# hazdzz/STGCN

Measured on AMD Instinct MI355X. Metric: training windows/sec, METR-LA ChebConv K=3 bs=32, higher is better.
Workload: dtype f32; 1 GPU; C2: METR-LA 207 nodes, STGCNChebGraphConv Ks=3 Kt=3, n_his=12, bs=32 per GPU, fp32, dropout 0.5, AdamW lr 1e-3 wd 1e-3; full step zero_grad+fwd+MSE+bwd+opt; graph=real metr_la adj -> sym_norm_lap -> cheb GSO, global_batch=32, parallelism=dp1, output_block=fused HIP path (stgcn_outblock_*), launch=hipGraph replay, chains=1, backward_products=fp32, operator_products=fp32

## Files before the change

### include/stgcn_hip.h

```cpp
#ifndef STGCN_HIP_H
#define STGCN_HIP_H
#include <stddef.h>
#include <stdint.h>
#ifdef __cplusplus
extern "C" {
#endif

#define STGCN_ABI_VERSION 9

#define STGCN_OK 0
#define STGCN_ERR_UNSUPPORTED 1
#define STGCN_ERR_INVALID 2
#define STGCN_ERR_LAUNCH 3

#define STGCN_ACT_GLU 0
#define STGCN_ACT_GTU 1
#define STGCN_GC_CHEB 0
#define STGCN_GC_KIPF 1

#define STGCN_DTYPE_F32 0
#define STGCN_DTYPE_BF16 1

typedef struct stgcn_stblock_desc {
    int32_t B, T, N;
    int32_t c_in;
    int32_t c0, c1, c2;
    int32_t Kt, Ks;
    int32_t act;
    int32_t graph_conv;
    int32_t training;
    float droprate;
    float ln_eps;
    int32_t need_dx;
    int32_t reserved;
    int32_t prepacked;
    int32_t defer_reduce;
    int64_t x_bstride;
    const int64_t* x_index_dev;
    int64_t x_index_stride;
    const int64_t* x_window_dev;
    int32_t dy_rowstats_ready;
    int32_t dtype;
} stgcn_stblock_desc;

typedef struct stgcn_stblock_params {
    const float *tc1_w, *tc1_b, *tc1_aw, *tc1_ab;
    const float *al_w, *al_b;
    const float *gc_w, *gc_b;
    const float *tc2_w, *tc2_b, *tc2_aw, *tc2_ab;
    const float *ln_w, *ln_b;
} stgcn_stblock_params;

typedef struct stgcn_stblock_grads {
    float *tc1_w, *tc1_b, *tc1_aw, *tc1_ab;
    float *al_w, *al_b;
    float *gc_w, *gc_b;
    float *tc2_w, *tc2_b, *tc2_aw, *tc2_ab;
    float *ln_w, *ln_b;
} stgcn_stblock_grads;

typedef struct stgcn_stblock_plan {
    int64_t T1, T2, rows1, rows2, NP;
    int64_t y_floats;
    int64_t saved_floats, ws_floats;
    int64_t sv_U1, sv_S1;
    int64_t sv_A;
    int64_t sv_Xk;
    int64_t sv_G;
    int64_t sv_U2, sv_S2;
    int64_t sv_mean, sv_rstd;
    int64_t sv_rowstat;
    int64_t ws_W1p, ws_W1d, ws_b1, ws_Wap, ws_WaT, ws_ba, ws_W2p, ws_W2d, ws_b2;
    int64_t ws_W1dense;
    int64_t recompute_tc1;
    int64_t ws_WaDense;
    int64_t thin_tc1;
    int64_t ws_rowstat_b;
    int64_t ws_dZ2;
    int64_t ws_dYg;
    int64_t ws_dA;
    int64_t ws_dZ1;
    int64_t ws_part;
    int64_t part_floats;
    int64_t tiled_gc;
    int64_t ws_Gk;
    int64_t ws_XT;
    int64_t fused_tc2_bwd;
    int64_t ws_W2dense;
    int64_t fused_tc1_bwd;
    int64_t stored_US2;
    int64_t ws_chain;
    int64_t chain_words;
} stgcn_stblock_plan;

int stgcn_version(void);
const char* stgcn_backend(void);
const char* stgcn_last_error(void);

int stgcn_stblock_plan_query(const stgcn_stblock_desc* desc, stgcn_stblock_plan* plan);

int stgcn_gso_prepare(const float* gso, int32_t N, int32_t terms, float* gso_pad, float* gso_t_pad, float* scratch, void* stream);

int stgcn_gso_layout(int32_t N, int32_t terms, int64_t* NP, int64_t* mats, int64_t* scratch_mats, int32_t* tiled);

int stgcn_set_debug_stages(int32_t on);

int stgcn_set_tc1_bwd_wgs(int32_t n);

int stgcn_stblock_chain_status(const stgcn_stblock_desc* desc, const float* ws, uint32_t* sticky, void* stream);

int stgcn_set_tc2ln_peers(int32_t n);

int stgcn_set_gc_tiled_min_nodes(int32_t n);

int stgcn_set_gc_precision(int32_t mode);

int stgcn_set_slab_gc_precision(int32_t mode);

int stgcn_set_bwd_precision(int32_t mode);

int stgcn_set_gemm_big_nt(int32_t nt);

int stgcn_set_gc_ld_pad(int32_t pad);

int stgcn_stblock_forward(const stgcn_stblock_desc* desc, const stgcn_stblock_params* params, const float* x,
                          const float* gso_pad, float* y, float* saved, float* ws, uint64_t seed, uint64_t offset,
                          const uint64_t* offset_dev, void* stream);

int stgcn_stblock_backward(const stgcn_stblock_desc* desc, const stgcn_stblock_params* params, const float* x,
                           const float* gso_t_pad, const float* dy, const float* y, const float* saved, float* ws,
                           const stgcn_stblock_grads* grads, float* dx, uint64_t seed, uint64_t offset,
                           const uint64_t* offset_dev, void* stream);

typedef struct stgcn_ln_hook {
    float* rowstat;
    const float* y;
    const float *gamma, *beta;
    int32_t N, C, reserved, training;
    float droprate;
    int32_t dtype;
    uint64_t seed, offset;
    const uint64_t* offset_dev;
} stgcn_ln_hook;
int stgcn_stblock_ln_hook(const stgcn_stblock_desc* desc, const stgcn_stblock_params* params, const float* y, float* ws, uint64_t seed,
                          uint64_t offset, const uint64_t* offset_dev, stgcn_ln_hook* hook);
int stgcn_stblock_backward_hook(const stgcn_stblock_desc* desc, const stgcn_stblock_params* params, const float* x,
                                const float* gso_t_pad, const float* dy, const float* y, const float* saved, float* ws,
                                const stgcn_stblock_grads* grads, float* dx, uint64_t seed, uint64_t offset,
                                const uint64_t* offset_dev, const stgcn_ln_hook* dx_hook, void* stream);

int stgcn_dropout_mask(float* out, int64_t n, float droprate, uint64_t seed, uint64_t offset, const uint64_t* offset_dev,
                       void* stream);

typedef struct stgcn_outblock_desc {
    int32_t B, T, N;
    int32_t c_in, c0, c1, c_end;
    int32_t Ko;
    int32_t act;
    int32_t training;
    float droprate;
    float ln_eps;
    int32_t need_dx;
    int32_t dtype;
    int32_t prepacked;
    int32_t defer_reduce;
} stgcn_outblock_desc;

typedef struct stgcn_outblock_params {
    const float *tc_w, *tc_b, *tc_aw, *tc_ab, *ln_w, *ln_b, *fc1_w, *fc1_b, *fc2_w, *fc2_b;
} stgcn_outblock_params;
typedef struct stgcn_outblock_grads {
    float *tc_w, *tc_b, *tc_aw, *tc_ab, *ln_w, *ln_b, *fc1_w, *fc1_b, *fc2_w, *fc2_b;
    float* loss;
} stgcn_outblock_grads;

typedef struct stgcn_head_loss {
    const float* pred;
    const float* target;
    const int64_t* target_index_dev;
    int64_t target_index_stride;
    const int64_t* target_window_dev;
    float grad_scale;
    int32_t reserved;
} stgcn_head_loss;

typedef struct stgcn_outblock_plan {
    int64_t T1, rows, rows_in;
    int64_t out_floats;
    int64_t saved_floats, ws_floats;
    int64_t sv_U, sv_S;
    int64_t sv_mean, sv_rstd;
    int64_t sv_yln;
    int64_t sv_hd;
    int64_t sv_rowstat;
    int64_t ws_Wp, ws_Wd, ws_b, ws_W1p, ws_W1d;
    int64_t ws_rowstat_b, ws_dh1, ws_dyln, ws_dZ, ws_part, part_floats;
    int64_t ws_chain;
    int64_t chain_words;
} stgcn_outblock_plan;

int stgcn_outblock_plan_query(const stgcn_outblock_desc* desc, stgcn_outblock_plan* plan);
int stgcn_outblock_forward(const stgcn_outblock_desc* desc, const stgcn_outblock_params* params, const float* x, float* out,
                           float* saved, float* ws, uint64_t seed, uint64_t offset, const uint64_t* offset_dev, void* stream);
int stgcn_outblock_chain_status(const stgcn_outblock_desc* desc, const float* ws, uint32_t* sticky, void* stream);
int64_t stgcn_set_chain_spin_ticks(int64_t ticks);
int stgcn_outblock_backward(const stgcn_outblock_desc* desc, const stgcn_outblock_params* params, const float* x,
                            const float* dout, const float* saved, float* ws, const stgcn_outblock_grads* grads, float* dx,
                            void* stream);
int stgcn_outblock_backward_hook(const stgcn_outblock_desc* desc, const stgcn_outblock_params* params, const float* x,
                                 const float* dout, const float* saved, float* ws, const stgcn_outblock_grads* grads, float* dx,
                                 const stgcn_ln_hook* dx_hook, void* stream);
int stgcn_outblock_backward_loss(const stgcn_outblock_desc* desc, const stgcn_outblock_params* params, const float* x,
                                 const stgcn_head_loss* loss, const float* saved, float* ws, const stgcn_outblock_grads* grads, float* dx,
                                 const stgcn_ln_hook* dx_hook, void* stream);

typedef struct stgcn_prepack_block {
    const stgcn_stblock_desc* desc;
    const stgcn_stblock_params* params;
    float* ws;
} stgcn_prepack_block;
typedef struct stgcn_step_counter {
    int64_t* ptr;
    int64_t inc, mod;
} stgcn_step_counter;
int stgcn_prepack(int32_t n_blocks, const stgcn_prepack_block* blocks, const stgcn_outblock_desc* head_desc,
                  const stgcn_outblock_params* head_params, float* head_ws, int32_t n_counters, const stgcn_step_counter* counters,
                  void* stream);
int stgcn_prepack_park(int32_t n_blocks, const stgcn_prepack_block* blocks, const stgcn_outblock_desc* head_desc,
                  const stgcn_outblock_params* head_params, float* head_ws, int32_t n_counters, const stgcn_step_counter* counters,
                  void* stream);
int stgcn_prepack_flush(void);

typedef struct stgcn_adamw_tensor {
    float* param;
    const float* grad;
    float* exp_avg;
    float* exp_avg_sq;
    int64_t numel;
} stgcn_adamw_tensor;
int stgcn_adamw_step(const stgcn_adamw_tensor* tensors, int32_t count, float lr, float beta1, float beta2, float eps,
                     float weight_decay, int64_t step, const int64_t* step_dev, const float* lr_dev, void* stream);

typedef struct stgcn_flush_block {
    const stgcn_stblock_desc* desc;
    const stgcn_stblock_grads* grads;
    float* ws;
} stgcn_flush_block;
typedef struct stgcn_adamw_hyper {
    float lr, beta1, beta2, eps, weight_decay;
    int64_t step;
    const int64_t* step_dev;
    const float* lr_dev;
} stgcn_adamw_hyper;
int stgcn_grad_flush(int32_t n_blocks, const stgcn_flush_block* blocks, const stgcn_outblock_desc* head_desc,
                     const stgcn_outblock_grads* head_grads, float* head_ws, const stgcn_adamw_tensor* opt, int32_t opt_count,
                     const stgcn_adamw_hyper* hyper, void* stream);

#define STGCN_OPT_ADAMW 0
#define STGCN_OPT_NADAMW 1
#define STGCN_OPT_LION 2
typedef struct stgcn_optim_hyper {
    int32_t kind;
    double lr, beta1, beta2, eps, weight_decay, momentum_decay;
    int64_t step;
    const int64_t* step_dev;
    const float* lr_dev;
    float mu_product;
    float* mu_product_dev;
} stgcn_optim_hyper;
int stgcn_optim_step(const stgcn_adamw_tensor* tensors, int32_t count, const stgcn_optim_hyper* hyper, void* stream);
int stgcn_grad_flush_optim(int32_t n_blocks, const stgcn_flush_block* blocks, const stgcn_outblock_desc* head_desc,
                           const stgcn_outblock_grads* head_grads, float* head_ws, const stgcn_adamw_tensor* opt, int32_t opt_count,
                           const stgcn_optim_hyper* hyper, void* stream);

int stgcn_mse_loss_grad(const float* pred, const float* target, int64_t n, float grad_scale, float* loss, float* dpred,
                        const int64_t* target_index_dev, int64_t target_index_stride, void* stream);
int stgcn_mse_loss_grad_windows(const float* pred, const float* target, int64_t n, float grad_scale, float* loss, float* dpred,
                                const int64_t* target_index_dev, int64_t target_index_stride, const int64_t* target_window_dev,
                                int64_t window_floats, void* stream);

#define STGCN_EVAL_STATE_WORDS 264
#define STGCN_EVAL_POS_WORDS 4
int stgcn_eval_arm(double* state, int64_t* pos, void* stream);
int stgcn_eval_accumulate(const float* pred, const float* target, int32_t B, int32_t N, const float* scale, const float* mean,
                          int64_t first_valid, int64_t* pos, int64_t target_stride, int64_t num_windows, double* state, void* stream);

// ... 8 lines not shown
```

### stgcn_amd/_lib.py

```python
from __future__ import annotations

import ctypes as C
import os
from typing import Optional

_HERE = os.path.dirname(os.path.abspath(__file__))
DEFAULT_LIB = os.path.join(_HERE, "libstgcn_hip.so")

STGCN_OK = 0
ABI_VERSION = 9
ACT = {"glu": 0, "gtu": 1}
GRAPH_CONV = {"cheb_graph_conv": 0, "graph_conv": 1}
DTYPE_F32, DTYPE_BF16 = 0, 1
EVAL_STATE_WORDS, EVAL_POS_WORDS = 264, 4

_fp = C.POINTER(C.c_float)


class StblockDesc(C.Structure):
    _fields_ = [("B", C.c_int32), ("T", C.c_int32), ("N", C.c_int32), ("c_in", C.c_int32),
                ("c0", C.c_int32), ("c1", C.c_int32), ("c2", C.c_int32), ("Kt", C.c_int32), ("Ks", C.c_int32),
                ("act", C.c_int32), ("graph_conv", C.c_int32), ("training", C.c_int32),
                ("droprate", C.c_float), ("ln_eps", C.c_float), ("need_dx", C.c_int32), ("reserved", C.c_int32),
                ("prepacked", C.c_int32), ("defer_reduce", C.c_int32),
                ("x_bstride", C.c_int64), ("x_index_dev", C.c_void_p), ("x_index_stride", C.c_int64), ("x_window_dev", C.c_void_p),
                ("dy_rowstats_ready", C.c_int32), ("dtype", C.c_int32)]


class LnHook(C.Structure):
    _fields_ = [("rowstat", C.c_void_p), ("y", C.c_void_p), ("gamma", C.c_void_p), ("beta", C.c_void_p),
                ("N", C.c_int32), ("C", C.c_int32), ("reserved", C.c_int32), ("training", C.c_int32), ("droprate", C.c_float), ("dtype", C.c_int32),
                ("seed", C.c_uint64), ("offset", C.c_uint64), ("offset_dev", C.c_void_p)]


PARAM_FIELDS = ["tc1_w", "tc1_b", "tc1_aw", "tc1_ab", "al_w", "al_b", "gc_w", "gc_b",
                "tc2_w", "tc2_b", "tc2_aw", "tc2_ab", "ln_w", "ln_b"]


class StblockParams(C.Structure):
    _fields_ = [(n, C.c_void_p) for n in PARAM_FIELDS]


class StblockGrads(C.Structure):
    _fields_ = [(n, C.c_void_p) for n in PARAM_FIELDS]


PLAN_FIELDS = ["T1", "T2", "rows1", "rows2", "NP", "y_floats", "saved_floats", "ws_floats",
               "sv_U1", "sv_S1", "sv_A", "sv_Xk", "sv_G", "sv_U2", "sv_S2", "sv_mean", "sv_rstd", "sv_rowstat",
               "ws_W1p", "ws_W1d", "ws_b1", "ws_Wap", "ws_WaT", "ws_ba", "ws_W2p", "ws_W2d", "ws_b2", "ws_W1dense", "recompute_tc1", "ws_WaDense", "thin_tc1",
               "ws_rowstat_b", "ws_dZ2", "ws_dYg", "ws_dA", "ws_dZ1", "ws_part", "part_floats",
               "tiled_gc", "ws_Gk", "ws_XT", "fused_tc2_bwd", "ws_W2dense", "fused_tc1_bwd", "stored_US2", "ws_chain", "chain_words"]


class StblockPlan(C.Structure):
    _fields_ = [(n, C.c_int64) for n in PLAN_FIELDS]


class OutblockDesc(C.Structure):
    _fields_ = [("B", C.c_int32), ("T", C.c_int32), ("N", C.c_int32), ("c_in", C.c_int32), ("c0", C.c_int32), ("c1", C.c_int32),
                ("c_end", C.c_int32), ("Ko", C.c_int32), ("act", C.c_int32), ("training", C.c_int32), ("droprate", C.c_float),
                ("ln_eps", C.c_float), ("need_dx", C.c_int32), ("dtype", C.c_int32), ("prepacked", C.c_int32),
                ("defer_reduce", C.c_int32)]


HEAD_PARAM_FIELDS = ["tc_w", "tc_b", "tc_aw", "tc_ab", "ln_w", "ln_b", "fc1_w", "fc1_b", "fc2_w", "fc2_b"]


class OutblockParams(C.Structure):
    _fields_ = [(n, C.c_void_p) for n in HEAD_PARAM_FIELDS]


class PrepackBlock(C.Structure):
    _fields_ = [("desc", C.POINTER(StblockDesc)), ("params", C.POINTER(StblockParams)), ("ws", C.c_void_p)]


class OutblockGrads(C.Structure):
    _fields_ = [(n, C.c_void_p) for n in HEAD_PARAM_FIELDS] + [("loss", C.c_void_p)]


class HeadLoss(C.Structure):
    _fields_ = [("pred", C.c_void_p), ("target", C.c_void_p), ("target_index_dev", C.c_void_p), ("target_index_stride", C.c_int64),
                ("target_window_dev", C.c_void_p), ("grad_scale", C.c_float), ("reserved", C.c_int32)]


HEAD_PLAN_FIELDS = ["T1", "rows", "rows_in", "out_floats", "saved_floats", "ws_floats", "sv_U", "sv_S", "sv_mean", "sv_rstd", "sv_yln",
                    "sv_hd", "sv_rowstat", "ws_Wp", "ws_Wd", "ws_b", "ws_W1p", "ws_W1d", "ws_rowstat_b", "ws_dh1", "ws_dyln", "ws_dZ", "ws_part",
                    "part_floats", "ws_chain", "chain_words"]


class OutblockPlan(C.Structure):
    _fields_ = [(n, C.c_int64) for n in HEAD_PLAN_FIELDS]


class AdamwTensor(C.Structure):
    _fields_ = [("param", C.c_void_p), ("grad", C.c_void_p), ("exp_avg", C.c_void_p), ("exp_avg_sq", C.c_void_p), ("numel", C.c_int64)]


class StepCounter(C.Structure):
    _fields_ = [("ptr", C.c_void_p), ("inc", C.c_int64), ("mod", C.c_int64)]


class FlushBlock(C.Structure):
    _fields_ = [("desc", C.POINTER(StblockDesc)), ("grads", C.POINTER(StblockGrads)), ("ws", C.c_void_p)]


class AdamwHyper(C.Structure):
    _fields_ = [("lr", C.c_float), ("beta1", C.c_float), ("beta2", C.c_float), ("eps", C.c_float), ("weight_decay", C.c_float),
                ("step", C.c_int64), ("step_dev", C.c_void_p), ("lr_dev", C.c_void_p)]


OPT_ADAMW, OPT_NADAMW, OPT_LION = 0, 1, 2


class OptimHyper(C.Structure):
    _fields_ = [("kind", C.c_int32), ("lr", C.c_double), ("beta1", C.c_double), ("beta2", C.c_double), ("eps", C.c_double),
                ("weight_decay", C.c_double), ("momentum_decay", C.c_double), ("step", C.c_int64), ("step_dev", C.c_void_p),
                ("lr_dev", C.c_void_p), ("mu_product", C.c_float), ("mu_product_dev", C.c_void_p)]


class StgcnError(RuntimeError):
    pass


class _Lib:
    def __init__(self, path: str):
        if not os.path.exists(path):
            raise StgcnError(
                f"{path} not found: the HIP extension has not been built. Run `python -c 'import __graft_entry__ as g; "
                f"g.build()'` (or `python -m stgcn_amd.build`). There is no fallback path.")
        self.path = path
        self.dll = C.CDLL(path)
        d = self.dll
        d.stgcn_version.restype = C.c_int
        got = int(d.stgcn_version())
        if got != ABI_VERSION:
            raise StgcnError(f"{path} was built for ABI revision {got}, this binding needs {ABI_VERSION} (include/stgcn_hip.h "
                             f"STGCN_ABI_VERSION): rebuild with `python -m stgcn_amd.build --force`")
        d.stgcn_backend.restype = C.c_char_p
        d.stgcn_last_error.restype = C.c_char_p
        d.stgcn_stblock_plan_query.argtypes = [C.POINTER(StblockDesc), C.POINTER(StblockPlan)]
        d.stgcn_gso_prepare.argtypes = [C.c_void_p, C.c_int32, C.c_int32, C.c_void_p, C.c_void_p, C.c_void_p, C.c_void_p]
        d.stgcn_gso_layout.argtypes = [C.c_int32, C.c_int32, C.POINTER(C.c_int64), C.POINTER(C.c_int64), C.POINTER(C.c_int64),
                                       C.POINTER(C.c_int32)]
        d.stgcn_gso_layout.restype = C.c_int
        d.stgcn_set_gc_tiled_min_nodes.argtypes = [C.c_int32]
        d.stgcn_set_gc_tiled_min_nodes.restype = C.c_int
        d.stgcn_outblock_backward_loss.argtypes = [C.POINTER(OutblockDesc), C.POINTER(OutblockParams), C.c_void_p, C.POINTER(HeadLoss), C.c_void_p,
                                                   C.c_void_p, C.POINTER(OutblockGrads), C.c_void_p, C.POINTER(LnHook), C.c_void_p]
        d.stgcn_outblock_backward_loss.restype = C.c_int
        d.stgcn_set_bwd_precision.argtypes = [C.c_int32]
        d.stgcn_set_bwd_precision.restype = C.c_int
        d.stgcn_set_slab_gc_precision.argtypes = [C.c_int32]
        d.stgcn_set_slab_gc_precision.restype = C.c_int
        d.stgcn_set_tc1_bwd_wgs.argtypes = [C.c_int32]
        d.stgcn_set_tc1_bwd_wgs.restype = C.c_int
        d.stgcn_set_tc2ln_peers.argtypes = [C.c_int32]
        d.stgcn_set_tc2ln_peers.restype = C.c_int
        d.stgcn_stblock_chain_status.argtypes = [C.POINTER(StblockDesc), C.c_void_p, C.POINTER(C.c_uint32), C.c_void_p]
        d.stgcn_stblock_chain_status.restype = C.c_int
        d.stgcn_set_debug_stages.argtypes = [C.c_int32]
        d.stgcn_set_debug_stages.restype = C.c_int
        d.stgcn_set_gc_precision.argtypes = [C.c_int32]
        d.stgcn_set_gc_precision.restype = C.c_int
        d.stgcn_set_gc_ld_pad.argtypes = [C.c_int32]
        d.stgcn_set_gc_ld_pad.restype = C.c_int
        d.stgcn_set_gemm_big_nt.argtypes = [C.c_int32]
        d.stgcn_set_gemm_big_nt.restype = C.c_int
        d.stgcn_set_chain_spin_ticks.argtypes = [C.c_int64]
        d.stgcn_set_chain_spin_ticks.restype = C.c_int64
        d.stgcn_outblock_chain_status.argtypes = [C.POINTER(OutblockDesc), C.c_void_p, C.POINTER(C.c_uint32), C.c_void_p]
        d.stgcn_outblock_chain_status.restype = C.c_int
        d.stgcn_stblock_forward.argtypes = [C.POINTER(StblockDesc), C.POINTER(StblockParams), C.c_void_p, C.c_void_p,
                                            C.c_void_p, C.c_void_p, C.c_void_p, C.c_uint64, C.c_uint64, C.c_void_p, C.c_void_p]
        d.stgcn_stblock_backward.argtypes = [C.POINTER(StblockDesc), C.POINTER(StblockParams), C.c_void_p, C.c_void_p,
                                             C.c_void_p, C.c_void_p, C.c_void_p, C.c_void_p, C.POINTER(StblockGrads), C.c_void_p,
                                             C.c_uint64, C.c_uint64, C.c_void_p, C.c_void_p]
        d.stgcn_stblock_backward_hook.argtypes = [C.POINTER(StblockDesc), C.POINTER(StblockParams), C.c_void_p, C.c_void_p,
                                                  C.c_void_p, C.c_void_p, C.c_void_p, C.c_void_p, C.POINTER(StblockGrads), C.c_void_p,
                                                  C.c_uint64, C.c_uint64, C.c_void_p, C.POINTER(LnHook), C.c_void_p]
        d.stgcn_stblock_ln_hook.argtypes = [C.POINTER(StblockDesc), C.POINTER(StblockParams), C.c_void_p, C.c_void_p, C.c_uint64, C.c_uint64,
                                            C.c_void_p, C.POINTER(LnHook)]
        d.stgcn_outblock_backward_hook.argtypes = [C.POINTER(OutblockDesc), C.POINTER(OutblockParams), C.c_void_p, C.c_void_p, C.c_void_p,
                                                   C.c_void_p, C.POINTER(OutblockGrads), C.c_void_p, C.POINTER(LnHook), C.c_void_p]
        for f in ("stgcn_stblock_backward_hook", "stgcn_stblock_ln_hook", "stgcn_outblock_backward_hook"):
            getattr(d, f).restype = C.c_int
        d.stgcn_dropout_mask.argtypes = [C.c_void_p, C.c_int64, C.c_float, C.c_uint64, C.c_uint64, C.c_void_p, C.c_void_p]
        d.stgcn_outblock_plan_query.argtypes = [C.POINTER(OutblockDesc), C.POINTER(OutblockPlan)]
        d.stgcn_outblock_forward.argtypes = [C.POINTER(OutblockDesc), C.POINTER(OutblockParams), C.c_void_p, C.c_void_p, C.c_void_p,
                                             C.c_void_p, C.c_uint64, C.c_uint64, C.c_void_p, C.c_void_p]
        d.stgcn_outblock_backward.argtypes = [C.POINTER(OutblockDesc), C.POINTER(OutblockParams), C.c_void_p, C.c_void_p, C.c_void_p,
                                              C.c_void_p, C.POINTER(OutblockGrads), C.c_void_p, C.c_void_p]
        for f in ("stgcn_outblock_plan_query", "stgcn_outblock_forward", "stgcn_outblock_backward"):
            getattr(d, f).restype = C.c_int
        d.stgcn_adamw_step.argtypes = [C.POINTER(AdamwTensor), C.c_int32, C.c_float, C.c_float, C.c_float, C.c_float, C.c_float, C.c_int64,
                                       C.c_void_p, C.c_void_p, C.c_void_p]
        d.stgcn_adamw_step.restype = C.c_int
        d.stgcn_prepack.argtypes = [C.c_int32, C.POINTER(PrepackBlock), C.POINTER(OutblockDesc), C.POINTER(OutblockParams), C.c_void_p,
                                    C.c_int32, C.POINTER(StepCounter), C.c_void_p]
        d.stgcn_prepack.restype = C.c_int
        d.stgcn_prepack_park.argtypes = [C.c_int32, C.POINTER(PrepackBlock), C.POINTER(OutblockDesc), C.POINTER(OutblockParams), C.c_void_p,
                                    C.c_int32, C.POINTER(StepCounter), C.c_void_p]
        d.stgcn_prepack_park.restype = C.c_int
        d.stgcn_prepack_flush.argtypes = []
        d.stgcn_prepack_flush.restype = C.c_int
        d.stgcn_grad_flush.argtypes = [C.c_int32, C.POINTER(FlushBlock), C.POINTER(OutblockDesc), C.POINTER(OutblockGrads), C.c_void_p,
                                       C.POINTER(AdamwTensor), C.c_int32, C.POINTER(AdamwHyper), C.c_void_p]
        d.stgcn_grad_flush.restype = C.c_int
        d.stgcn_optim_step.argtypes = [C.POINTER(AdamwTensor), C.c_int32, C.POINTER(OptimHyper), C.c_void_p]
        d.stgcn_optim_step.restype = C.c_int
        d.stgcn_grad_flush_optim.argtypes = [C.c_int32, C.POINTER(FlushBlock), C.POINTER(OutblockDesc), C.POINTER(OutblockGrads), C.c_void_p,
                                             C.POINTER(AdamwTensor), C.c_int32, C.POINTER(OptimHyper), C.c_void_p]
        d.stgcn_grad_flush_optim.restype = C.c_int
        d.stgcn_mse_loss_grad.argtypes = [C.c_void_p, C.c_void_p, C.c_int64, C.c_float, C.c_void_p, C.c_void_p, C.c_void_p, C.c_int64,
                                          C.c_void_p]
        d.stgcn_mse_loss_grad.restype = C.c_int
        d.stgcn_mse_loss_grad_windows.argtypes = [C.c_void_p, C.c_void_p, C.c_int64, C.c_float, C.c_void_p, C.c_void_p, C.c_void_p, C.c_int64,
                                                  C.c_void_p, C.c_int64, C.c_void_p]
        d.stgcn_mse_loss_grad_windows.restype = C.c_int
        d.stgcn_eval_arm.argtypes = [C.c_void_p, C.c_void_p, C.c_void_p]
        d.stgcn_eval_arm.restype = C.c_int
        d.stgcn_eval_accumulate.argtypes = [C.c_void_p, C.c_void_p, C.c_int32, C.c_int32, C.c_void_p, C.c_void_p, C.c_int64, C.c_void_p,
                                            C.c_int64, C.c_int64, C.c_void_p, C.c_void_p]
        d.stgcn_eval_accumulate.restype = C.c_int
        d.stgcn_profile_enable.argtypes = [C.c_int]
        d.stgcn_profile_enable.restype = C.c_int
        d.stgcn_profile_collect.argtypes = [C.c_char_p, C.c_size_t]
        d.stgcn_profile_collect.restype = C.c_int
        for f in ("stgcn_stblock_plan_query", "stgcn_gso_prepare", "stgcn_stblock_forward", "stgcn_stblock_backward",
                  "stgcn_dropout_mask"):
            getattr(d, f).restype = C.c_int
        self.backend = d.stgcn_backend().decode()
        self.is_emulator = self.backend.startswith("emu")

    def check(self, rc: int, what: str):
        if rc != STGCN_OK:
            msg = self.dll.stgcn_last_error().decode()
            if rc == 1:
                raise NotImplementedError(f"{what}: {msg}")
            if rc == 2:
                raise ValueError(f"{what}: {msg}")
            raise StgcnError(f"{what}: {msg} (code {rc})")


_lib: Optional[_Lib] = None


def use_library(path: str) -> _Lib:
    global _lib
    _lib = _Lib(path)
    return _lib


def lib() -> _Lib:
    global _lib
    if _lib is None:
        _lib = _Lib(os.environ.get("STGCN_AMD_LIB", DEFAULT_LIB))
    return _lib


EXPORTED_SYMBOLS = ["stgcn_version", "stgcn_backend", "stgcn_last_error", "stgcn_stblock_plan_query", "stgcn_gso_prepare",
                    "stgcn_stblock_forward", "stgcn_stblock_backward", "stgcn_dropout_mask", "stgcn_profile_enable",
                    "stgcn_profile_collect", "stgcn_outblock_plan_query", "stgcn_outblock_forward", "stgcn_outblock_backward", "stgcn_adamw_step", "stgcn_prepack",
                    "stgcn_mse_loss_grad", "stgcn_mse_loss_grad_windows", "stgcn_grad_flush", "stgcn_gso_layout", "stgcn_set_gc_tiled_min_nodes",
                    "stgcn_set_gc_precision", "stgcn_set_gc_ld_pad", "stgcn_set_debug_stages",
                    "stgcn_stblock_ln_hook", "stgcn_stblock_backward_hook", "stgcn_outblock_backward_hook", "stgcn_set_tc1_bwd_wgs",
                    "stgcn_set_slab_gc_precision", "stgcn_outblock_backward_loss", "stgcn_set_bwd_precision", "stgcn_set_gemm_big_nt",
                    "stgcn_set_chain_spin_ticks", "stgcn_outblock_chain_status", "stgcn_set_tc2ln_peers", "stgcn_stblock_chain_status", "stgcn_prepack_park", "stgcn_prepack_flush",
                    "stgcn_optim_step", "stgcn_grad_flush_optim", "stgcn_eval_arm", "stgcn_eval_accumulate"]
```

### stgcn_amd/csrc/stgcn_capi_head.inc

```

struct HeadGeom {
    int T1, NC, KP, KCH, CPin, ln_spg, ln_sg, fc_wgs;
    int dense_bwd;
    int fused_ln_bwd;
    int64_t rows, rows_in, slabs;
    WgradGeom wc, wf;
    long off_ln_g, off_ln_b, off_fc, total;
};

static int head_check(const stgcn_outblock_desc* d) {
    if (!d) return fail(STGCN_ERR_INVALID, "desc is NULL");
    if (d->B < 1 || d->T < 1 || d->N < 1 || d->c_in < 1 || d->Ko < 1) return fail(STGCN_ERR_INVALID, "B/T/N/c_in/Ko must be positive");
    if (d->T < d->Ko) return fail(STGCN_ERR_INVALID, "T=%d shorter than Ko=%d", d->T, d->Ko);
    if (d->act != STGCN_ACT_GLU && d->act != STGCN_ACT_GTU) return fail(STGCN_ERR_INVALID, "act must be glu or gtu");
    if (d->droprate < 0.f || d->droprate >= 1.f) return fail(STGCN_ERR_INVALID, "droprate must be in [0, 1)");
    if (!(d->c0 == 64 || d->c0 == 128)) return fail(STGCN_ERR_UNSUPPORTED, "output-head conv channels must be 64 or 128 (got %d)", d->c0);
    if (d->c1 != 128) return fail(STGCN_ERR_UNSUPPORTED, "output-head fc1 width must be 128 (got %d)", d->c1);
    if (d->c_end != 1) return fail(STGCN_ERR_UNSUPPORTED, "end_channel must be 1 (got %d)", d->c_end);
    if ((d->c_in & 3) != 0 && d->Ko * d->c_in > 16) return fail(STGCN_ERR_UNSUPPORTED, "c_in=%d must be a multiple of 4", d->c_in);
    if (d->dtype != STGCN_DTYPE_F32 && d->dtype != STGCN_DTYPE_BF16) return fail(STGCN_ERR_INVALID, "dtype must be STGCN_DTYPE_F32 or STGCN_DTYPE_BF16");
    return STGCN_OK;
}

static HeadGeom head_geom(const stgcn_outblock_desc* d) {
    HeadGeom g;
    g.T1 = d->T - d->Ko + 1;
    g.NC = 2 * d->c0;
    g.KP = (int)rup((int64_t)d->Ko * d->c_in, 16);
    g.KCH = g.KP / 16;
    g.CPin = (int)rup(d->c_in, 16);
    {
        static const int off = getenv("STGCN_TCONV4") ? atoi(getenv("STGCN_TCONV4")) == 0 : 0;
        g.dense_bwd = !off && g.T1 == 1 && g.NC == 256 && d->Ko * d->c_in == 256 && (d->c_in & 3) == 0;
    }
    g.rows = (int64_t)d->B * g.T1 * d->N;
    g.rows_in = (int64_t)d->B * d->T * d->N;
    g.slabs = (int64_t)d->B * g.T1;
    const long n = (long)d->N * d->c0, n4 = n / 4;
    const int colgroups = (int)((n4 + kThreads - 1) / kThreads);
    int sg = (512 + colgroups - 1) / colgroups;
    if (colgroups >= kLnBigColgroups) sg = (4096 + colgroups - 1) / colgroups;
    if (sg > g.slabs) sg = (int)g.slabs;
    if (sg < 1) sg = 1;
    g.ln_spg = (int)((g.slabs + sg - 1) / sg);
    g.ln_sg = (int)((g.slabs + g.ln_spg - 1) / g.ln_spg);
    const bool fusable = (fuse_mask() & FUSE_HEAD_LN_BWD) && (fuse_mask() & FUSE_ROWSTATS) && g.dense_bwd && d->c0 == 128 && d->c1 == 128 &&
                         d->N <= 1024 && colgroups < kLnBigColgroups;
    const long sg_plain = g.ln_sg, sg_max = fusable && g.slabs > sg_plain ? g.slabs : sg_plain;
    g.fused_ln_bwd = fusable && d->need_dx;
    if (g.fused_ln_bwd) { g.ln_spg = 1; g.ln_sg = (int)g.slabs; }
    const long tiles = (g.rows + head_fc_tile_rows() - 1) / head_fc_tile_rows();
    g.fc_wgs = (int)(tiles < 512 * 32 / head_fc_tile_rows() / 2 ? tiles : 512 * 32 / head_fc_tile_rows() / 2);
    long o = 0;
    auto take = [&](long f) { long at = o; o += (f + 63) / 64 * 64; return at; };
    g.off_ln_g = take(sg_max * n);
    g.off_ln_b = take((d->dtype == STGCN_DTYPE_BF16 ? sg_max : sg_plain) * n);
    g.off_fc = take((long)g.fc_wgs * (d->c1 + 2));
    constexpr int t_conv = 160, t_fc = 96;
    const bool one_round = g.rows <= 32768;
    g.wc = wgrad_geom(g.rows, d->Ko * d->c_in, g.NC, 0, one_round ? t_conv : 256);
    g.wc.off = take(g.wc.floats);
    g.wf = wgrad_geom(g.rows, d->c0, d->c1, 0, one_round ? t_fc : 256);
    g.wf.off = take(g.wf.floats);
    g.total = o;
    return g;
}

static void reduce_jobs_head(ReduceList& L, const stgcn_outblock_desc* d, const HeadGeom& g, const float* part, const float* dyln,
                             const stgcn_outblock_grads* G) {
    {
        const WgradGeom& w = g.wc;
        const float* wp = part + w.off;
        const float* bp = wp + (long)w.chunks * w.Mpad * w.NC;
        const long ps = (long)w.Mpad * w.NC;
        L.add(G->tc_w, wp, w.chunks, ps, w.NC, d->Ko, d->c_in, w.Mpad, d->c_in, 1, (long)d->c_in * d->Ko, 1, d->Ko);
        L.add_flat(G->tc_b, bp, w.chunks, w.NC, w.NC);
        if (d->c_in > d->c0) {
            L.add(G->tc_aw, wp + (long)(d->Ko - 1) * d->c_in, w.chunks, ps, 1, d->c0, d->c_in, 0, w.Mpad, 1, 0, d->c_in, 1);
            L.add_flat(G->tc_ab, bp, w.chunks, w.NC, d->c0);
        }
    }
    {
        const WgradGeom& w = g.wf;
        const float* wp = part + w.off;
        const float* bp = wp + (long)w.chunks * w.Mpad * w.NC;
        L.add(G->fc1_w, wp, w.chunks, (long)w.Mpad * w.NC, 1, d->c1, d->c0, 0, w.Mpad, 1, 0, d->c0, 1);
        L.add_flat(G->fc1_b, bp, w.chunks, w.NC, d->c1);
    }
    L.add_flat(G->fc2_w, part + g.off_fc, g.fc_wgs, d->c1 + 2, d->c1);
    L.add_flat(G->fc2_b, part + g.off_fc + d->c1, g.fc_wgs, d->c1 + 2, 1);
    if (G->loss) L.add_flat(G->loss, part + g.off_fc + d->c1 + 1, g.fc_wgs, d->c1 + 2, 1);
    const int n = d->N * d->c0;
    L.add_flat(G->ln_w, part + g.off_ln_g, g.ln_sg, n, n);
    if (g.fused_ln_bwd && d->dtype == STGCN_DTYPE_F32) L.add_flat(G->ln_b, dyln, g.ln_sg, n, n);
    else L.add_flat(G->ln_b, part + g.off_ln_b, g.ln_sg, n, n);
}

int stgcn_outblock_plan_query(const stgcn_outblock_desc* d, stgcn_outblock_plan* p) {
    int rc = head_check(d);
    if (rc) return rc;
    if (!p) return fail(STGCN_ERR_INVALID, "plan is NULL");
    const HeadGeom g = head_geom(d);
    memset(p, 0, sizeof(*p));
    p->T1 = g.T1; p->rows = g.rows; p->rows_in = g.rows_in; p->out_floats = g.rows * d->c_end;
    int64_t o = 0;
    auto take = [&](int64_t n) { int64_t at = o; o += rup(n, 64); return at; };
    const bool bf = d->dtype == STGCN_DTYPE_BF16;
    auto act = [&](int64_t n) { return bf ? (n + 1) / 2 : n; };
    p->sv_U = take(act(g.rows * d->c0));
    p->sv_S = take(act(g.rows * d->c0));
    p->sv_mean = take(g.slabs);
    p->sv_rstd = take(g.slabs);
    p->sv_yln = take(act(g.rows * d->c0));
    p->sv_hd = take(act(g.rows * d->c1));
    p->sv_rowstat = take(2 * g.rows);
    p->saved_floats = o;
    o = 0;
    p->chain_words = kChainHdr + g.slabs;
    p->ws_chain = take(p->chain_words);
    p->ws_Wp = take((int64_t)g.NC * g.KP);
    p->ws_Wd = take((int64_t)d->Ko * g.NC * g.CPin);
    p->ws_b = take(g.NC);
    p->ws_W1p = take((int64_t)d->c0 * d->c1);
    p->ws_W1d = take((int64_t)d->c1 * d->c0);
    p->ws_rowstat_b = take(2 * g.rows + 2 * g.slabs);
    p->ws_dh1 = take(act(g.rows * d->c1));
    p->ws_dyln = take(act(g.rows * d->c0));
    p->ws_dZ = take(act(g.rows * g.NC));
    p->part_floats = g.total;
    p->ws_part = take(g.total);
    p->ws_floats = o;
    return STGCN_OK;
}

}
namespace {
bool pack_fill_head(PackList& L, const stgcn_outblock_desc* d, const stgcn_outblock_params* P, const stgcn_outblock_plan& pl, float* ws,
                    bool all) {
    const HeadGeom g = head_geom(d);
    bool ok = true;
    ok &= L.add(PK_TCONV_FWD, g.NC * g.KP, ws + pl.ws_Wp, P->tc_w, P->tc_b, P->tc_aw, P->tc_ab, d->c_in, d->c0, d->Ko, g.KCH);
    if (d->need_dx || all) {
        if (g.dense_bwd)
            ok &= L.add(PK_TCONV_BWDT, g.NC * d->Ko * d->c_in, ws + pl.ws_Wd, P->tc_w, P->tc_b, P->tc_aw, P->tc_ab, d->c_in, d->c0, d->Ko, g.NC / 16);
        else
            ok &= L.add(PK_TCONV_BWD, d->Ko * g.NC * g.CPin, ws + pl.ws_Wd, P->tc_w, P->tc_b, P->tc_aw, P->tc_ab, d->c_in, d->c0, d->Ko,
                        d->Ko * g.NC / 16);
    }
    ok &= L.add(PK_TCONV_BIAS, g.NC, ws + pl.ws_b, P->tc_w, P->tc_b, P->tc_aw, P->tc_ab, d->c_in, d->c0, d->Ko, 0);
    ok &= L.add(PK_LIN_FWD, d->c0 * d->c1, ws + pl.ws_W1p, P->fc1_w, nullptr, nullptr, nullptr, d->c0, d->c1, 1, d->c0 / 16);
    ok &= L.add(PK_LIN_BWD, d->c1 * d->c0, ws + pl.ws_W1d, P->fc1_w, nullptr, nullptr, nullptr, d->c0, d->c1, 1, d->c1 / 16);
    ok &= L.add(PK_ZERO, (int)pl.chain_words, ws + pl.ws_chain, nullptr, nullptr, nullptr, nullptr, 0, 0, 0, 0);
    return ok;
}
}
extern "C" {

}
namespace {
int prepack_impl(int32_t n_blocks, const stgcn_prepack_block* blocks, const stgcn_outblock_desc* hd, const stgcn_outblock_params* hp,
                 float* hws, int32_t n_counters, const stgcn_step_counter* counters, void* stream, bool park);
}
extern "C" {
int stgcn_prepack(int32_t n_blocks, const stgcn_prepack_block* blocks, const stgcn_outblock_desc* hd, const stgcn_outblock_params* hp,
                  float* hws, int32_t n_counters, const stgcn_step_counter* counters, void* stream) {
    return prepack_impl(n_blocks, blocks, hd, hp, hws, n_counters, counters, stream, false);
}
int stgcn_prepack_flush(void) {
    return flush_pending_pack();
}
int stgcn_prepack_park(int32_t n_blocks, const stgcn_prepack_block* blocks, const stgcn_outblock_desc* hd, const stgcn_outblock_params* hp,
                       float* hws, int32_t n_counters, const stgcn_step_counter* counters, void* stream) {
    return prepack_impl(n_blocks, blocks, hd, hp, hws, n_counters, counters, stream, true);
}
}
namespace {
int prepack_impl(int32_t n_blocks, const stgcn_prepack_block* blocks, const stgcn_outblock_desc* hd, const stgcn_outblock_params* hp,
                 float* hws, int32_t n_counters, const stgcn_step_counter* counters, void* stream, bool park) {
    if (n_blocks < 0 || (n_blocks > 0 && !blocks)) return fail(STGCN_ERR_INVALID, "stgcn_prepack: bad block list");
    if (n_counters < 0 || n_counters > kMaxStepCounters || (n_counters > 0 && !counters))
        return fail(STGCN_ERR_INVALID, "stgcn_prepack: at most %d step counters", kMaxStepCounters);
    STGCN_FLUSH_PENDING_PACK();
    g_prof_tag = 0;
    PackList L;
    L.pa.ncounters = n_counters;
    for (int k = 0; k < n_counters; ++k) {
        if (!counters[k].ptr) return fail(STGCN_ERR_INVALID, "stgcn_prepack: NULL step counter %d", k);
        L.pa.cptr[k] = reinterpret_cast<long*>(counters[k].ptr); L.pa.cinc[k] = (long)counters[k].inc; L.pa.cmod[k] = (long)counters[k].mod;
    }
    auto flush_list = [&]() -> int {
        const int rc = launch_pack_list("prepack", L, (hipStream_t)stream);
        L = PackList();
        return rc;
    };
    for (int i = 0; i < n_blocks; ++i) {
        const stgcn_prepack_block& b = blocks[i];
        if (!b.desc || !b.params || !b.ws) return fail(STGCN_ERR_INVALID, "stgcn_prepack: NULL entry in block %d", i);
        stgcn_stblock_plan pl;
        int rc = stgcn_stblock_plan_query(b.desc, &pl);
        if (rc) return rc;
        PackList trial = L;
        if (!pack_fill_block(trial, b.desc, b.params, pl, b.ws, true)) {
            if (L.nj == 0) return fail(STGCN_ERR_UNSUPPORTED, "stgcn_prepack: one block needs more than %d pack jobs", kMaxPackJobs);
            rc = flush_list();
            if (rc) return rc;
            trial = L;
            if (!pack_fill_block(trial, b.desc, b.params, pl, b.ws, true)) return fail(STGCN_ERR_UNSUPPORTED, "stgcn_prepack: pack job table overflow");
        }
        L = trial;
    }
    if (hd) {
        if (!hp || !hws) return fail(STGCN_ERR_INVALID, "stgcn_prepack: head params / ws are NULL");
        stgcn_outblock_plan pl;
        int rc = stgcn_outblock_plan_query(hd, &pl);
        if (rc) return rc;
        PackList trial = L;
        if (!pack_fill_head(trial, hd, hp, pl, hws, true)) {
            rc = flush_list();
            if (rc) return rc;
            trial = L;
            if (!pack_fill_head(trial, hd, hp, pl, hws, true)) return fail(STGCN_ERR_UNSUPPORTED, "stgcn_prepack: pack job table overflow");
        }
        L = trial;
    }
    if (L.nj == 0 && L.pa.ncounters == 0) return STGCN_OK;
    if (park && L.nj > 0) {
        g_pending_pack.valid = true;
        g_pending_pack.L = L;
        g_pending_pack.st = (hipStream_t)stream;
        return STGCN_OK;
    }
    return launch_pack_list("prepack", L, (hipStream_t)stream);
}
}
extern "C" {

int stgcn_outblock_forward(const stgcn_outblock_desc* d, const stgcn_outblock_params* P, const float* x, float* out, float* saved,
                           float* ws, uint64_t seed, uint64_t offset, const uint64_t* offset_dev, void* stream) {
    STGCN_FLUSH_PENDING_PACK();
    stgcn_outblock_plan pl;
    int rc = stgcn_outblock_plan_query(d, &pl);
    if (rc) return rc;
    if (!P || !x || !out || !saved || !ws) return fail(STGCN_ERR_INVALID, "stgcn_outblock_forward: NULL buffer");
    if (!P->tc_w || !P->tc_b || !P->ln_w || !P->ln_b || !P->fc1_w || !P->fc2_w)
        return fail(STGCN_ERR_INVALID, "stgcn_outblock_forward: missing parameter pointer");
    if (d->c_in > d->c0 && !P->tc_aw) return fail(STGCN_ERR_INVALID, "tc_aw required when c_in > c0");
    const HeadGeom g = head_geom(d);
    hipStream_t st = (hipStream_t)stream;
    g_prof_tag = 0;
    g_bf16 = d->dtype == STGCN_DTYPE_BF16;

    if (!d->prepacked) {
        PackList L;
        if (!pack_fill_head(L, d, P, pl, ws, false)) return fail(STGCN_ERR_INVALID, "pack job table overflow");
        rc = launch_pack_list("head.pack", L, st);
        if (rc) return rc;
    }

    TconvFwdArgs t;
    memset(&t, 0, sizeof(t));
    t.ts.src = x; t.ts.C = d->c_in; t.ts.taps = d->Ko; t.ts.N = d->N; t.ts.Tsrc = d->T; t.ts.Tdst = g.T1; t.ts.dir = 1; t.ts.rows = g.rows;
    t.Wp = ws + pl.ws_Wp; t.bias = ws + pl.ws_b; t.KCH = g.KCH; t.Cout = d->c0; t.act = d->act;
    t.U = saved + pl.sv_U; t.S = saved + pl.sv_S; t.rowstat = reinterpret_cast<float2*>(saved + pl.sv_rowstat);

    if (head_fuse_mode() && g.T1 == 1 && d->c0 == 128 && d->c1 == 128 && tconv4_ok(t)) {
        constexpr int KC = 4;
        int tm = 0, ticket = 0;
        {
            const int forced = head_fuse_mode() > 1 ? head_fuse_mode() : 0;
            const size_t l2 = (size_t)(tconv2_lds_floats(g.KP, 256, 32) + 48) * sizeof(float), l4 = (size_t)(tconv2_lds_floats(g.KP, 256, 64) + 48) * sizeof(float);
            const int cap2 = STGCN_ET_VALUE(wg_capacity(head_fwd_kernel<2, KC, ET>, 512, l2));
            const int cap4 = STGCN_ET_VALUE(wg_capacity(head_fwd_kernel<4, KC, ET>, 512, l4));
            const int t2 = cdiv(g.rows, 32), t4 = cdiv(g.rows, 64);
            const bool tk2 = d->N >= 32 && d->N <= 1024 && cap2 >= 4 * cdiv(d->N, 32) + 16, tk4 = d->N >= 64 && d->N <= 2048 && cap4 >= 4 * cdiv(d->N, 64) + 16;
            if (forced == 2) { if (d->N >= 32 && t2 <= cap2) tm = 2; }
            else if (forced == 4) { if (d->N >= 64 && t4 <= cap4) tm = 4; }
            else if (forced == 3) { if (tk2) { tm = 2; ticket = 1; } }
            else if (forced == 5) { if (tk4) { tm = 4; ticket = 1; } }
            else if (tk2 && t2 <= cap2) { tm = 2; ticket = 1; }
            else if (tk4 && t4 <= cap4) { tm = 4; ticket = 1; }
            else if (tk2) { tm = 2; ticket = 1; }
            else if (tk4) { tm = 4; ticket = 1; }
        }
        if (tm) {
            Tconv4Args aa;
            memset(&aa, 0, sizeof(aa));
            aa.f = t;
            HeadFcTail f;
            memset(&f, 0, sizeof(f));
            const int TR = 16 * tm, tiles = cdiv(g.rows, TR);
            f.chain.words = reinterpret_cast<unsigned*>(ws + pl.ws_chain); f.chain.ncount = (int)g.slabs; f.chain.total = (unsigned)tiles;
            f.chain.spin = g_chain_spin_ticks;
            f.gamma = P->ln_w; f.beta = P->ln_b; f.yln = saved + pl.sv_yln; f.mean = saved + pl.sv_mean; f.rstd = saved + pl.sv_rstd;
            f.eps = d->ln_eps;
            f.W1p = ws + pl.ws_W1p; f.b1 = P->fc1_b; f.w2 = P->fc2_w; f.b2 = P->fc2_b; f.hd = saved + pl.sv_hd; f.out = out;
            f.training = d->training && d->droprate > 0.f;
            f.keep_scale = 1.0f / (1.0f - d->droprate); f.thresh = drop_thresh(d->droprate); f.seed = seed; f.offset = offset;
            f.offset_dev = offset_dev;
            f.use_ticket = ticket;
            const size_t lds = (size_t)(tconv2_lds_floats(g.KP, 256, TR) + 48) * sizeof(float);
            if (tm == 2) STGCN_LAUNCH_ET("head.fwd", st, (head_fwd_kernel<2, KC, ET>), dim3(tiles), dim3(512), lds, aa, f);
            else STGCN_LAUNCH_ET("head.fwd", st, (head_fwd_kernel<4, KC, ET>), dim3(tiles), dim3(512), lds, aa, f);
            return STGCN_OK;
        }
    }
    rc = launch_tconv_fwd("head.tconv_fwd", t, st);
    if (rc) return rc;

    LnFwdArgs ln;
    memset(&ln, 0, sizeof(ln));
    ln.U = saved + pl.sv_U; ln.S = saved + pl.sv_S; ln.gamma = P->ln_w; ln.beta = P->ln_b; ln.y = saved + pl.sv_yln;
    ln.mean = saved + pl.sv_mean; ln.rstd = saved + pl.sv_rstd; ln.rowstat = reinterpret_cast<const float2*>(saved + pl.sv_rowstat);
    ln.n = d->N * d->c0; ln.N = d->N; ln.C = d->c0; ln.act = d->act; ln.training = 0;
    ln.eps = d->ln_eps; ln.keep_scale = 1.f; ln.thresh = 0;
    const bool fuse_ln = (fuse_mask() & FUSE_HEAD_LN_FWD) && g.T1 == 1 && d->c0 % 16 == 0 && d->c0 <= 128 && d->N <= 1024;
    if (!fuse_ln) {
        rc = launch_ln_fwd("head.ln_fwd", ln, g.slabs, st);
        if (rc) return rc;
    }

    FcFwdArgs f;
    memset(&f, 0, sizeof(f));
    if (fuse_ln) f.ln = ln;
    f.ts.src = saved + pl.sv_yln; f.ts.C = d->c0; f.ts.taps = 1; f.ts.N = d->N; f.ts.Tsrc = g.T1; f.ts.Tdst = g.T1; f.ts.dir = 1;
    f.ts.rows = g.rows;
    f.W1p = ws + pl.ws_W1p; f.b1 = P->fc1_b; f.w2 = P->fc2_w; f.b2 = P->fc2_b; f.hd = saved + pl.sv_hd; f.out = out;
    f.KCH = d->c0 / 16; f.c1 = d->c1; f.training = d->training && d->droprate > 0.f;
    f.keep_scale = 1.0f / (1.0f - d->droprate); f.thresh = drop_thresh(d->droprate); f.seed = seed; f.offset = offset;
    f.offset_dev = offset_dev;
    const int fct = (getenv("STGCN_HEAD_FC_TILE") || g.rows <= 32768) ? head_fc_tile_rows() : 32;
    const size_t lds = (size_t)(kTileHdr + fct * (128 + 4)) * sizeof(float);
    if (fct == 16) STGCN_LAUNCH_ET("head.fc_fwd", st, (fc_fwd_kernel<1, ET>), dim3(cdiv(g.rows, 16)), dim3(kThreads), lds, f);
    else STGCN_LAUNCH_ET("head.fc_fwd", st, (fc_fwd_kernel<2, ET>), dim3(cdiv(g.rows, 32)), dim3(kThreads), lds, f);
    return STGCN_OK;
}


int stgcn_outblock_chain_status(const stgcn_outblock_desc* d, const float* ws, uint32_t* sticky, void* stream) {
    STGCN_FLUSH_PENDING_PACK();
    stgcn_outblock_plan pl;
    int rc = stgcn_outblock_plan_query(d, &pl);
    if (rc) return rc;
    if (!ws || !sticky) return fail(STGCN_ERR_INVALID, "stgcn_outblock_chain_status: NULL argument");
    if (hipStreamSynchronize((hipStream_t)stream) != hipSuccess) return fail(STGCN_ERR_LAUNCH, "stgcn_outblock_chain_status: stream synchronisation failed");
    unsigned w = 0;
    if (hipMemcpy(&w, reinterpret_cast<const unsigned*>(ws + pl.ws_chain) + 2, sizeof(w), hipMemcpyDeviceToHost) != hipSuccess)
        return fail(STGCN_ERR_LAUNCH, "stgcn_outblock_chain_status: copy failed");
    *sticky = w;
    return STGCN_OK;
}

}
namespace {
int outblock_backward_impl(const stgcn_outblock_desc* d, const stgcn_outblock_params* P, const float* x, const float* dout,
                           const stgcn_head_loss* hl, const float* saved, float* ws, const stgcn_outblock_grads* G, float* dx,
                           const stgcn_ln_hook* dx_hook, void* stream);
}
extern "C" {
int stgcn_outblock_backward(const stgcn_outblock_desc* d, const stgcn_outblock_params* P, const float* x, const float* dout,
                            const float* saved, float* ws, const stgcn_outblock_grads* G, float* dx, void* stream) {
    return outblock_backward_impl(d, P, x, dout, nullptr, saved, ws, G, dx, nullptr, stream);
}

int stgcn_outblock_backward_hook(const stgcn_outblock_desc* d, const stgcn_outblock_params* P, const float* x, const float* dout,
                                 const float* saved, float* ws, const stgcn_outblock_grads* G, float* dx, const stgcn_ln_hook* dx_hook,
                                 void* stream) {
    return outblock_backward_impl(d, P, x, dout, nullptr, saved, ws, G, dx, dx_hook, stream);
}

int stgcn_outblock_backward_loss(const stgcn_outblock_desc* d, const stgcn_outblock_params* P, const float* x, const stgcn_head_loss* hl,
                                 const float* saved, float* ws, const stgcn_outblock_grads* G, float* dx, const stgcn_ln_hook* dx_hook,
                                 void* stream) {
    if (!hl || !hl->pred || !hl->target) return fail(STGCN_ERR_INVALID, "stgcn_outblock_backward_loss: NULL pred / target");
    if (!G || !G->loss) return fail(STGCN_ERR_INVALID, "stgcn_outblock_backward_loss: grads->loss is NULL");
    if (hl->target_window_dev && !hl->target_index_dev)
        return fail(STGCN_ERR_INVALID, "stgcn_outblock_backward_loss: target_window_dev (window table) needs target_index_dev != NULL");
    return outblock_backward_impl(d, P, x, nullptr, hl, saved, ws, G, dx, dx_hook, stream);
}
}
namespace {
int outblock_backward_impl(const stgcn_outblock_desc* d, const stgcn_outblock_params* P, const float* x, const float* dout,
                           const stgcn_head_loss* hl, const float* saved, float* ws, const stgcn_outblock_grads* G, float* dx,
                           const stgcn_ln_hook* dx_hook, void* stream) {
    STGCN_FLUSH_PENDING_PACK();
    stgcn_outblock_plan pl;
    int rc = stgcn_outblock_plan_query(d, &pl);
    if (rc) return rc;
    if (!P || !x || (!dout && !hl) || !saved || !ws || !G) return fail(STGCN_ERR_INVALID, "stgcn_outblock_backward: NULL buffer");
    if (d->need_dx && !dx) return fail(STGCN_ERR_INVALID, "stgcn_outblock_backward: need_dx set but dx is NULL");
    if (dx_hook && dx_hook->rowstat && (dx_hook->N != d->N || dx_hook->C != d->c_in || !d->need_dx))
        return fail(STGCN_ERR_INVALID, "stgcn_outblock_backward: dx_hook describes a LayerNorm over [%d, %d], the input gradient is [%d, %d] per slab",
                    dx_hook->N, dx_hook->C, d->N, d->c_in);
    const HeadGeom g = head_geom(d);
    hipStream_t st = (hipStream_t)stream;
    g_prof_tag = 0;
    g_bf16 = d->dtype == STGCN_DTYPE_BF16;
    if (dx_hook && dx_hook->rowstat && dx_hook->dtype != d->dtype)
        return fail(STGCN_ERR_INVALID, "stgcn_outblock_backward: dx_hook describes tensors of another dtype than this call");
    float* part = ws + pl.ws_part;
    const int training = d->training && d->droprate > 0.f;
    const bool own_rowstats = (fuse_mask() & FUSE_ROWSTATS) && d->c0 == d->c1 && d->c0 == 128;

    {
        FcBwdArgs a;
        memset(&a, 0, sizeof(a));
        a.dout = dout; a.hd = saved + pl.sv_hd; a.w2 = P->fc2_w; a.W1d = ws + pl.ws_W1d; a.dh1 = ws + pl.ws_dh1; a.dyln = ws + pl.ws_dyln;
        a.part = part + g.off_fc; a.rows = g.rows; a.c0 = d->c0; a.c1 = d->c1; a.KCH = d->c1 / 16;
        a.grad_scale = training ? 1.0f / (1.0f - d->droprate) : 1.0f;
        if (hl) {
            a.pred = hl->pred; a.target = hl->target; a.target_index = reinterpret_cast<const long*>(hl->target_index_dev);
            a.target_index_stride = (long)hl->target_index_stride; a.loss_scale = hl->grad_scale;
            a.target_window = reinterpret_cast<const long*>(hl->target_window_dev); a.target_window_elems = (unsigned)(g.rows / d->B);
        }
        if (own_rowstats) {
            a.rs.rowstat = reinterpret_cast<float2*>(ws + pl.ws_rowstat_b); a.rs.U = saved + pl.sv_U; a.rs.S = saved + pl.sv_S; a.rs.gamma = P->ln_w;
            a.rs.mean = saved + pl.sv_mean; a.rs.rstd = saved + pl.sv_rstd; a.rs.N = d->N; a.rs.C = d->c0; a.rs.act = d->act; a.rs.training = 0;
            a.rs.keep_scale = 1.f;
        }
        const size_t lds = (size_t)(head_fc_tile_rows() * (d->c1 + 4) + 8 * d->c1 + 16) * sizeof(float);
        if (head_fc_tile_rows() == 16) {
            if (d->c0 == 128) STGCN_LAUNCH_ETB("head.fc_bwd", st, (fc_bwd_kernel<1, 2, ET>), dim3(g.fc_wgs), dim3(kThreads), lds, a);
            else STGCN_LAUNCH_ETB("head.fc_bwd", st, (fc_bwd_kernel<1, 1, ET>), dim3(g.fc_wgs), dim3(kThreads), lds, a);
        } else if (d->c0 == 128) STGCN_LAUNCH_ETB("head.fc_bwd", st, (fc_bwd_kernel<2, 2, ET>), dim3(g.fc_wgs), dim3(kThreads), lds, a);
        else STGCN_LAUNCH_ETB("head.fc_bwd", st, (fc_bwd_kernel<2, 1, ET>), dim3(g.fc_wgs), dim3(kThreads), lds, a);
    }
    TconvBwdWeightArgs wa;
    memset(&wa, 0, sizeof(wa));
    wa.ts.src = saved + pl.sv_yln; wa.ts.C = d->c0; wa.ts.taps = 1; wa.ts.N = d->N; wa.ts.Tsrc = g.T1; wa.ts.Tdst = g.T1; wa.ts.dir = 1;
    wa.ts.rows = g.rows;
    wa.dZ = ws + pl.ws_dh1; wa.part = part + g.wf.off; wa.NC = d->c1; wa.Mpad = g.wf.Mpad; wa.rows_per_chunk = g.wf.rows_per_chunk;
    wa.chunks = g.wf.chunks;
    const TconvBwdWeightArgs wfc = wa;
    TconvBwdWeightArgs wcv = wa;
    wcv.ts.src = x; wcv.ts.C = d->c_in; wcv.ts.taps = d->Ko; wcv.ts.Tsrc = d->T; wcv.ts.Tdst = g.T1;
    wcv.dZ = ws + pl.ws_dZ; wcv.part = part + g.wc.off; wcv.NC = g.NC; wcv.Mpad = g.wc.Mpad; wcv.rows_per_chunk = g.wc.rows_per_chunk;
    wcv.chunks = g.wc.chunks;
    const bool pair = wgrad_pair_ok(wcv, g.wc, wfc, g.wf);
    if (!pair) {
        rc = launch_bwd_weight("head.fc1_bwd_weight", wfc, g.wf, st);
        if (rc) return rc;
    }
    LnBwdArgs ln;
    memset(&ln, 0, sizeof(ln));
    ln.dy = ws + pl.ws_dyln; ln.U = saved + pl.sv_U; ln.S = saved + pl.sv_S; ln.gamma = P->ln_w;
    ln.mean = saved + pl.sv_mean; ln.rstd = saved + pl.sv_rstd; ln.rowstat = reinterpret_cast<float2*>(ws + pl.ws_rowstat_b);
    ln.dZ = ws + pl.ws_dZ; ln.dgam_part = part + g.off_ln_g; ln.dbet_part = part + g.off_ln_b;
    ln.n = d->N * d->c0; ln.N = d->N; ln.C = d->c0; ln.act = d->act; ln.training = 0; ln.spg = g.ln_spg; ln.slabs = g.slabs;
    ln.keep_scale = 1.f; ln.thresh = 0;
    if (!own_rowstats)
        STGCN_LAUNCH_ET("head.ln_bwd_rowstats", st, (ln_bwd_rowstats_kernel<ET>), dim3(cdiv(g.slabs * (ln.n / 4), kThreads)), dim3(kThreads), 0, ln);
    if (cdiv(ln.n / 4, kThreads) >= kLnBigColgroups) {
        ln.slabconst = reinterpret_cast<float2*>(ws + pl.ws_rowstat_b + 2 * g.rows);
        STGCN_LAUNCH("head.ln_slab_consts", st, ln_slab_consts_kernel, dim3((unsigned)g.slabs), dim3(kThreads), 64, ln);
    }
    const bool fused_ln = g.fused_ln_bwd && own_rowstats;
    if (!fused_ln)
        STGCN_LAUNCH_ET("head.ln_gate_bwd", st, (ln_gate_bwd_kernel<ET>), dim3(cdiv(ln.n / 4, kThreads), g.ln_sg), dim3(kThreads),
                        (8 + 2 * g.ln_spg) * sizeof(float), ln);
    bool hook_pending = false;
    if (d->need_dx && g.dense_bwd) {
        Tconv4Args aa;
        memset(&aa, 0, sizeof(aa));
        aa.f.ts.src = ws + pl.ws_dZ; aa.f.ts.C = g.NC; aa.f.ts.taps = 1; aa.f.ts.N = d->N; aa.f.ts.Tsrc = 1; aa.f.ts.Tdst = 1; aa.f.ts.dir = 1;
        aa.f.ts.rows = g.rows;
        aa.f.Wp = ws + pl.ws_Wd; aa.f.KCH = g.NC / 16; aa.f.Cout = 128;
        aa.out = dx; aa.outT = d->T; aa.outC = d->c_in;
        const bool epi = dx_hook && dx_hook->rowstat && dx_hook->C == d->c_in && (d->c_in == 64 || d->c_in == 128) && dx_hook->N == d->N;
        if (epi) aa.rs = rowstat_out(dx_hook);
        if (fused_ln) {
            aa.lnb.dy = ln.dy; aa.lnb.U = ln.U; aa.lnb.S = ln.S; aa.lnb.gamma = ln.gamma; aa.lnb.mean = ln.mean; aa.lnb.rstd = ln.rstd;
            aa.lnb.rowstat = ln.rowstat; aa.lnb.dZ = ln.dZ; aa.lnb.dgam = ln.dgam_part; aa.lnb.N = d->N; aa.lnb.C = d->c0; aa.lnb.act = d->act;
            aa.lnb.dbet = g_bf16 ? ln.dbet_part : nullptr;
        }
        rc = launch_tconv_fwd4<true>("head.tconv_bwd_data", aa, st);
        if (rc) return rc;
        if (dx_hook && dx_hook->rowstat && !epi) hook_pending = true;
    } else if (d->need_dx) {
        TconvBwdDataArgs a;
        memset(&a, 0, sizeof(a));
        a.ts.src = ws + pl.ws_dZ; a.ts.C = g.NC; a.ts.taps = d->Ko; a.ts.N = d->N; a.ts.Tsrc = g.T1; a.ts.Tdst = d->T; a.ts.dir = -1;
        a.ts.rows = g.rows_in;
        a.Wp = ws + pl.ws_Wd; a.KCH = d->Ko * g.NC / 16; a.Cin = d->c_in; a.Gmask = nullptr; a.dX = dx;
        rc = launch_bwd_data("head.tconv_bwd_data", a, g.CPin / 16, st);
        if (rc) return rc;
        if (dx_hook && dx_hook->rowstat) hook_pending = true;
    }
    rc = pair ? launch_wgrad_pair("head.wgrad_pair", wcv, g.wc, wfc, g.wf, st) : launch_bwd_weight("head.tconv_bwd_weight", wcv, g.wc, st);
    if (rc) return rc;
    if (hook_pending) {
        LnBwdArgs hl;
        memset(&hl, 0, sizeof(hl));
        const LnRowstatOut o = rowstat_out(dx_hook);
        hl.dy = dx; hl.y = o.y; hl.beta = o.beta; hl.gamma = o.gamma; hl.rowstat = o.rowstat;
        hl.n = o.N * o.C; hl.N = o.N; hl.C = o.C; hl.act = o.act; hl.training = o.training; hl.slabs = (long)d->B * d->T;
        hl.keep_scale = o.keep_scale; hl.thresh = o.thresh; hl.seed = o.seed; hl.offset = o.offset; hl.offset_dev = o.offset_dev;
        STGCN_LAUNCH_ET("ln_bwd_rowstats", st, (ln_bwd_rowstats_kernel<ET>), dim3(cdiv(hl.slabs * (hl.n / 4), kThreads)), dim3(kThreads), 0, hl);
    }
    if (d->defer_reduce) return STGCN_OK;
    ReduceList RL;
    reduce_jobs_head(RL, d, g, part, ws + pl.ws_dyln, G);
    return launch_reduce_list("head.reduce", RL, st);
}
// ... 257 lines not shown
```

### stgcn_amd/csrc/stgcn_kernels_fwd.hip.h

```cpp
#pragma once
#include "stgcn_device.hip.h"

namespace stgcn {

enum PackKind { PK_TCONV_FWD = 0, PK_TCONV_BWD = 1, PK_TCONV_BIAS = 2, PK_ALIGN_FWD = 3, PK_ALIGN_BWD = 4, PK_ALIGN_BIAS = 5,
                PK_LIN_FWD = 6, PK_LIN_BWD = 7,
                PK_TCONV_DENSE = 8, PK_ALIGN_DENSE = 9,
                PK_TCONV_BWDT = 10,
                PK_ZERO = 11 };

struct PackJob {
    int kind;
    int n;
    float* dst;
    const float* w;
    const float* b;
    const float* aw;
    const float* ab;
    int Cin, Cout, Kt, KCH, gated;
};
constexpr int kMaxPackJobs = 40;
constexpr int kMaxStepCounters = 4;
struct PackArgs {
    PackJob job[kMaxPackJobs];
// ... 517 lines not shown
    const ET* const src = tap_origin<ET>(ts);
    const TapWin tw = tap_win(ts);
    if ((ts.C & 3) == 0) {
        const int c4n = ts.C >> 2, c4sh = pow2_shift(c4n), per_tap = TR * c4n, total = ts.taps * per_tap;
        for (int base = 0; base < total; base += THREADS * SB) {
            f32x4 v[SB];
            int dst[SB];
#pragma unroll
            for (int i = 0; i < SB; ++i) {
                const int idx = base + i * THREADS + tid;
                v[i] = zero4();
                dst[i] = -1;
                if (idx < total) {
                    int tap = 0, rem = idx;
                    while (rem >= per_tap) { rem -= per_tap; ++tap; }
                    const int r = fast_div(rem, c4n, c4sh), c4 = rem - r * c4n;
                    dst[i] = r * lda + tap * ts.C + 4 * c4;
                    if (row0 + r < ts.rows) {
                        const RowCoord c = row_advance(ts, c0, r);
                        v[i] = ldx4(src + (tap_src_row(tw, (unsigned)c.b, (unsigned)(c.t * ts.N + c.n)) + (size_t)tap * ts.N) * ts.C + 4 * c4);
                    }
                }
            }
#pragma unroll
            for (int i = 0; i < SB; ++i)
                if (dst[i] >= 0) st4(At + dst[i], v[i]);
        }
        if (K < KP) {
            const int padw = KP - K;
            for (int idx = tid; idx < TR * padw; idx += THREADS) {
                const int r = idx / padw, q = idx - r * padw;
                At[r * lda + K + q] = 0.f;
            }
        }
    } else {
        const int total = TR * KP;
        for (int base = 0; base < total; base += THREADS * SB) {
            float v[SB];
            int dst[SB];
#pragma unroll
            for (int i = 0; i < SB; ++i) {
                const int idx = base + i * THREADS + tid;
                v[i] = 0.f;
                dst[i] = -1;
                if (idx < total) {
                    const int r = idx / KP, q = idx - r * KP;
                    dst[i] = r * lda + q;
                    if (q < K && row0 + r < ts.rows) {
                        const int tap = q / ts.C, ch = q - tap * ts.C;
                        const RowCoord c = row_advance(ts, c0, r);
                        v[i] = ldx1(src + (tap_src_row(tw, (unsigned)c.b, (unsigned)(c.t * ts.N + c.n)) + (size_t)tap * ts.N) * ts.C + ch);
                    }
                }
            }
#pragma unroll
            for (int i = 0; i < SB; ++i)
                if (dst[i] >= 0) At[dst[i]] = v[i];
        }
    }
}

inline int tconv2_lds_floats(int kp, int nc, int rows) { return rows * ((kp > nc ? kp : nc) + 4); }


struct LnRowstatOut {
    float2* rowstat;
    const float* y;
    const float* beta;
    const float* U;
    const float* S;
    const float* gamma;
    const float* mean;
    const float* rstd;
    int N, C, act, training;
    int mask_from_y;
    float keep_scale;
    uint32_t thresh;
    uint64_t seed, offset;
    const uint64_t* offset_dev;
};
__device__ __forceinline__ uint64_t ln_rowstat_offset(const LnRowstatOut& o) {
    return (o.rowstat && o.training) ? o.offset + (o.offset_dev ? *o.offset_dev : 0) : 0;
}
template <typename ET = float>
__device__ __forceinline__ float2 ln_rowstat4(const LnRowstatOut& o, uint64_t off, f32x4 dy, long slab, int node, int c) {
    const size_t e = ((size_t)slab * o.N + node) * o.C + c;
    const f32x4 ga = ld4(o.gamma + (size_t)node * o.C + c);
    f32x4 k = {1.f, 1.f, 1.f, 1.f};
    if (o.training && !(o.y && o.mask_from_y)) {
        k = dropout_scale4((uint64_t)slab * (((uint64_t)o.N * o.C) >> 2) + (((uint64_t)node * o.C + c) >> 2), o.seed, off, o.thresh, o.keep_scale);
    }
    float s1 = 0.f, s2 = 0.f;
    if (o.y) {
        const f32x4 y = ldx4(et_ptr<ET>(o.y) + e), be = ld4(o.beta + (size_t)node * o.C + c);
        const float ks = o.training ? o.keep_scale : 1.f;
        if (o.training && o.mask_from_y) {
#pragma unroll
            for (int i = 0; i < 4; ++i) {
                const float yi = y[i];
                k[i] = drop_kept(yi) ? o.keep_scale : 0.f;
            }
        }
#pragma unroll
        for (int i = 0; i < 4; ++i) {
            s1 += dy[i] * k[i] * ga[i];
            if (k[i] > 0.f) s2 += dy[i] * (y[i] - ks * be[i]);
        }
        return make_float2(s1, s2);
    }
    const f32x4 u = ldx4(et_ptr<ET>(o.U) + e), s = ldx4(et_ptr<ET>(o.S) + e);
    const float mean = o.mean[slab], rstd = o.rstd[slab];
#pragma unroll
    for (int i = 0; i < 4; ++i) dy[i] *= k[i];
#pragma unroll
    for (int i = 0; i < 4; ++i) {
        const float xh = (gate_fwd(u[i], s[i], o.act) - mean) * rstd;
        const float gg = dy[i] * ga[i];
        s1 += gg;
        s2 += gg * xh;
    }
    return make_float2(s1, s2);
}

struct LnGateBwdIn {
    const float* dy;
    const float* U;
    const float* S;
    const float* gamma;
    const float* mean;
    const float* rstd;
    const float2* rowstat;
    float* dZ;
    float* dgam;
    float* dbet;
    int N, C, act;
};
struct Tconv4Args {
    TconvFwdArgs f;
    float* out;
    int outT, outC;
    LnRowstatOut rs;
    LnGateBwdIn lnb;
};

struct HeadFcTail {
    ChainCtl chain;
    const float* gamma;
    const float* beta;
    float* yln;
    float* mean;
    float* rstd;
    float eps;
    const float* W1p;
    const float* b1;
    const float* w2;
    const float* b2;
    float* hd;
    float* out;
    int training;
    float keep_scale;
    uint32_t thresh;
    uint64_t seed, offset;
    const uint64_t* offset_dev;
    int use_ticket;
};

template <int TM, int KC, bool PLAIN, typename ET, bool HEADF = false>
__device__ __forceinline__ void tconv_fwd4_body(const Tconv4Args& aa, const HeadFcTail* ht) {
    static_assert(!(PLAIN && HEADF), "the fused head tail follows the gated epilogue");
    constexpr int WAVES = 8, NT = 2, THREADS = 512, TR = TM * 16, NC = 256, COUT = 128, LDZ = NC + 4;
    const TconvFwdArgs& a = aa.f;
    ET* const U_ = et_ptr<ET>(a.U);
    ET* const S_ = et_ptr<ET>(a.S);
    ET* const H_ = et_ptr<ET>(a.H);
    ET* const out_ = et_ptr<ET>(aa.out);
    extern __shared__ float stgcn_smem[];
    float* At = stgcn_smem;
    const int tid = threadIdx.x, wave = tid >> 6, lane = tid & 63, g = lane >> 4, l15 = lane & 15;
    long row0 = (long)xcd_item(blockIdx.x, gridDim.x) * TR;
    const int KCH = a.KCH, KP = KCH * 16, lda = KP + 4;

    f32x4 wA[KC][NT], wB[KC][NT];
    auto load_round = [&](f32x4 (&w)[KC][NT], int kc0) {
#pragma unroll
        for (int kc = 0; kc < KC; ++kc)
#pragma unroll
            for (int j = 0; j < NT; ++j)
                w[kc][j] = (kc0 + kc < KCH) ? ld4(a.Wp + ((size_t)((wave + WAVES * j) * KCH + kc0 + kc) * 64 + lane) * 4) : zero4();
    };
    load_round(wA, 0);
    if constexpr (HEADF) {
        if (ht->use_ticket) row0 = (long)chain_enter_peer(ht->chain, reinterpret_cast<unsigned*>(stgcn_smem + TR * LDZ + 4 * WAVES)) * TR;
    }
    bool staged = false;
    if constexpr (PLAIN) {
        if (aa.lnb.dy) {
            staged = true;
            const LnGateBwdIn& b = aa.lnb;
            const int N = b.N, C = b.C, c4n = C >> 2;
            const float inv_n = 1.0f / ((float)N * (float)C);
            const long rows = a.ts.rows, rend = row0 + TR < rows ? row0 + TR : rows;
            float* red = At + TR * lda;
            for (long slab = row0 / N; slab * N < rend; ++slab) {
                float x = 0.f, y = 0.f;
                for (int r = tid; r < N; r += THREADS) {
                    const float2 v = b.rowstat[slab * N + r];
                    x += v.x;
                    y += v.y;
                }
#pragma unroll
                for (int m = 32; m >= 1; m >>= 1) {
                    x += __shfl_xor(x, m);
                    y += __shfl_xor(y, m);
                }
                __syncthreads();
                if (lane == 0) {
                    red[wave] = x;
                    red[WAVES + wave] = y;
                }
                __syncthreads();
                float c1 = 0.f, c2 = 0.f;
#pragma unroll
                for (int w = 0; w < WAVES; ++w) {
                    c1 += red[w];
                    c2 += red[WAVES + w];
                }
                c1 *= inv_n;
                c2 *= inv_n;
                const float mean = b.mean[slab], rstd = b.rstd[slab];
                for (int idx = tid; idx < TR * c4n; idx += THREADS) {
                    const int row = idx / c4n, c4 = idx - row * c4n;
                    const long R = row0 + row;
                    if (R >= rows || R / N != slab) continue;
                    const int n = (int)(R - slab * N);
                    const size_t e = (size_t)R * C + 4 * c4;
                    const f32x4 dy = ldx4(et_ptr<ET>(b.dy) + e), u = ldx4(et_ptr<ET>(b.U) + e), sg = ldx4(et_ptr<ET>(b.S) + e),
                                ga = ld4(b.gamma + (size_t)n * C + 4 * c4);
                    f32x4 du, dq, dg;
#pragma unroll
                    for (int i = 0; i < 4; ++i) {
                        const float xh = (gate_fwd(u[i], sg[i], b.act) - mean) * rstd;
                        const float dh = rstd * (dy[i] * ga[i] - c1 - xh * c2);
                        dg[i] = dy[i] * xh;
                        float du_, dq_;
                        gate_bwd(dh, u[i], sg[i], b.act, du_, dq_);
                        du[i] = du_;
                        dq[i] = dq_;
                    }
                    st4(At + row * lda + 4 * c4, du);
                    st4(At + row * lda + C + 4 * c4, dq);
                    stx4_wt(et_ptr<ET>(b.dZ) + (size_t)R * 2 * C + 4 * c4, du);
                    stx4_wt(et_ptr<ET>(b.dZ) + (size_t)R * 2 * C + C + 4 * c4, dq);
// ... 60 lines not shown
            if (rin) stx4_wt(out_ + (((size_t)c.b * aa.outT + tap) * a.ts.N + c.n) * aa.outC + ci, v);
            if (aa.rs.rowstat) {
                const long slab = (long)c.b * aa.outT + tap;
                float2 p = rin ? ln_rowstat4<ET>(aa.rs, hoff, v, slab, c.n, ci) : make_float2(0.f, 0.f);
                for (int m = aa.outC >> 3; m >= 1; m >>= 1) {
                    p.x += __shfl_xor(p.x, m);
                    p.y += __shfl_xor(p.y, m);
                }
                if (rin && ci == 0) aa.rs.rowstat[slab * a.ts.N + c.n] = p;
            }
        }
    } else {
        constexpr int C4N = COUT / 4, NIT = TR * C4N / THREADS;
        const int c4 = tid & (C4N - 1);
        const f32x4 bp = ld4(a.bias + 4 * c4), bq = ld4(a.bias + COUT + 4 * c4);
        f32x4 uk[HEADF ? NIT : 1], sk[HEADF ? NIT : 1];
#pragma unroll
        for (int it = 0; it < NIT; ++it) {
            const int row = (tid + it * THREADS) / C4N;
            const long R = row0 + row;
            const f32x4 p = ld4(Zt + row * LDZ + 4 * c4), q = ld4(Zt + row * LDZ + COUT + 4 * c4);
            f32x4 u, sg, h;
#pragma unroll
            for (int i = 0; i < 4; ++i) {
                u[i] = p[i] + bp[i];
                sg[i] = sigmoid_f(q[i] + bq[i]);
                h[i] = gate_fwd(u[i], sg[i], a.act);
            }
            if constexpr (HEADF) {
                uk[it] = u;
                sk[it] = sg;
            } else if (R < a.ts.rows) {
                const size_t o = (size_t)R * COUT + 4 * c4;
                if (a.U) stx4_wt(U_ + o, u);
                if (a.S) stx4_wt(S_ + o, sg);
                if (a.H) stx4_wt(H_ + o, h);
            }
            if constexpr (HEADF) {
                f32x4 hs = h;
                if constexpr (sizeof(ET) == 2) {
                    const f32x4 ur = et_round4<ET>(u), sr_ = et_round4<ET>(sg);
#pragma unroll
                    for (int i = 0; i < 4; ++i) hs[i] = gate_fwd(ur[i], sr_[i], a.act);
                }
                st4(Zt + row * LDZ + 4 * c4, hs);
            }
            if (a.rowstat) {
                float sr = (h[0] + h[1]) + (h[2] + h[3]);
#pragma unroll
                for (int m = C4N >> 1; m >= 1; m >>= 1) sr += __shfl_xor(sr, m);
                const float mr = sr / (float)COUT;
                float d2 = 0.f;
#pragma unroll
                for (int i = 0; i < 4; ++i) d2 += (h[i] - mr) * (h[i] - mr);
#pragma unroll
                for (int m = C4N >> 1; m >= 1; m >>= 1) d2 += __shfl_xor(d2, m);
                if (c4 == 0 && R < a.ts.rows) {
                    if constexpr (HEADF) st2_wt(a.rowstat + R, make_float2(mr, d2));
                    else a.rowstat[R] = make_float2(mr, d2);
                }
            }
        }
        if constexpr (HEADF) {
            const HeadFcTail& f = *ht;
            const long rows = a.ts.rows;
            const int N = a.ts.N;
            const long rend = row0 + TR < rows ? row0 + TR : rows;
            const int s_lo = (int)(row0 / N), s_hi = (int)((rend - 1) / N);
            chain_drain_stores();
            __syncthreads();
            if (tid == 0 && !chain_withhold(f.chain, row0))
                for (int sw = s_lo; sw <= s_hi; ++sw) chain_publish_peer(f.chain, sw);
#pragma unroll
            for (int it = 0; it < NIT; ++it) {
                const long R = row0 + (tid + it * THREADS) / C4N;
                if (R < rows) {
                    const size_t o = (size_t)R * COUT + 4 * c4;
                    if (a.U) stx4_wt(U_ + o, uk[it]);
                    if (a.S) stx4_wt(S_ + o, sk[it]);
                }
            }
            PreW<1, 8> w1;
            pre_load_weights<1, 8>(w1, f.W1p, 8, wave, 8);
            f32x4 ga[NIT], be[NIT];
#pragma unroll
            for (int it = 0; it < NIT; ++it) {
                const int row = (tid + it * THREADS) / C4N;
                const long R = row0 + row < rows ? row0 + row : rows - 1;
                const int n = (int)(R % N);
                ga[it] = ld4(f.gamma + (size_t)n * COUT + 4 * c4);
                be[it] = ld4(f.beta + (size_t)n * COUT + 4 * c4);
            }
            const f32x4 w2 = ld4(f.w2 + 4 * c4);
            f32x4 b1 = zero4();
            if (f.b1) b1 = ld4(f.b1 + 4 * c4);
            const float b2 = f.b2 ? f.b2[0] : 0.f;
            const uint64_t off = f.offset + (f.offset_dev ? *f.offset_dev : 0);
            float* const gaveup = Zt + TR * LDZ + 4 * WAVES + 1;
            if (tid == 0) {
                bool ok = true;
                for (int sw = s_lo; sw <= s_hi; ++sw) {
                    const long w0 = (long)sw * N, w1r = w0 + N < rows ? w0 + N : rows;
                    ok &= chain_poll_peer(f.chain, sw, (unsigned)((w1r - 1) / TR - w0 / TR + 1));
                }
                *gaveup = ok ? 0.f : __builtin_nanf("");
            }
            __syncthreads();
            const float poison = *gaveup;
            float* red = Zt + TR * LDZ;
            float mean2[2] = {0.f, 0.f}, rstd2[2] = {1.f, 1.f};
            {
                const bool two = s_hi > s_lo;
                const float2* rs0 = a.rowstat + (size_t)s_lo * N;
                const float2* rs1 = a.rowstat + (size_t)s_hi * N;
                const float xa = ld2_sc1(rs0, N, 0).x, xb = two ? ld2_sc1(rs1, N, 0).x : 0.f;
                float sa1 = 0.f, sa2 = 0.f, sb1 = 0.f, sb2 = 0.f;
                for (int r = tid; r < N; r += THREADS) {
                    const float2 va = ld2_sc1(rs0, N, r);
                    float2 vb = make_float2(0.f, 0.f);
                    if (two) vb = ld2_sc1(rs1, N, r);
                    const float da = va.x - xa, db = vb.x - xb;
                    sa1 += da;
                    sa2 += va.y + (float)COUT * da * da;
                    sb1 += db;
                    sb2 += vb.y + (float)COUT * db * db;
                }
#pragma unroll
                for (int m = 32; m >= 1; m >>= 1) {
                    sa1 += __shfl_xor(sa1, m);
                    sa2 += __shfl_xor(sa2, m);
                    sb1 += __shfl_xor(sb1, m);
                    sb2 += __shfl_xor(sb2, m);
                }
                if (lane == 0) {
                    red[wave] = sa1;
                    red[WAVES + wave] = sa2;
                    red[2 * WAVES + wave] = sb1;
                    red[3 * WAVES + wave] = sb2;
                }
                __syncthreads();
                sa1 = sa2 = sb1 = sb2 = 0.f;
#pragma unroll
                for (int wv = 0; wv < WAVES; ++wv) {
                    sa1 += red[wv];
                    sa2 += red[WAVES + wv];
                    sb1 += red[2 * WAVES + wv];
                    sb2 += red[3 * WAVES + wv];
                }
                const float nf = (float)N, nc = (float)N * (float)COUT;
                const float dma = sa1 / nf, dmb = sb1 / nf;
                mean2[0] = xa + dma;
                mean2[1] = xb + dmb;
                rstd2[0] = 1.0f / sqrtf(fmaxf(sa2 - nc * dma * dma, 0.f) / nc + f.eps);
                rstd2[1] = 1.0f / sqrtf(fmaxf(sb2 - nc * dmb * dmb, 0.f) / nc + f.eps);
                if (tid == 0) {
                    if ((long)s_lo * N >= row0) {
                        f.mean[s_lo] = mean2[0];
                        f.rstd[s_lo] = rstd2[0];
                    }
                    if (two) {
                        f.mean[s_hi] = mean2[1];
                        f.rstd[s_hi] = rstd2[1];
                    }
                }
            }
            ET* const yln_ = et_ptr<ET>(f.yln);
#pragma unroll
            for (int it = 0; it < NIT; ++it) {
                const int row = (tid + it * THREADS) / C4N;
                const long R = row0 + row;
                f32x4 o = zero4();
                if (R < rows) {
                    const int wi = (int)(R / N) - s_lo;
                    const float mean = wi ? mean2[1] : mean2[0], rstd = wi ? rstd2[1] : rstd2[0];
                    const f32x4 h = ld4(Zt + row * LDZ + 4 * c4);
#pragma unroll
                    for (int i = 0; i < 4; ++i) o[i] = (h[i] - mean) * rstd * ga[it][i] + be[it][i];
                    stx4_wt(yln_ + (size_t)R * COUT + 4 * c4, o);
                }
                st4(Zt + row * LDZ + 4 * c4, o);
            }
            __syncthreads();
            f32x4 acc1[TM][1];
#pragma unroll
            for (int i = 0; i < TM; ++i) acc1[i][0] = zero4();
            pre_mma<TM, 1, 8, ET>(acc1, Zt, LDZ, 0, 8, w1);
#pragma unroll
            for (int i = 0; i < TM; ++i)
#pragma unroll
                for (int r = 0; r < 4; ++r) Zt[(i * 16 + 4 * g + r) * LDZ + COUT + wave * 16 + l15] = acc1[i][0][r];
            __syncthreads();
            ET* const hd_ = et_ptr<ET>(f.hd);
#pragma unroll
            for (int it = 0; it < NIT; ++it) {
                const int row = (tid + it * THREADS) / C4N;
                const long R = row0 + row;
                f32x4 h = ld4(Zt + row * LDZ + COUT + 4 * c4);
#pragma unroll
                for (int i = 0; i < 4; ++i) h[i] = fmaxf(h[i] + b1[i], 0.f);
                if (f.training) {
                    const f32x4 k = dropout_scale4((uint64_t)R * C4N + c4, f.seed, off, f.thresh, f.keep_scale);
#pragma unroll
                    for (int i = 0; i < 4; ++i) h[i] *= k[i];
                }
                float pd = h[0] * w2[0] + h[1] * w2[1] + h[2] * w2[2] + h[3] * w2[3];
#pragma unroll
                for (int m = 16; m >= 1; m >>= 1) pd += __shfl_xor(pd, m);
                if (R < rows) {
                    stx4_wt(hd_ + (size_t)R * COUT + 4 * c4, h);
                    if (c4 == 0) f.out[R] = pd + b2 + poison;
                }
            }
            chain_exit(f.chain);
        }
    }
}
template <int TM, int KC, bool PLAIN, typename ET>
__global__ __launch_bounds__(512) void tconv_fwd4_kernel(Tconv4Args aa) {
    tconv_fwd4_body<TM, KC, PLAIN, ET, false>(aa, nullptr);
}
template <int TM, int KC, typename ET>
__global__ __launch_bounds__(512) void head_fwd_kernel(Tconv4Args aa, HeadFcTail ht) {
    tconv_fwd4_body<TM, KC, false, ET, true>(aa, &ht);
}

struct GconvFwdArgs {
    const float* A;
    const float* Lp;
    const float* W;
    const float* bias;
    float* Xk;
    float* G;
    int N, NP, Ks, kipf;
    int parts;
    long slabs;
    float* XT;
};

__host__ __device__ inline int gc_np32(int N) { return (N + 31) / 32 * 32; }
inline size_t gconv_fwd_b16p_lds_bytes(int NP, int N) { return (size_t)16 * (NP + 4) * 4 + (size_t)16 * (gc_np32(N) + 8) * 2; }
__host__ __device__ inline size_t gc_plane_floats(int NP, int N) { return (size_t)(NP / 16) * (gc_np32(N) / 32) * 64 * 4; }
template <int MAXQ, int MAXW, typename ET, int SP, bool B16P = false>
__device__ __forceinline__ void gconv_fwd_body(const GconvFwdArgs& a, const int bid, const int THREADS) {
    static_assert(!B16P || (sizeof(ET) == 2 && SP == 1), "the bf16-plane products are the bf16-activation form, one slab per workgroup");
    typedef Mma<ET> MM;
    extern __shared__ float stgcn_smem[];
    const int tid = threadIdx.x, lane = tid & 63, g = lane >> 4, l15 = lane & 15;
    const int P = a.parts, part = (int)((unsigned)bid % (unsigned)P);
    const long slab0 = (long)((unsigned)bid / (unsigned)P) * SP;
    const int wave = part + P * __builtin_amdgcn_readfirstlane(tid >> 6), WAVES = P * (THREADS >> 6);
    const int N = a.N, NP = a.NP, LDX = NP + 4, HT = NP >> 4, KCH = NP >> 4;
    const size_t MSZ = (size_t)NP * NP;
    float* const XT0 = stgcn_smem;
    const int NP32 = gc_np32(N), KC32 = NP32 >> 5, LDB = NP32 + 8;
    unsigned short* const XH = reinterpret_cast<unsigned short*>(XT0 + SP * 16 * LDX);

    STGCN_PHASE(4, 0);
    ET* const Xk_ = et_ptr<ET>(a.Xk);
    ET* const G_ = et_ptr<ET>(a.G);
    bool live[SP];
#pragma unroll
    for (int j = 0; j < SP; ++j) {
        live[j] = slab0 + j < a.slabs;
        const ET* Asl = et_ptr<ET>(a.A) + (size_t)(live[j] ? slab0 + j : slab0) * N * 16;
        for (int idx0 = tid; idx0 < NP * 4; idx0 += 4 * THREADS) {
            Raw4<ET> rw[4];
#pragma unroll
            for (int u = 0; u < 4; ++u) {
                const int idx = idx0 + u * THREADS, n = idx >> 2, c4 = idx & 3;
                const int eo = (n < N ? n : N - 1) * 16 + c4 * 4;
                rw[u] = ldraw4(Asl + eo);
            }
#pragma unroll
            for (int u = 0; u < 4; ++u) {
                const int idx = idx0 + u * THREADS, n = idx >> 2, c4 = idx & 3;
                if (idx < NP * 4) {
                    const f32x4 v = n < N ? cvt4(rw[u]) : zero4();
#pragma unroll
                    for (int i = 0; i < 4; ++i) XT0[(j * 16 + c4 * 4 + i) * LDX + n] = v[i];
                    if constexpr (B16P) {
#pragma unroll
                        for (int i = 0; i < 4; ++i) {
                            const float vi = v[i];
                            XH[(c4 * 4 + i) * LDB + n] = (unsigned short)(__builtin_bit_cast(unsigned, vi) >> 16);
                        }
                    }
                }
            }
        }
    }
    if constexpr (B16P) {
        for (int idx = tid; idx < 16 * (LDB - NP); idx += THREADS) XH[(idx / (LDB - NP)) * LDB + NP + idx % (LDB - NP)] = 0;
    }
    __syncthreads();
    STGCN_PHASE(4, 1);

    f32x4 yacc[MAXQ][SP], res[MAXQ][SP];
#pragma unroll
    for (int q = 0; q < MAXQ; ++q) {
        const int ht = wave + WAVES * q;
#pragma unroll
        for (int j = 0; j < SP; ++j) {
            yacc[q][j] = zero4();
            res[q][j] = ht < HT ? ld4(XT0 + (j * 16 + l15) * LDX + ht * 16 + 4 * g) : zero4();
        }
    }
// ... 267 lines not shown
```

### stgcn_amd/csrc/stgcn_kernels_head.hip.h

```cpp
#pragma once
#include "stgcn_kernels_fwd.hip.h"

namespace stgcn {

struct FcFwdArgs {
    TapSrc ts;
    LnFwdArgs ln;
    const float* W1p;
    const float* b1;
    const float* w2;
    const float* b2;
    float* hd;
    float* out;
    int KCH, c1, training;
    float keep_scale;
    uint32_t thresh;
    uint64_t seed, offset;
    const uint64_t* offset_dev;
};

template <int WM, typename ET>
__global__ __launch_bounds__(256) void fc_fwd_kernel(FcFwdArgs a) {
    constexpr int TR = WM * 16, NT = 2;
    extern __shared__ float stgcn_smem[];
// ... 22 lines not shown
                const f32x4 ga = ld4(a.ln.gamma + (size_t)n * C + 4 * c4), be = ld4(a.ln.beta + (size_t)n * C + 4 * c4);
                f32x4 o;
#pragma unroll
                for (int i = 0; i < 4; ++i) o[i] = (gate_fwd(u[i], sg[i], a.ln.act) - mean) * rstd * ga[i] + be[i];
                st4(At + row * lda0 + 4 * c4, o);
                stx4_wt(et_ptr<ET>(a.ln.y) + (size_t)R * C + 4 * c4, o);
            }
        }
        for (int idx = threadIdx.x; idx < TR * c4n0; idx += kThreads) {
            const int row = idx / c4n0, c4 = idx - row * c4n0;
            if (row0 + row >= rows) st4(At + row * lda0 + 4 * c4, zero4());
        }
    } else {
        stage_tile_fwd<TR, 4, kThreads, ET>(a.ts, row0, KP, At, KP + 4);
    }
    __syncthreads();
    f32x4 acc[WM][NT];
#pragma unroll
    for (int i = 0; i < WM; ++i)
#pragma unroll
        for (int j = 0; j < NT; ++j) acc[i][j] = zero4();
    pre_mma<WM, NT, 8, ET>(acc, At, KP + 4, 0, a.KCH, w);
    __syncthreads();
    const int c1 = a.c1, ldz = c1 + 4;
    float* Zt = At;
#pragma unroll
    for (int j = 0; j < NT; ++j) {
        const int col = (wave + 4 * j) * 16 + l15;
#pragma unroll
        for (int i = 0; i < WM; ++i)
#pragma unroll
            for (int r = 0; r < 4; ++r) Zt[(i * 16 + 4 * g + r) * ldz + col] = acc[i][j][r];
    }
    __syncthreads();
    const uint64_t off = a.offset + (a.offset_dev ? *a.offset_dev : 0);
    const int c4n = c1 >> 2, c4sh = pow2_shift(c4n);
    const float b2 = a.b2 ? a.b2[0] : 0.f;
    for (int idx = threadIdx.x; idx < TR * c4n; idx += kThreads) {
        const int row = fast_div(idx, c4n, c4sh), c4 = idx - row * c4n;
        const long R = row0 + row;
        f32x4 h = ld4(Zt + row * ldz + 4 * c4);
        const f32x4 w2 = ld4(a.w2 + 4 * c4);
        if (a.b1) {
            const f32x4 b1 = ld4(a.b1 + 4 * c4);
#pragma unroll
            for (int i = 0; i < 4; ++i) h[i] += b1[i];
        }
#pragma unroll
        for (int i = 0; i < 4; ++i) h[i] = fmaxf(h[i], 0.f);
        if (a.training) {
            const f32x4 k = dropout_scale4((uint64_t)R * c4n + c4, a.seed, off, a.thresh, a.keep_scale);
#pragma unroll
            for (int i = 0; i < 4; ++i) h[i] *= k[i];
        }
        float p = h[0] * w2[0] + h[1] * w2[1] + h[2] * w2[2] + h[3] * w2[3];
#pragma unroll
        for (int m = 16; m >= 1; m >>= 1) p += __shfl_xor(p, m);
        if (R < a.ts.rows) {
            stx4_wt(et_ptr<ET>(a.hd) + (size_t)R * c1 + 4 * c4, h);
            if (c4 == 0) a.out[R] = p + b2;
        }
    }
}

struct FcBwdArgs {
    const float* dout;
    const float* hd;
    const float* w2;
    const float* W1d;
    float* dh1;
    float* dyln;
    float* part;
    long rows;
    int c0, c1, KCH;
    float grad_scale;
    const float* pred;
    const float* target;
    const long* target_index;
    long target_index_stride;
    const long* target_window;
    unsigned target_window_elems;
    float loss_scale;
    LnRowstatOut rs;
};

__device__ __forceinline__ const float* label_ptr(const float* y, const long* tab, long stride, unsigned per_w, long e) {
    if (!tab) return y + e;
    const unsigned eu = (unsigned)e, b = eu / per_w;
    return y + tab[b] * stride + (eu - b * per_w);
}

template <int WM, int NT, typename ET>
__global__ __launch_bounds__(256) void fc_bwd_kernel(FcBwdArgs a) {
    constexpr int TR = WM * 16;
    extern __shared__ float stgcn_smem[];
    const int tid = threadIdx.x, wave = tid >> 6, lane = tid & 63, g = lane >> 4, l15 = lane & 15;
    const int c1 = a.c1, c0 = a.c0, lda = c1 + 4, c4n = c1 >> 2;
    float* At = stgcn_smem;
    float* red = stgcn_smem + TR * lda;
    const long tiles = (a.rows + TR - 1) / TR;
    const int c4 = tid % c4n, rsub = tid / c4n;
    f32x4 dw2 = zero4();
    float db2 = 0.f, lsum = 0.f;
    const f32x4 w2 = ld4(a.w2 + 4 * c4);
    const float* tgt = a.target;
    const long* ttab = nullptr;
    if (a.pred && a.target_window) ttab = a.target_window + *a.target_index;
    else if (a.pred && a.target_index) tgt += *a.target_index * a.target_index_stride;
    const float inv_n = 1.0f / (float)a.rows;
    PreW<NT, 8> w;
    pre_load_weights<NT, 8>(w, a.W1d, a.KCH, wave, 4);
    for (long t = blockIdx.x; t < tiles; t += gridDim.x) {
        const long row0 = t * TR;
        __syncthreads();
        for (int row = rsub; row < TR; row += kThreads / c4n) {
            const long R = row0 + row;
            f32x4 d = zero4();
            if (R < a.rows) {
                float go;
                if (a.pred) {
                    const float df = a.pred[R] - *label_ptr(tgt, ttab, a.target_index_stride, a.target_window_elems, R);
                    go = 2.0f * df * inv_n * a.loss_scale;
                    if (c4 == 0) lsum += df * df;
                } else {
                    go = a.dout[R];
                }
                const f32x4 h = ldx4(et_ptr<ET>(a.hd) + (size_t)R * c1 + 4 * c4);
#pragma unroll
                for (int i = 0; i < 4; ++i) {
                    d[i] = h[i] != 0.f ? go * w2[i] * a.grad_scale : 0.f;
                    dw2[i] += go * h[i];
                }
                if (c4 == 0) db2 += go;
                stx4_wt(et_ptr<ET>(a.dh1) + (size_t)R * c1 + 4 * c4, d);
            }
            st4(At + row * lda + 4 * c4, d);
        }
        __syncthreads();
        f32x4 acc[WM][NT];
#pragma unroll
        for (int i = 0; i < WM; ++i)
#pragma unroll
            for (int j = 0; j < NT; ++j) acc[i][j] = zero4();
        pre_mma<WM, NT, 8, ET>(acc, At, lda, 0, a.KCH, w);
        if (a.rs.rowstat && c0 == c1) {
            __syncthreads();
#pragma unroll
            for (int j = 0; j < NT; ++j) {
                const int col = (wave + 4 * j) * 16 + l15;
#pragma unroll
                for (int i = 0; i < WM; ++i)
#pragma unroll
                    for (int r = 0; r < 4; ++r) At[(i * 16 + 4 * g + r) * lda + col] = acc[i][j][r];
            }
            __syncthreads();
            const uint64_t hoff = ln_rowstat_offset(a.rs);
            for (int row = rsub; row < TR; row += kThreads / c4n) {
                const long R = row0 + row;
                const bool rin = R < a.rows;
                const f32x4 v = et_round4<ET>(ld4(At + row * lda + 4 * c4));
                if (rin) stx4_wt(et_ptr<ET>(a.dyln) + (size_t)R * c0 + 4 * c4, v);
                const long slab = rin ? R / a.rs.N : 0;
                const int node = rin ? (int)(R - slab * a.rs.N) : 0;
                float2 p = rin ? ln_rowstat4<ET>(a.rs, hoff, v, slab, node, 4 * c4) : make_float2(0.f, 0.f);
                for (int m = c4n >> 1; m >= 1; m >>= 1) {
                    p.x += __shfl_xor(p.x, m);
                    p.y += __shfl_xor(p.y, m);
                }
                if (rin && c4 == 0) a.rs.rowstat[R] = p;
            }
        } else {
#pragma unroll
            for (int j = 0; j < NT; ++j) {
                const int col = (wave + 4 * j) * 16 + l15;
#pragma unroll
                for (int i = 0; i < WM; ++i)
#pragma unroll
                    for (int r = 0; r < 4; ++r) {
                        const long R = row0 + i * 16 + 4 * g + r;
                        if (R < a.rows && col < c0) stx1(et_ptr<ET>(a.dyln) + (size_t)R * c0 + col, acc[i][j][r]);
                    }
            }
        }
    }
    __syncthreads();
    st4(red + rsub * c1 + 4 * c4, dw2);
    if (c4 == 0) {
        red[8 * c1 + rsub] = db2;
        red[8 * c1 + 8 + rsub] = lsum;
    }
    __syncthreads();
    float* part = a.part + (size_t)blockIdx.x * (c1 + 2);
    if (tid < c1) {
        float s = 0.f;
        for (int k = 0; k < kThreads / c4n; ++k) s += red[k * c1 + tid];
        part[tid] = s;
    }
    if (tid == 0) {
        float s = 0.f;
        for (int k = 0; k < kThreads / c4n; ++k) s += red[8 * c1 + k];
        part[c1] = s;
        float l = 0.f;
        for (int k = 0; k < kThreads / c4n; ++k) l += red[8 * c1 + 8 + k];
        part[c1 + 1] = l * inv_n;
    }
}

struct AdamwTensor {
    float* p;
    const float* g;
    float* m;
    float* v;
    long n;
};
constexpr int kAdamwMaxTensors = 48;
constexpr int kAdamwChunk = 512;
struct AdamwArgs {
    AdamwTensor t[kAdamwMaxTensors];
    int start[kAdamwMaxTensors + 1];
    int count;
    float lr, b1, b2, eps, wd;
    float lb1, lb2;
    long step;
    const long* step_dev;
    const float* lr_dev;
};

__global__ __launch_bounds__(256) void adamw_kernel(AdamwArgs a) {
    int jb = 0;
    while (jb + 1 < a.count && (int)blockIdx.x >= a.start[jb + 1]) ++jb;
    const AdamwTensor& T = a.t[jb];
    const long base = ((long)blockIdx.x - a.start[jb]) * kAdamwChunk;
    const float t = (float)(a.step_dev ? *a.step_dev : a.step);
    const float lr = a.lr_dev ? *a.lr_dev : a.lr;
    const float bc1 = -expm1f(t * a.lb1);
    const float rs2 = rsqrtf(-expm1f(t * a.lb2));
    const float decay = 1.0f - lr * a.wd, step_size = lr / bc1;
#pragma unroll
    for (int k = 0; k < kAdamwChunk / kThreads; ++k) {
        const long e = base + k * kThreads + threadIdx.x;
        if (e < T.n) {
            const float g = T.g[e];
            const float m = a.b1 * T.m[e] + (1.0f - a.b1) * g;
            const float v = a.b2 * T.v[e] + (1.0f - a.b2) * g * g;
            T.m[e] = m;
            T.v[e] = v;
            T.p[e] = T.p[e] * decay - step_size * (m / (sqrtf(v) * rs2 + a.eps));
        }
    }
}

template <int KIND>
__global__ __launch_bounds__(256) void optim_kernel(AdamwArgs a, OptimExtra x) {
    int jb = 0;
    while (jb + 1 < a.count && (int)blockIdx.x >= a.start[jb + 1]) ++jb;
    const AdamwTensor& T = a.t[jb];
    const long base = ((long)blockIdx.x - a.start[jb]) * kAdamwChunk;
    const float t = (float)(a.step_dev ? *a.step_dev : a.step);
    const OptimScalars s = optim_scalars<KIND>(t, a.lr_dev ? *a.lr_dev : a.lr, a.b1, a.lb2, a.wd, x);
#pragma unroll
    for (int k = 0; k < kAdamwChunk / kThreads; ++k) {
        const long e = base + k * kThreads + threadIdx.x;
        if (e < T.n) {
            float p = T.p[e], m = T.m[e];
            if (KIND == kOptNadamw) {
                float v = T.v[e];
                nadamw_element(T.g[e], p, m, v, a.b2, a.eps, s, x);
// ... 147 lines not shown
```

### stgcn_amd/ops.py

```python
from __future__ import annotations

import ctypes as C
import os
from dataclasses import dataclass
from typing import Dict, Optional, Tuple

import torch

from . import _lib
from ._lib import (HEAD_PARAM_FIELDS, PARAM_FIELDS, AdamwHyper, AdamwTensor, FlushBlock, OutblockDesc, OutblockGrads, OutblockParams, OutblockPlan, StblockDesc,
                   StblockGrads, StblockParams, StblockPlan)


@dataclass(frozen=True)
class BlockConfig:
    Kt: int
    Ks: int
    n_vertex: int
    c_in: int
    channels: Tuple[int, int, int]
    act_func: str
    graph_conv_type: str
    droprate: float
    ln_eps: float = 1e-12
    tag: int = 0


def _stream_of(t: torch.Tensor) -> Optional[int]:
    if t.is_cuda:
        return torch.cuda.current_stream(t.device).cuda_stream
    return None


ACT_DTYPES = {torch.float32: _lib.DTYPE_F32, torch.bfloat16: _lib.DTYPE_BF16}


def _check_device(t: torch.Tensor, what: str, activation: bool = False):
    L = _lib.lib()
    if activation:
        if t.dtype not in ACT_DTYPES:
            raise TypeError(f"{what}: expected float32 or bfloat16 activations, got {t.dtype}")
    elif t.dtype != torch.float32:
        raise TypeError(f"{what}: expected float32, got {t.dtype}")
    if L.is_emulator:
        if t.is_cuda:
            raise RuntimeError(f"{what}: the bound library is the CPU emulator but the tensor is on {t.device}")
    elif not t.is_cuda:
        raise RuntimeError(f"{what}: stgcn_amd runs on MI355X only (tensor is on {t.device}); there is no CPU fallback")


_input_index: Dict[int, Tuple[torch.Tensor, int, Optional[torch.Tensor]]] = {}


def bind_input_index(base: torch.Tensor, index: torch.Tensor, stride_floats: int, table: Optional[torch.Tensor] = None) -> None:
    assert index.dtype == torch.int64 and index.numel() == 1 and index.device == base.device
    if table is not None:
        if table.dtype != torch.int64 or table.dim() != 1 or not table.is_contiguous() or table.device != base.device:
            raise ValueError("bind_input_index: table must be a contiguous 1-D int64 tensor on the device of base")
    _input_index[base.data_ptr()] = (index, int(stride_floats), table)


def unbind_input_index(base: torch.Tensor) -> None:
    _input_index.pop(base.data_ptr(), None)


def _index_of(t: torch.Tensor):
    e = _input_index.get(t.data_ptr())
    return (None, 0, None) if e is None else (e[0].data_ptr(), e[1], None if e[2] is None else e[2].data_ptr())


def window_strided_rows(x_p: torch.Tensor) -> Optional[int]:
    B, T, N, Cc = x_p.shape
    sb, st, sn, sc = x_p.stride()
    inner = (Cc == 1 or sc == 1) and sn == Cc and st == N * Cc
    if B > 1 and inner and sb >= 0 and sb % Cc == 0 and sb != T * N * Cc:
        return sb // Cc
    return None


def make_desc(cfg: BlockConfig, B: int, T: int, training: bool, need_dx: bool, prepacked: bool = False, defer: bool = False,
              x_bstride: int = 0, x_index: Optional[int] = None, x_index_stride: int = 0, dtype: torch.dtype = torch.float32,
              x_window: Optional[int] = None) -> StblockDesc:
    if cfg.act_func not in _lib.ACT:
        raise NotImplementedError(f"ERROR: The activation function {cfg.act_func} is not implemented.")
# ... 125 lines not shown

def graph_terms(cfg: "BlockConfig") -> int:
    return int(cfg.Ks) if cfg.graph_conv_type == "cheb_graph_conv" else 2


def _optr(t: Optional[torch.Tensor]):
    return None if t is None else t.data_ptr()


def dropout_mask(n: int, droprate: float, seed: int, offset: int, device, offset_dev: Optional[torch.Tensor] = None) -> torch.Tensor:
    L = _lib.lib()
    out = torch.empty(n, dtype=torch.float32, device=device)
    L.check(L.dll.stgcn_dropout_mask(out.data_ptr(), n, float(droprate), seed, offset, _optr(offset_dev), _stream_of(out)),
            "stgcn_dropout_mask")
    return out


def mse_loss_and_grad(pred: torch.Tensor, target: torch.Tensor, grad_scale: float = 1.0) -> Tuple[torch.Tensor, torch.Tensor]:
    L = _lib.lib()
    p = pred.detach()
    _check_device(p, "pred")
    if p.shape != target.shape or not p.is_contiguous() or not target.is_contiguous() or target.dtype != torch.float32:
        raise ValueError(f"mse_loss_and_grad: contiguous float32 tensors of one shape expected, got {tuple(p.shape)} / {tuple(target.shape)}")
    loss = torch.empty(1, dtype=torch.float32, device=p.device)
    dpred = torch.empty_like(p)
    ti, tis, tw = _index_of(target)
    if tw is not None:
        L.check(L.dll.stgcn_mse_loss_grad_windows(p.data_ptr(), target.data_ptr(), p.numel(), float(grad_scale), loss.data_ptr(),
                                                  dpred.data_ptr(), ti, tis, tw, p.numel() // p.shape[0], _stream_of(p)),
                "stgcn_mse_loss_grad_windows")
        return loss, dpred
    L.check(L.dll.stgcn_mse_loss_grad(p.data_ptr(), target.data_ptr(), p.numel(), float(grad_scale), loss.data_ptr(), dpred.data_ptr(),
                                      ti, tis, _stream_of(p)), "stgcn_mse_loss_grad")
    return loss, dpred


EVAL_STATE_WORDS, EVAL_POS_WORDS = _lib.EVAL_STATE_WORDS, _lib.EVAL_POS_WORDS


def eval_state(device) -> Tuple[torch.Tensor, torch.Tensor]:
    return (torch.zeros(EVAL_STATE_WORDS, dtype=torch.float64, device=device), torch.zeros(EVAL_POS_WORDS, dtype=torch.int64, device=device))


def eval_arm(state: torch.Tensor, pos: Optional[torch.Tensor] = None) -> None:
    L = _lib.lib()
    _check_eval_state(L, state, pos)
    L.check(L.dll.stgcn_eval_arm(state.data_ptr(), _optr(pos), _stream_of(state)), "stgcn_eval_arm")


def _check_eval_state(L, state: torch.Tensor, pos: Optional[torch.Tensor]) -> None:
    if state.dtype != torch.float64 or state.numel() < EVAL_STATE_WORDS or not state.is_contiguous():
        raise ValueError(f"evaluation state: {EVAL_STATE_WORDS} contiguous float64 words expected, got {state.numel()} x {state.dtype}")
    if pos is not None and (pos.dtype != torch.int64 or pos.numel() < EVAL_POS_WORDS or not pos.is_contiguous() or pos.device != state.device):
        raise ValueError(f"evaluation position: {EVAL_POS_WORDS} contiguous int64 words on the state's device expected")
    if L.is_emulator == state.is_cuda:
        raise RuntimeError(f"evaluation state is on {state.device}, the bound library is {L.backend}")


def eval_accumulate(pred: torch.Tensor, target: torch.Tensor, state: torch.Tensor, scale: Optional[torch.Tensor] = None,
                    mean: Optional[torch.Tensor] = None, first_valid: int = 0, pos: Optional[torch.Tensor] = None, num_windows: int = 0,
                    target_stride: Optional[int] = None) -> None:
    L = _lib.lib()
    p = pred.detach()
    _check_device(p, "pred")
    _check_eval_state(L, state, pos)
    if p.dim() != 2 or not p.is_contiguous() or target.dtype != torch.float32 or not target.is_contiguous() or target.shape != p.shape:
        raise ValueError(f"eval_accumulate: contiguous float32 (B, N) tensors expected, got {tuple(p.shape)} / {tuple(target.shape)}")
    B, N = p.shape
    for t, what in ((scale, "scale"), (mean, "mean")):
        if t is not None and (t.dtype != torch.float32 or t.numel() != N or not t.is_contiguous() or t.device != p.device):
            raise ValueError(f"eval_accumulate: {what} must be {N} contiguous float32 values on {p.device}")
    L.check(L.dll.stgcn_eval_accumulate(p.data_ptr(), target.data_ptr(), B, N, _optr(scale), _optr(mean), int(first_valid), _optr(pos),
                                        N if target_stride is None else int(target_stride), int(num_windows), state.data_ptr(),
                                        _stream_of(p)), "stgcn_eval_accumulate")


def eval_metrics(words) -> dict:
    import math
    sse, sad, ssd, sy, n = (float(w) for w in words[:5])
    return {"mse": sse / n, "mae": sad / n, "rmse": math.sqrt(ssd / n), "wmape": sad / sy, "elements": int(n)}


class _PendingLoss:
    __slots__ = ("placeholder", "pred", "target", "index", "index_stride", "window", "grad_scale", "loss")


_pending_loss: Optional[_PendingLoss] = None
_VIEW_NODES = ("ViewBackward", "UnsafeViewBackward", "ReshapeAliasBackward", "UnsqueezeBackward", "SqueezeBackward", "AliasBackward")


def _head_node_of(pred: torch.Tensor):
    fn = pred.grad_fn
    while fn is not None and type(fn).__name__.startswith(_VIEW_NODES):
        nxt = [f for f, _ in fn.next_functions if f is not None]
        if len(nxt) != 1:
            return None
        fn = nxt[0]
    return fn if fn is not None and type(fn).__name__ == "_OutBlockFnBackward" else None


def mse_backward(pred: torch.Tensor, target: torch.Tensor, grad_scale: float = 1.0) -> torch.Tensor:
    global _pending_loss
    p = pred.detach()
    if (_head_node_of(pred) is None or not p.is_contiguous() or p.shape != target.shape or not target.is_contiguous()
            or target.dtype != torch.float32 or os.environ.get("STGCN_FUSED_LOSS", "1") == "0"):
        loss, dpred = mse_loss_and_grad(pred, target, grad_scale)
        pred.backward(dpred)
        return loss
    _check_device(p, "pred")
    pl = _PendingLoss()
    pl.placeholder = torch.empty_like(p)
    pl.pred, pl.target, pl.grad_scale = p, target, float(grad_scale)
    pl.index, pl.index_stride, pl.window = _index_of(target)
    pl.loss = torch.empty(1, dtype=torch.float32, device=p.device)
    _pending_loss = pl
    try:
        pred.backward(pl.placeholder)
        if _pending_loss is not None:
            raise RuntimeError("mse_backward: the output head did not take the fused loss (was its backward run through another path?)")
    finally:
        _pending_loss = None
    return pl.loss


class GradSink:

    def __init__(self, grads: Dict[torch.nn.Parameter, torch.Tensor]):
        self.by_ptr = {p.data_ptr(): g for p, g in grads.items()}
        self.blocks = []
        self.head = None
        self.owners = []

    def holds(self, wsc) -> bool:
        return any(o is wsc for o in self.owners)

    def grad_for(self, p: Optional[torch.Tensor]) -> Optional[torch.Tensor]:
        return None if p is None else self.by_ptr.get(p.data_ptr())

    def flush(self, opt_table=None, hyper: Optional[AdamwHyper | _lib.OptimHyper] = None, stream: Optional[int] = None) -> None:
        L = _lib.lib()
        arr = (FlushBlock * max(len(self.blocks), 1))()
        for i, (desc, gst, ws, _) in enumerate(self.blocks):
            arr[i].desc, arr[i].grads, arr[i].ws = C.pointer(desc), C.pointer(gst), ws.data_ptr()
        hd = hg = hws = None
        if self.head is not None:
            hd, hg, hws = C.byref(self.head[0]), C.byref(self.head[1]), self.head[2].data_ptr()
        n_opt = 0 if opt_table is None else len(opt_table)
        if isinstance(hyper, _lib.OptimHyper):
            L.check(L.dll.stgcn_grad_flush_optim(len(self.blocks), arr, hd, hg, hws, opt_table, n_opt, C.byref(hyper), stream),
                    "stgcn_grad_flush_optim")
        else:
            L.check(L.dll.stgcn_grad_flush(len(self.blocks), arr, hd, hg, hws, opt_table, n_opt, None if hyper is None else C.byref(hyper), stream),
                    "stgcn_grad_flush")
        self.blocks, self.head = [], None
        for o in self.owners:
            o.pending_sink = None
        self.owners = []


_sink: Optional[GradSink] = None


class grad_sink_scope:
    def __init__(self, sink: Optional[GradSink]):
        self.sink = sink

    def __enter__(self):
        global _sink
        self.prev, _sink = _sink, self.sink
        return self.sink

    def __exit__(self, *exc):
        global _sink
        _sink = self.prev
        return False


_chain = 0


def current_chain() -> int:
    return _chain


class chain_scope:

    def __init__(self, c: int):
        self.c = int(c)

    def __enter__(self):
        global _chain
        self.prev, _chain = _chain, self.c
        return self

    def __exit__(self, *exc):
        global _chain
        _chain = self.prev
        return False


class WorkspaceCache:

    def __init__(self):
        self.bufs: Dict[int, torch.Tensor] = {}
        self.prepacked = False
        self.pending_sink = None

    @property
    def buf(self) -> Optional[torch.Tensor]:
        return self.bufs.get(0)

    def take_prepacked(self) -> bool:
        p, self.prepacked = self.prepacked, False
        return p

    def get(self, n_floats: int, device) -> torch.Tensor:
        if self.pending_sink is not None and self.pending_sink.holds(self):
            raise RuntimeError("this module's gradient partials are still waiting in an active GradSink: call sink.flush() before the module "
                               "runs again (one forward/backward per module per flush)")
        b = self.bufs.get(_chain)
        if b is None or b.numel() < n_floats or b.device != device:
            nb = torch.empty(max(n_floats, 1), dtype=torch.float32, device=device)
            if b is not None and b.device == device:
                nb[:b.numel()].copy_(b)
            b = self.bufs[_chain] = nb
        return b


class LnHookState:
    __slots__ = ("hook", "keep", "ready", "dx_ptr", "dx_version", "y_ptr")

    def __init__(self, hook, keep):
        self.hook, self.keep, self.ready, self.dx_ptr, self.dx_version, self.y_ptr = hook, keep, False, None, -1, None

    def mark_ready(self, dx: torch.Tensor) -> None:
        self.ready, self.dx_ptr, self.dx_version = True, dx.data_ptr(), dx._version

    def matches(self, dy: torch.Tensor) -> bool:
        return self.ready and self.dx_ptr == dy.data_ptr() and self.dx_version == dy._version


_ln_hooks: "Dict[int, tuple]" = {}
_offer_hook_next = False


def _offer_ln_hook(y: torch.Tensor, state: LnHookState) -> None:
    while len(_ln_hooks) >= 8:
        _ln_hooks.pop(next(iter(_ln_hooks)))
    state.y_ptr = y.data_ptr()
    _ln_hooks[state.y_ptr] = (state, y)


def _retire_ln_hook(state: Optional[LnHookState]) -> None:
    if state is not None and state.y_ptr is not None:
        e = _ln_hooks.get(state.y_ptr)
        if e is not None and e[0] is state:
            del _ln_hooks[state.y_ptr]


def clear_ln_hooks() -> None:
    _ln_hooks.clear()


def _take_ln_hook(x_cl: torch.Tensor) -> Optional[LnHookState]:
    e = _ln_hooks.pop(x_cl.data_ptr(), None)
    if e is None:
        return None
    state, y = e
    if tuple(y.shape) != tuple(x_cl.shape) or y.stride() != x_cl.stride():
        return None
    return state


def _param_struct(cls, tensors):
    s = cls()
    for name, t in zip(PARAM_FIELDS, tensors):
        setattr(s, name, None if t is None else t.data_ptr())
    return s


class _STBlockFn(torch.autograd.Function):

    @staticmethod
    def forward(ctx, x_cl, gso_pad, gso_t_pad, cfg: BlockConfig, training: bool, seed: int, offset: int, offset_dev,
                wsc: WorkspaceCache, *params):
        L = _lib.lib()
        B, T, N, c_in = x_cl.shape
        need_dx = bool(x_cl.requires_grad)
        bstride = 0 if x_cl.is_contiguous() else window_strided_rows(x_cl)
# ... 97 lines not shown
    _offer_hook_next = torch.is_grad_enabled() and (x.requires_grad or any(p is not None and p.requires_grad for p in params))
    y_cl = _STBlockFn.apply(x_cl, gso_pad, gso_t_pad, cfg, training, seed, offset, offset_dev, wsc, *params)
    return y_cl.permute(0, 3, 1, 2)


def prepack_modules(blocks, head, B: int, device, counters=None, dtype: torch.dtype = torch.float32, park: bool = False) -> None:
    L = _lib.lib()
    arr = (_lib.PrepackBlock * max(len(blocks), 1))()
    keep = []
    for i, (cfg, T, params, wsc) in enumerate(blocks):
        desc = make_desc(cfg, B, T, True, True, dtype=dtype)
        plan = query_plan(desc)
        ps = [None if p is None else p.detach() for p in params]
        pst = _param_struct(StblockParams, ps)
        ws = wsc.get(plan.ws_floats, device)
        keep += [desc, pst, ps, ws]
        arr[i].desc = C.pointer(desc)
        arr[i].params = C.pointer(pst)
        arr[i].ws = ws.data_ptr()
    hd = hp = hws = None
    if head is not None:
        cfg, T, params, wsc = head
        hdesc = make_head_desc(cfg, B, T, True, True, dtype=dtype)
        hplan = query_head_plan(hdesc)
        hps = [None if p is None else p.detach() for p in params]
        hpst = _head_struct(OutblockParams, hps)
        hws_t = wsc.get(hplan.ws_floats, device)
        keep += [hdesc, hpst, hps, hws_t]
        hd, hp, hws = C.byref(hdesc), C.byref(hpst), hws_t.data_ptr()
    stream = torch.cuda.current_stream(device).cuda_stream if torch.device(device).type == "cuda" else None
    carr = None
    if counters:
        carr = (_lib.StepCounter * len(counters))()
        for i, (t, inc, mod) in enumerate(counters):
            assert t.dtype == torch.int64 and t.numel() == 1
            carr[i].ptr, carr[i].inc, carr[i].mod = t.data_ptr(), int(inc), int(mod)
    fn = L.dll.stgcn_prepack_park if park else L.dll.stgcn_prepack
    L.check(fn(len(blocks), arr, hd, hp, hws, 0 if carr is None else len(counters), carr, stream), "stgcn_prepack")
    for _, _, _, wsc in blocks:
        wsc.prepacked = True
    if head is not None:
        head[3].prepacked = True


@dataclass(frozen=True)
class HeadConfig:
    Ko: int
    n_vertex: int
    c_in: int
    channels: Tuple[int, int]
    end_channel: int
    act_func: str
    droprate: float
    ln_eps: float = 1e-12


def head_supported(cfg: HeadConfig) -> bool:
    return (cfg.channels[0] in (64, 128) and cfg.channels[1] == 128 and cfg.end_channel == 1 and cfg.act_func in _lib.ACT
            and (cfg.c_in % 4 == 0 or cfg.Ko * cfg.c_in <= 16))


def make_head_desc(cfg: HeadConfig, B: int, T: int, training: bool, need_dx: bool, prepacked: bool = False, defer: bool = False,
                   dtype: torch.dtype = torch.float32) -> OutblockDesc:
    if cfg.act_func not in _lib.ACT:
        raise NotImplementedError(f"ERROR: The activation function {cfg.act_func} is not implemented.")
    d = OutblockDesc()
    d.B, d.T, d.N, d.c_in = B, T, cfg.n_vertex, cfg.c_in
    d.c0, d.c1 = cfg.channels
    d.c_end, d.Ko = cfg.end_channel, cfg.Ko
    d.act = _lib.ACT[cfg.act_func]
    d.training = 1 if training else 0
    d.droprate, d.ln_eps = float(cfg.droprate), float(cfg.ln_eps)
    d.need_dx = 1 if need_dx else 0
    d.prepacked = 1 if prepacked else 0
    d.defer_reduce = 1 if defer else 0
    d.dtype = ACT_DTYPES[dtype]
    return d


_head_plan_cache: Dict[tuple, OutblockPlan] = {}


def query_head_plan(desc: OutblockDesc) -> OutblockPlan:
    key = tuple(getattr(desc, f) for f, _ in OutblockDesc._fields_) + (os.environ.get("STGCN_HEAD_FC_TILE"),)
    p = _head_plan_cache.get(key)
    if p is None:
        L = _lib.lib()
        p = OutblockPlan()
        L.check(L.dll.stgcn_outblock_plan_query(C.byref(desc), C.byref(p)), "stgcn_outblock_plan_query")
        _head_plan_cache[key] = p
    return p


def _head_struct(cls, tensors):
    s = cls()
    for name, t in zip(HEAD_PARAM_FIELDS, tensors):
        setattr(s, name, None if t is None else t.data_ptr())
    return s


class _OutBlockFn(torch.autograd.Function):

    @staticmethod
    def forward(ctx, x_cl, cfg: HeadConfig, training: bool, seed: int, offset: int, offset_dev, wsc: WorkspaceCache, *params):
        L = _lib.lib()
        B, T, N, c_in = x_cl.shape
        need_dx = bool(x_cl.requires_grad)
        desc = make_head_desc(cfg, B, T, training, need_dx, prepacked=wsc.take_prepacked(), dtype=x_cl.dtype)
        plan = query_head_plan(desc)
        dev = x_cl.device
        ps = [None if p is None else p.detach() for p in params]
        out = torch.empty(B, plan.T1, N, dtype=torch.float32, device=dev)
        saved = torch.empty(plan.saved_floats, dtype=torch.float32, device=dev)
        ws = wsc.get(plan.ws_floats, dev)
        pst = _head_struct(OutblockParams, ps)
        L.check(L.dll.stgcn_outblock_forward(C.byref(desc), C.byref(pst), x_cl.data_ptr(), out.data_ptr(), saved.data_ptr(), ws.data_ptr(),
                                             seed, offset, _optr(offset_dev), _stream_of(x_cl)), "stgcn_outblock_forward")
        ctx.in_hook = _take_ln_hook(x_cl) if need_dx else None
        ctx.save_for_backward(x_cl, saved, *[p for p in params if p is not None])
        ctx.param_present = [p is not None for p in params]
        ctx.param_needs_grad = [p is not None and p.requires_grad for p in params]
        ctx.cfg, ctx.training, ctx.ws, ctx.need_dx, ctx.wsc = cfg, training, ws, need_dx, wsc
        return out

    @staticmethod
    def backward(ctx, dout):
        L = _lib.lib()
        x_cl, saved, *present = ctx.saved_tensors
        it = iter(present)
        params = [next(it) if pr else None for pr in ctx.param_present]
        cfg = ctx.cfg
        B, T, N, c_in = x_cl.shape
        sink = _sink
        desc = make_head_desc(cfg, B, T, ctx.training, ctx.need_dx, defer=sink is not None, dtype=x_cl.dtype)
        dout = dout.contiguous()
        if dout.dtype != torch.float32:
            dout = dout.float()
        global _pending_loss
        fused_loss = _pending_loss if (_pending_loss is not None and _pending_loss.placeholder.data_ptr() == dout.data_ptr()) else None
        if fused_loss is not None:
            _pending_loss = None
        used = {"tc_aw": c_in > cfg.channels[0], "tc_ab": c_in > cfg.channels[0]}
        grads = []
        for name, p, need in zip(HEAD_PARAM_FIELDS, params, ctx.param_needs_grad):
            if not (p is not None and need and used.get(name, True)):
                grads.append(None)
            elif sink is not None:
                grads.append(sink.grad_for(p))
                if grads[-1] is None:
                    raise RuntimeError(f"gradient sink has no buffer for head parameter {name}")
            else:
                grads.append(torch.empty_like(p))
        dx = torch.empty_like(x_cl) if ctx.need_dx else None
        pst = _head_struct(OutblockParams, [None if p is None else p.detach() for p in params])
        gst = _head_struct(OutblockGrads, grads)
        ih = ctx.in_hook if dx is not None else None
        if fused_loss is not None:
            gst.loss = fused_loss.loss.data_ptr()
            hl = _lib.HeadLoss()
            hl.pred, hl.target = fused_loss.pred.data_ptr(), fused_loss.target.data_ptr()
            hl.target_index_dev, hl.target_index_stride, hl.grad_scale = fused_loss.index, fused_loss.index_stride, fused_loss.grad_scale
            hl.target_window_dev = fused_loss.window
            ctx.keep_loss = fused_loss
            L.check(L.dll.stgcn_outblock_backward_loss(C.byref(desc), C.byref(pst), x_cl.data_ptr(), C.byref(hl), saved.data_ptr(),
                                                       ctx.ws.data_ptr(), C.byref(gst), None if dx is None else dx.data_ptr(),
                                                       None if ih is None else C.byref(ih.hook), _stream_of(x_cl)),
                    "stgcn_outblock_backward_loss")
        else:
            L.check(L.dll.stgcn_outblock_backward_hook(C.byref(desc), C.byref(pst), x_cl.data_ptr(), dout.data_ptr(), saved.data_ptr(),
                                                       ctx.ws.data_ptr(), C.byref(gst), None if dx is None else dx.data_ptr(),
                                                       None if ih is None else C.byref(ih.hook), _stream_of(x_cl)),
                    "stgcn_outblock_backward")
        if ih is not None:
            ih.mark_ready(dx)
        if sink is not None:
            sink.head = (desc, gst, ctx.ws, (grads, params))
            sink.owners.append(ctx.wsc)
            ctx.wsc.pending_sink = sink
            grads = [None] * len(grads)
        return (dx, None, None, None, None, None, None, *grads)


def block_chain_status(cfg: BlockConfig, B: int, T: int, wsc: WorkspaceCache, dtype=torch.float32) -> int:
    L = _lib.lib()
    ws = wsc.buf
    if ws is None:
        return 0
    desc = make_desc(cfg, B, T, False, False, dtype=dtype)
    w = C.c_uint32(0)
    L.check(L.dll.stgcn_stblock_chain_status(C.byref(desc), ws.data_ptr(), C.byref(w), _stream_of(ws)), "stgcn_stblock_chain_status")
    return int(w.value)


def head_chain_status(cfg: HeadConfig, B: int, T: int, wsc: WorkspaceCache, dtype=torch.float32) -> int:
    L = _lib.lib()
    ws = wsc.buf
    if ws is None:
        return 0
    desc = make_head_desc(cfg, B, T, False, False, dtype=dtype)
    w = C.c_uint32(0)
    L.check(L.dll.stgcn_outblock_chain_status(C.byref(desc), ws.data_ptr(), C.byref(w), _stream_of(ws)), "stgcn_outblock_chain_status")
    return int(w.value)


def output_block(x: torch.Tensor, cfg: HeadConfig, params, training: bool, seed: int, offset: int, wsc: WorkspaceCache,
                 offset_dev: Optional[torch.Tensor] = None) -> torch.Tensor:
    _check_device(x, "x", activation=True)
    if x.dim() != 4 or x.shape[1] != cfg.c_in or x.shape[3] != cfg.n_vertex:
        raise ValueError(f"expected input (B, {cfg.c_in}, T, {cfg.n_vertex}), got {tuple(x.shape)}")
    x_cl = x.permute(0, 2, 3, 1).contiguous()
    out = _OutBlockFn.apply(x_cl, cfg, training, seed, offset, offset_dev, wsc, *params)
    return out.unsqueeze(1)
```

### stgcn_amd/train.py

```python
from __future__ import annotations

import os
from typing import List, Optional, Tuple

import torch
import torch.distributed as dist


def dist_env():
    rank = int(os.environ.get("RANK", "0"))
    local_rank = int(os.environ.get("LOCAL_RANK", "0"))
    world = int(os.environ.get("WORLD_SIZE", "1"))
    return rank, local_rank, world


def init_distributed(backend: Optional[str] = None):
    rank, local_rank, world = dist_env()
    if backend is None:
        backend = "nccl" if torch.cuda.is_available() else "gloo"
    if backend == "nccl":
        torch.cuda.set_device(local_rank)
    if world > 1 and not dist.is_initialized():
        os.environ.setdefault("MASTER_ADDR", "127.0.0.1")
        os.environ.setdefault("MASTER_PORT", "29500")
# ... 54 lines not shown
        "for _ in range(3):\n"
        "    t.fill_(float(r + 1)); g.replay()\n"
        "torch.cuda.synchronize()\n"
        "want = sum(range(1, w + 1)) / w\n"
        "assert abs(float(t[0]) - want) < 1e-6 and abs(float(t[-1]) - want) < 1e-6, (float(t[0]), want)\n"
        "dist.destroy_process_group()\n"
        "print('CAPTURE_OK')\n")
    env = capture_child_env(env)
    ok, why = False, ""
    try:
        p = subprocess.run([sys.executable, "-c", code], env=env, capture_output=True, text=True, timeout=timeout_s)
        ok = p.returncode == 0 and "CAPTURE_OK" in p.stdout
        why = "" if ok else ("probe failed: " + (p.stderr.strip().splitlines() or ["rc %d" % p.returncode])[-1][:200])
    except subprocess.TimeoutExpired:
        why = f"probe hung for {timeout_s:.0f} s (killed)"
    except Exception as e:
        why = "probe could not run: " + repr(e)[:200]
    return ok, why


def sync_operators(model, src: int = 0) -> None:
    if not (dist.is_available() and dist.is_initialized()) or dist.get_world_size() <= 1:
        return
    from .layers import STConvBlock
    seen = {}
    for m in model.modules():
        if isinstance(m, STConvBlock) and torch.is_tensor(m.gso):
            g = seen.get(id(m.gso))
            if g is None:
                home = m.gso.device
                comm_dev = torch.device("cuda", torch.cuda.current_device()) if dist.get_backend() == "nccl" else torch.device("cpu")
                t = m.gso.detach().to(comm_dev, copy=True).contiguous()
                dist.broadcast(t, src=src)
                g = t.to(home)
                seen[id(m.gso)] = g
            m.gso = g
            m.graph_conv.gso = g
            gc = getattr(m.graph_conv, "cheb_graph_conv", None) or getattr(m.graph_conv, "graph_conv", None)
            if gc is not None:
                gc.gso = g
            m._gso_cache = None


class FlatGradAllReduce:

    def __init__(self, params: List[torch.nn.Parameter], world: int):
        self.params = list(params)
        self.world = world
        self.flat: Optional[torch.Tensor] = None
        self.live: Optional[List[torch.nn.Parameter]] = None

    def __call__(self):
        if self.world <= 1:
            return
        live = [p for p in self.params if p.grad is not None]
        if self.live is None or len(live) != len(self.live):
            self.live = live
            n = sum(p.numel() for p in live)
            self.flat = torch.empty(n, dtype=torch.float32, device=live[0].device)
        grads = [p.grad.reshape(-1) for p in live]
        torch.cat(grads, out=self.flat)
        dist.all_reduce(self.flat, op=dist.ReduceOp.SUM)
        self.flat.mul_(1.0 / self.world)
        torch._foreach_copy_([p.grad.reshape(-1) for p in live], list(self.flat.split([p.numel() for p in live])))


def make_optimizer(model: torch.nn.Module, lr: float = 1e-3, weight_decay: float = 1e-3, name: str = "adamw",
                   capturable: bool = False):
    params = list(model.parameters())
    if name == "adamw":
        from .optim import AdamW
        return AdamW(params, lr=lr, weight_decay=weight_decay, capturable=capturable)
    if name == "nadamw":
        from .optim import NAdamW
        return NAdamW(params, lr=lr, weight_decay=weight_decay, capturable=capturable)
    if name == "lion":
        from .optim import Lion
        return Lion(params, lr=lr, weight_decay=weight_decay, capturable=capturable)
    raise ValueError(f"ERROR: The {name} optimizer is undefined.")


def fwd_loss_bwd(model, x, y):
    from . import ops
    y_pred = model(x).reshape(len(x), -1)
    return ops.mse_backward(y_pred, y)[0]


def check_in_launch_waits(model) -> None:
    from .layers import OutputBlock, STConvBlock
    for name, m in model.named_modules():
        if isinstance(m, (STConvBlock, OutputBlock)):
            w = m.chain_status()
            if w:
                what = "(b, t) slab" if isinstance(m, STConvBlock) else "window"
                raise RuntimeError(f"{name or type(m).__name__}: an in-launch wait of the last forward gave up on {what} {w - 1} -- its outputs are NaN "
                                   f"(the device was not this launch's alone for stgcn_set_chain_spin_ticks; the next weight pack re-arms the words)")


def fused_tail_supported(model, live_params) -> bool:
    from . import ops
    from .layers import OutputBlock, STConvBlock
    owned = set()
    for m in model.modules():
        if isinstance(m, STConvBlock) or (isinstance(m, OutputBlock) and ops.head_supported(m.cfg)):
            owned.update(id(p) for p in m.parameters())
    return all(id(p) in owned for p in live_params)


class GradArena:

    def __init__(self, live_params: List[torch.nn.Parameter]):
        from . import ops
        self.params = list(live_params)
        dev = self.params[0].device
        self.flat = torch.zeros(sum(p.numel() for p in self.params), dtype=torch.float32, device=dev)
        self.grads = {}
        off = 0
        for p in self.params:
            self.grads[p] = self.flat[off:off + p.numel()].view_as(p)
            off += p.numel()
        self.sink = ops.GradSink(self.grads)

    def install(self):
        for p, g in self.grads.items():
            p.grad = g


def fused_train_step(model, optimizer, x, y, arena: GradArena, world: int = 1, all_reduce=None):
    from . import ops
    if not fused_tail_supported(model, arena.params):
        raise RuntimeError("fused_train_step: the model has live parameters outside the fused operators (see fused_tail_supported); "
                           "use train_step")
    arena.install()
    with ops.grad_sink_scope(arena.sink):
        y_pred = model(x).reshape(len(x), -1)
        loss = ops.mse_backward(y_pred, y, grad_scale=1.0 / world)
    if world <= 1 and hasattr(optimizer, "flush_with"):
        optimizer.flush_with(arena.sink, arena.grads)
    else:
        arena.sink.flush(stream=torch.cuda.current_stream(x.device).cuda_stream if x.is_cuda else None)
        if world > 1 and all_reduce is not None:
            all_reduce(arena.flat)
        optimizer.step()
    return loss[0]


def train_step(model, optimizer, x, y, allreduce: Optional[FlatGradAllReduce] = None):
    from .layers import DropoutStream
    optimizer.zero_grad(set_to_none=True)
    loss = fwd_loss_bwd(model, x, y)
    if allreduce is not None:
        allreduce()
    optimizer.step()
    DropoutStream.advance()
    return loss.detach()


def tail_step(model, optimizer, x, y, world: int = 1, rank: int = 0):
    from . import ops
    from .layers import DropoutStream
    n = len(x)
    per = (n + world - 1) // world
    lo, hi = min(rank * per, n), min(rank * per + per, n)
    optimizer.zero_grad(set_to_none=True)
    dev = x.device
    loss_sum = torch.zeros(1, dtype=torch.float32, device=dev)
    folded = getattr(model, "_step_counters", None)
    if folded is not None:
        model._step_counters = None
    try:
        if hi > lo:
            pred = model(x[lo:hi]).reshape(hi - lo, -1)
            loss = ops.mse_backward(pred, y[lo:hi].contiguous(), grad_scale=(hi - lo) / n)
            loss_sum = loss * ((hi - lo) / n)
    finally:
        if folded is not None:
            model._step_counters = folded
    if world > 1:
        params = [p for p in model.parameters() if p.requires_grad]
        live = torch.tensor([1.0 if p.grad is not None else 0.0 for p in params], device=dev)
        dist.all_reduce(live, op=dist.ReduceOp.MAX)
        keep = [p for p, l in zip(params, live.tolist()) if l > 0]
        flat = torch.cat([(p.grad if p.grad is not None else torch.zeros_like(p)).reshape(-1) for p in keep])
        dist.all_reduce(flat, op=dist.ReduceOp.SUM)
        for p, g in zip(keep, flat.split([p.numel() for p in keep])):
            p.grad = g.view_as(p).clone()
        dist.all_reduce(loss_sum, op=dist.ReduceOp.SUM)
    if getattr(optimizer, "trainer_owns_step", False) and hasattr(optimizer, "device_step_counter"):
        optimizer.device_step_counter(dev).add_(1)
    optimizer.step()
    DropoutStream.advance()
    return loss_sum[0].detach()


def chained_fwd_bwd(model, x, y, chains: int, streams=None):
    from contextlib import nullcontext
    from . import ops
    params = [p for p in model.parameters() if p.requires_grad]
    B = len(x)
    assert chains >= 1 and B % chains == 0, f"batch {B} does not split into {chains} chains"
    Bc = B // chains
    use_streams = streams is not None and x.is_cuda and chains > 1
    main = torch.cuda.current_stream(x.device) if use_streams else None
    losses, grads = [], []
    for c in range(chains):
        s = streams[c] if (use_streams and c > 0) else None
        if s is not None:
            s.wait_stream(main)
        with (torch.cuda.stream(s) if s is not None else nullcontext()), ops.chain_scope(c):
            xc, yc = x[c * Bc:(c + 1) * Bc], y[c * Bc:(c + 1) * Bc]
            pred = model(xc).reshape(Bc, -1)
            loss = torch.nn.functional.mse_loss(pred, yc) * (1.0 / chains)
            grads.append(torch.autograd.grad(loss, params, allow_unused=True))
            losses.append(loss.detach())
    if use_streams:
        for c in range(1, chains):
            main.wait_stream(streams[c])
    live = [i for i, g in enumerate(grads[0]) if g is not None]
    acc = [grads[0][i] for i in live]
    for c in range(1, chains):
        torch._foreach_add_(acc, [grads[c][i] for i in live])
    for i, g in zip(live, acc):
        params[i].grad = g
    total = losses[0]
    for l in losses[1:]:
        total = total + l
    return total


class WindowOrder:

    def __init__(self, num: int, usable: int, device, seed: int = 0):
        self.num, self.usable = int(num), int(usable)
        assert 0 < self.usable <= self.num
        self.order = torch.arange(self.usable, dtype=torch.int64, device=device)
        self.generator = torch.Generator(device="cpu")
        self.generator.manual_seed(int(seed))

    def set_order(self, starts) -> None:
        import numpy as np
        if isinstance(starts, torch.Tensor):
            if starts.dtype != torch.int64:
                raise ValueError(f"set_order: int64 window starts expected, got {starts.dtype}")
            host = starts.detach().to("cpu").reshape(-1) if starts.dim() == 1 else None
        else:
            arr = np.asarray(starts)
            if arr.dtype != np.int64:
                raise ValueError(f"set_order: int64 window starts expected, got {arr.dtype}")
            host = torch.from_numpy(np.ascontiguousarray(arr)) if arr.ndim == 1 else None
        if host is None or host.numel() != self.usable:
            raise ValueError(f"set_order: {self.usable} window starts expected (one per window of the whole global minibatches), got "
                             f"{'a non 1-D value' if host is None else host.numel()}")
        lo, hi = int(host.min()), int(host.max())
        if lo < 0 or hi > self.num - 1:
            raise ValueError(f"set_order: window starts must lie in [0, {self.num - 1}], got [{lo}, {hi}]")
        self.order.copy_(host, non_blocking=False)
# ... 86 lines not shown
                            DropoutStream.advance()
                            self._advance_series()
                else:
                    self.opt.flush_with(self.arena.sink, self.arena.grads, bump_step=not self.fold)
                    if not self.fold:
                        DropoutStream.advance()
                        self._advance_series()
            else:
                self.loss = self._fwd_bwd()
                if world > 1:
                    self.live = [p for p in model.parameters() if p.grad is not None]
                    self.flat = torch.cat([p.grad.reshape(-1) for p in self.live])
                    if self.capture_collective:
                        dist.all_reduce(self.flat, op=dist.ReduceOp.SUM)
                        self.flat.mul_(1.0 / world)
                        torch._foreach_copy_([p.grad.reshape(-1) for p in self.live], list(self.flat.split([p.numel() for p in self.live])))
                        self.opt.step()
                        DropoutStream.advance()
                        self._advance_series()
                else:
                    self.opt.step()
                    DropoutStream.advance()
                    self._advance_series()
        self.g2 = None
        if world > 1 and not self.capture_collective:
            self.g2 = torch.cuda.CUDAGraph()
            with torch.cuda.graph(self.g2, pool=self.g1.pool(), **cap):
                if not self.fused:
                    self.flat.mul_(1.0 / world)
                    torch._foreach_copy_([p.grad.reshape(-1) for p in self.live], list(self.flat.split([p.numel() for p in self.live])))
                self.opt.step()
                if not self.fold:
                    DropoutStream.advance()
                    self._advance_series()
        self(x_example, y_example)
        torch.cuda.synchronize(dev)

    @property
    def order(self) -> Optional[torch.Tensor]:
        return None if self._order is None else self._order.order

    def set_order(self, starts) -> None:
        if self._order is None:
            raise RuntimeError("set_order: this step was built without shuffle=True (no window table is bound)")
        self._order.set_order(starts)

    def reshuffle(self) -> None:
        if self._order is None:
            raise RuntimeError("reshuffle: this step was built without shuffle=True (no window table is bound)")
        self._order.reshuffle()

    def check(self) -> None:
        check_in_launch_waits(self.model)

    def close(self):
        from . import ops
        from .layers import DropoutStream
        if getattr(self.model, "_step_counters", None) is not None:
            self.model._step_counters = None
        if self.series is not None:
            ops.unbind_input_index(self.x)
            ops.unbind_input_index(self.y)
        if DropoutStream.counter is self.counter:
            DropoutStream.disable_device_counter()
        if hasattr(self.opt, "trainer_owns_step"):
            self.opt.trainer_owns_step = False

    def __enter__(self):
        return self

    def __exit__(self, *exc):
        self.close()
        return False

    def _fwd_bwd(self):
        if self.chains > 1:
            return chained_fwd_bwd(self.model, self.x, self.y, self.chains, self.streams)
        return fwd_loss_bwd(self.model, self.x, self.y)

    def _fused_fwd_bwd(self):
        from . import ops
        self.arena.install()
        with ops.grad_sink_scope(self.arena.sink):
            y_pred = self.model(self.x).reshape(len(self.x), -1)
            loss = ops.mse_backward(y_pred, self.y, grad_scale=1.0 / self.world)
        if self.world > 1:
            self.arena.sink.flush(stream=torch.cuda.current_stream(self.x.device).cuda_stream)
        return loss[0]

    def _try_fold_counters(self, dev):
        from .layers import DropoutStream
        step_t = self.opt.device_step_counter(dev)
        self.model._step_counters = [(DropoutStream.counter, DropoutStream.SITE_STRIDE, 0), (step_t, 1, 0)]
        i0 = None
        if self._index_bump is not None:
            idx, inc, mod = self._index_bump
            i0 = int(idx.item())
            idx.sub_(inc).remainder_(mod)
            self.model._step_counters.append(self._index_bump)
        c0, s0 = int(DropoutStream.counter.item()), int(step_t.item())
        self.fold = True
        self.opt.trainer_owns_step = True
        self._eager_fused_once()
        if int(DropoutStream.counter.item()) != c0 + DropoutStream.SITE_STRIDE or int(step_t.item()) != s0 + 1:
            self.model._step_counters = None
            DropoutStream.counter.fill_(c0 + DropoutStream.SITE_STRIDE)
            step_t.fill_(s0 + 1)
            if i0 is not None:
                self._index_bump[0].fill_((i0 + self._index_bump[1]) % self._index_bump[2])
            self.fold = False
            self.opt.trainer_owns_step = False

    def _eager_fused_once(self):
        from .layers import DropoutStream
        self._fused_fwd_bwd()
        if self.world > 1:
            dist.all_reduce(self.arena.flat)
            self.opt.step()
            if not self.fold:
                DropoutStream.advance()
                self._advance_series()
        else:
            self.opt.flush_with(self.arena.sink, self.arena.grads, bump_step=not self.fold)
            if not self.fold:
                DropoutStream.advance()
                self._advance_series()

    def _eager_once(self):
        from .layers import DropoutStream
        self.opt.zero_grad(set_to_none=True)
        self._fwd_bwd()
        if self.world > 1:
            live = [p for p in self.model.parameters() if p.grad is not None]
            flat = torch.cat([p.grad.reshape(-1) for p in live])
            dist.all_reduce(flat)
            flat.mul_(1.0 / self.world)
            torch._foreach_copy_([p.grad.reshape(-1) for p in live], list(flat.split([p.numel() for p in live])))
        self.opt.step()
        DropoutStream.advance()
        self._advance_series()

    def _advance_series(self):
        if self._index_bump is not None and not self.fold:
            idx, inc, mod = self._index_bump
            idx.add_(inc).remainder_(mod)

    def __call__(self, x: Optional[torch.Tensor] = None, y: Optional[torch.Tensor] = None) -> torch.Tensor:
        if self.series is None:
            self.x.copy_(x, non_blocking=True)
            self.y.copy_(y, non_blocking=True)
        self.g1.replay()
        if self.g2 is not None:
            dist.all_reduce(self.flat, op=dist.ReduceOp.SUM)
            self.g2.replay()
        return self.loss


def _workspace_owners(model):
    from .layers import OutputBlock, STConvBlock
    return [(name or type(m).__name__, m) for name, m in model.named_modules() if isinstance(m, (STConvBlock, OutputBlock))]


class GraphedEvalPass:

    def __init__(self, model, series, n_his: int, n_pred: int, batch_size: int, scaler=None, capture: bool = True):
        import numpy as np
        from . import _lib, ops
# ... 133 lines not shown
```

Before: 90170 windows/s.

## Fuse MSE loss and fc backward tail into the one-launch head forward kernel

Adds a head forward variant that takes the training targets and computes the MSE loss, the output gradient and the fc2 backward partials (dh1, per-16-row reduction parts) inside the same one-launch forward kernel. The head backward then skips the separate fc backward launch when the loss was formed in the forward. It is enabled by default through a loss scope in the training paths, falling back when the plan has no single-round forward. The change removes one kernel launch and a re-read of saved activations per step, at the cost of a larger forward kernel (occupancy is checked against the plain kernel) and more per-block partials to reduce.

```diff
diff --git a/include/stgcn_hip.h b/include/stgcn_hip.h
--- a/include/stgcn_hip.h
+++ b/include/stgcn_hip.h
@@ -6,7 +6,7 @@
 extern "C" {
 #endif
 
-#define STGCN_ABI_VERSION 9
+#define STGCN_ABI_VERSION 10
 
 #define STGCN_OK 0
 #define STGCN_ERR_UNSUPPORTED 1
@@ -164,6 +164,8 @@
     int32_t dtype;
     int32_t prepacked;
     int32_t defer_reduce;
+    int32_t loss_in_forward;
+    int32_t reserved;
 } stgcn_outblock_desc;
 
 typedef struct stgcn_outblock_params {
@@ -197,11 +199,15 @@
     int64_t ws_rowstat_b, ws_dh1, ws_dyln, ws_dZ, ws_part, part_floats;
     int64_t ws_chain;
     int64_t chain_words;
+    int64_t fwd_loss_ok;
 } stgcn_outblock_plan;
 
 int stgcn_outblock_plan_query(const stgcn_outblock_desc* desc, stgcn_outblock_plan* plan);
 int stgcn_outblock_forward(const stgcn_outblock_desc* desc, const stgcn_outblock_params* params, const float* x, float* out,
                            float* saved, float* ws, uint64_t seed, uint64_t offset, const uint64_t* offset_dev, void* stream);
+int stgcn_outblock_forward_loss(const stgcn_outblock_desc* desc, const stgcn_outblock_params* params, const float* x, float* out,
+                                float* saved, float* ws, const stgcn_head_loss* loss, uint64_t seed, uint64_t offset,
+                                const uint64_t* offset_dev, void* stream);
 int stgcn_outblock_chain_status(const stgcn_outblock_desc* desc, const float* ws, uint32_t* sticky, void* stream);
 int64_t stgcn_set_chain_spin_ticks(int64_t ticks);
 int stgcn_outblock_backward(const stgcn_outblock_desc* desc, const stgcn_outblock_params* params, const float* x,
diff --git a/stgcn_amd/_lib.py b/stgcn_amd/_lib.py
--- a/stgcn_amd/_lib.py
+++ b/stgcn_amd/_lib.py
@@ -8,7 +8,7 @@
 DEFAULT_LIB = os.path.join(_HERE, "libstgcn_hip.so")
 
 STGCN_OK = 0
-ABI_VERSION = 9
+ABI_VERSION = 10
 ACT = {"glu": 0, "gtu": 1}
 GRAPH_CONV = {"cheb_graph_conv": 0, "graph_conv": 1}
 DTYPE_F32, DTYPE_BF16 = 0, 1
@@ -60,7 +60,7 @@
     _fields_ = [("B", C.c_int32), ("T", C.c_int32), ("N", C.c_int32), ("c_in", C.c_int32), ("c0", C.c_int32), ("c1", C.c_int32),
                 ("c_end", C.c_int32), ("Ko", C.c_int32), ("act", C.c_int32), ("training", C.c_int32), ("droprate", C.c_float),
                 ("ln_eps", C.c_float), ("need_dx", C.c_int32), ("dtype", C.c_int32), ("prepacked", C.c_int32),
-                ("defer_reduce", C.c_int32)]
+                ("defer_reduce", C.c_int32), ("loss_in_forward", C.c_int32), ("reserved", C.c_int32)]
 
 
 HEAD_PARAM_FIELDS = ["tc_w", "tc_b", "tc_aw", "tc_ab", "ln_w", "ln_b", "fc1_w", "fc1_b", "fc2_w", "fc2_b"]
@@ -85,7 +85,7 @@
 
 HEAD_PLAN_FIELDS = ["T1", "rows", "rows_in", "out_floats", "saved_floats", "ws_floats", "sv_U", "sv_S", "sv_mean", "sv_rstd", "sv_yln",
                     "sv_hd", "sv_rowstat", "ws_Wp", "ws_Wd", "ws_b", "ws_W1p", "ws_W1d", "ws_rowstat_b", "ws_dh1", "ws_dyln", "ws_dZ", "ws_part",
-                    "part_floats", "ws_chain", "chain_words"]
+                    "part_floats", "ws_chain", "chain_words", "fwd_loss_ok"]
 
 
 class OutblockPlan(C.Structure):
@@ -188,6 +188,9 @@
         d.stgcn_outblock_plan_query.argtypes = [C.POINTER(OutblockDesc), C.POINTER(OutblockPlan)]
         d.stgcn_outblock_forward.argtypes = [C.POINTER(OutblockDesc), C.POINTER(OutblockParams), C.c_void_p, C.c_void_p, C.c_void_p,
                                              C.c_void_p, C.c_uint64, C.c_uint64, C.c_void_p, C.c_void_p]
+        d.stgcn_outblock_forward_loss.argtypes = [C.POINTER(OutblockDesc), C.POINTER(OutblockParams), C.c_void_p, C.c_void_p, C.c_void_p,
+                                                  C.c_void_p, C.POINTER(HeadLoss), C.c_uint64, C.c_uint64, C.c_void_p, C.c_void_p]
+        d.stgcn_outblock_forward_loss.restype = C.c_int
         d.stgcn_outblock_backward.argtypes = [C.POINTER(OutblockDesc), C.POINTER(OutblockParams), C.c_void_p, C.c_void_p, C.c_void_p,
                                               C.c_void_p, C.POINTER(OutblockGrads), C.c_void_p, C.c_void_p]
         for f in ("stgcn_outblock_plan_query", "stgcn_outblock_forward", "stgcn_outblock_backward"):
@@ -266,4 +269,4 @@
                     "stgcn_stblock_ln_hook", "stgcn_stblock_backward_hook", "stgcn_outblock_backward_hook", "stgcn_set_tc1_bwd_wgs",
                     "stgcn_set_slab_gc_precision", "stgcn_outblock_backward_loss", "stgcn_set_bwd_precision", "stgcn_set_gemm_big_nt",
                     "stgcn_set_chain_spin_ticks", "stgcn_outblock_chain_status", "stgcn_set_tc2ln_peers", "stgcn_stblock_chain_status", "stgcn_prepack_park", "stgcn_prepack_flush",
-                    "stgcn_optim_step", "stgcn_grad_flush_optim", "stgcn_eval_arm", "stgcn_eval_accumulate"]
+                    "stgcn_optim_step", "stgcn_grad_flush_optim", "stgcn_eval_arm", "stgcn_eval_accumulate", "stgcn_outblock_forward_loss"]
diff --git a/stgcn_amd/csrc/stgcn_capi_head.inc b/stgcn_amd/csrc/stgcn_capi_head.inc
--- a/stgcn_amd/csrc/stgcn_capi_head.inc
+++ b/stgcn_amd/csrc/stgcn_capi_head.inc
@@ -1,6 +1,8 @@
 
 struct HeadGeom {
     int T1, NC, KP, KCH, CPin, ln_spg, ln_sg, fc_wgs;
+    int fwd_tm, fwd_ticket;
+    int fc_parts;
     int dense_bwd;
     int fused_ln_bwd;
     int64_t rows, rows_in, slabs;
@@ -20,6 +22,48 @@
     if ((d->c_in & 3) != 0 && d->Ko * d->c_in > 16) return fail(STGCN_ERR_UNSUPPORTED, "c_in=%d must be a multiple of 4", d->c_in);
     if (d->dtype != STGCN_DTYPE_F32 && d->dtype != STGCN_DTYPE_BF16) return fail(STGCN_ERR_INVALID, "dtype must be STGCN_DTYPE_F32 or STGCN_DTYPE_BF16");
     return STGCN_OK;
+}
+
+}
+struct HeadFwdForm { int tm, ticket, one_round; };
+template <bool LOSS>
+static HeadFwdForm head_fwd_form(const stgcn_outblock_desc* d, int KP, int64_t rows) {
+    constexpr int KC = 4;
+    HeadFwdForm r = {0, 0, 0};
+    const bool bf = d->dtype == STGCN_DTYPE_BF16;
+    const int forced = head_fuse_mode() > 1 ? head_fuse_mode() : 0;
+    const size_t l2 = (size_t)(tconv2_lds_floats(KP, 256, 32) + 48) * sizeof(float), l4 = (size_t)(tconv2_lds_floats(KP, 256, 64) + 48) * sizeof(float);
+    int cap2, cap4;
+    if constexpr (LOSS) {
+        cap2 = bf ? wg_capacity(head_fwd_loss_kernel<2, KC, bf16>, 512, l2) : wg_capacity(head_fwd_loss_kernel<2, KC, float>, 512, l2);
+        cap4 = bf ? wg_capacity(head_fwd_loss_kernel<4, KC, bf16>, 512, l4) : wg_capacity(head_fwd_loss_kernel<4, KC, float>, 512, l4);
+    } else {
+        cap2 = bf ? wg_capacity(head_fwd_kernel<2, KC, bf16>, 512, l2) : wg_capacity(head_fwd_kernel<2, KC, float>, 512, l2);
+        cap4 = bf ? wg_capacity(head_fwd_kernel<4, KC, bf16>, 512, l4) : wg_capacity(head_fwd_kernel<4, KC, float>, 512, l4);
+    }
+    const int t2 = cdiv(rows, 32), t4 = cdiv(rows, 64);
+    const bool tk2 = d->N >= 32 && d->N <= 1024 && cap2 >= 4 * cdiv(d->N, 32) + 16, tk4 = d->N >= 64 && d->N <= 2048 && cap4 >= 4 * cdiv(d->N, 64) + 16;
+    if (forced == 2) { if (d->N >= 32 && t2 <= cap2) r.tm = 2; }
+    else if (forced == 4) { if (d->N >= 64 && t4 <= cap4) r.tm = 4; }
+    else if (forced == 3) { if (tk2) { r.tm = 2; r.ticket = 1; } }
+    else if (forced == 5) { if (tk4) { r.tm = 4; r.ticket = 1; } }
+    else if (tk2 && t2 <= cap2) { r.tm = 2; r.ticket = 1; }
+    else if (tk4 && t4 <= cap4) { r.tm = 4; r.ticket = 1; }
+    else if (tk2) { r.tm = 2; r.ticket = 1; }
+    else if (tk4) { r.tm = 4; r.ticket = 1; }
+    r.one_round = r.tm == 2 ? t2 <= cap2 : r.tm == 4 ? t4 <= cap4 : 0;
+    return r;
+}
+extern "C" {
+static bool head_fwd_fusable(const stgcn_outblock_desc* d, int T1, int KP) {
+    TconvFwdArgs t;
+    memset(&t, 0, sizeof(t));
+    t.ts.C = d->c_in; t.ts.taps = d->Ko; t.KCH = KP / 16; t.Cout = d->c0;
+    return head_fuse_mode() && T1 == 1 && d->c0 == 128 && d->c1 == 128 && tconv4_ok(t);
+}
+static bool head_fwd_loss_enabled() {
+    static const int off = getenv("STGCN_HEAD_FWD_LOSS") ? atoi(getenv("STGCN_HEAD_FWD_LOSS")) == 0 : 0;
+    return !off;
 }
 
 static HeadGeom head_geom(const stgcn_outblock_desc* d) {
@@ -51,11 +95,19 @@
     if (g.fused_ln_bwd) { g.ln_spg = 1; g.ln_sg = (int)g.slabs; }
     const long tiles = (g.rows + head_fc_tile_rows() - 1) / head_fc_tile_rows();
     g.fc_wgs = (int)(tiles < 512 * 32 / head_fc_tile_rows() / 2 ? tiles : 512 * 32 / head_fc_tile_rows() / 2);
+    g.fwd_tm = g.fwd_ticket = 0;
+    long fc_blocks = g.fc_wgs;
+    if (head_fwd_loss_enabled() && (fuse_mask() & FUSE_ROWSTATS) && head_fwd_fusable(d, g.T1, g.KP) && d->N >= 32) {
+        const HeadFwdForm ff = head_fwd_form<true>(d, g.KP, g.rows), f0 = head_fwd_form<false>(d, g.KP, g.rows);
+        if (ff.one_round && ff.tm == f0.tm) { g.fwd_tm = ff.tm; g.fwd_ticket = ff.ticket; }
+    }
+    if (g.fwd_tm) fc_blocks = (g.rows + 15) / 16;
+    g.fc_parts = (int)fc_blocks;
     long o = 0;
     auto take = [&](long f) { long at = o; o += (f + 63) / 64 * 64; return at; };
     g.off_ln_g = take(sg_max * n);
     g.off_ln_b = take((d->dtype == STGCN_DTYPE_BF16 ? sg_max : sg_plain) * n);
-    g.off_fc = take((long)g.fc_wgs * (d->c1 + 2));
+    g.off_fc = take(fc_blocks * (d->c1 + 2));
     constexpr int t_conv = 160, t_fc = 96;
     const bool one_round = g.rows <= 32768;
     g.wc = wgrad_geom(g.rows, d->Ko * d->c_in, g.NC, 0, one_round ? t_conv : 256);
@@ -87,9 +139,9 @@
         L.add(G->fc1_w, wp, w.chunks, (long)w.Mpad * w.NC, 1, d->c1, d->c0, 0, w.Mpad, 1, 0, d->c0, 1);
         L.add_flat(G->fc1_b, bp, w.chunks, w.NC, d->c1);
     }
-    L.add_flat(G->fc2_w, part + g.off_fc, g.fc_wgs, d->c1 + 2, d->c1);
-    L.add_flat(G->fc2_b, part + g.off_fc + d->c1, g.fc_wgs, d->c1 + 2, 1);
-    if (G->loss) L.add_flat(G->loss, part + g.off_fc + d->c1 + 1, g.fc_wgs, d->c1 + 2, 1);
+    L.add_flat(G->fc2_w, part + g.off_fc, g.fc_parts, d->c1 + 2, d->c1);
+    L.add_flat(G->fc2_b, part + g.off_fc + d->c1, g.fc_parts, d->c1 + 2, 1);
+    if (G->loss) L.add_flat(G->loss, part + g.off_fc + d->c1 + 1, g.fc_parts, d->c1 + 2, 1);
     const int n = d->N * d->c0;
     L.add_flat(G->ln_w, part + g.off_ln_g, g.ln_sg, n, n);
     if (g.fused_ln_bwd && d->dtype == STGCN_DTYPE_F32) L.add_flat(G->ln_b, dyln, g.ln_sg, n, n);
@@ -101,7 +153,10 @@
     if (rc) return rc;
     if (!p) return fail(STGCN_ERR_INVALID, "plan is NULL");
     const HeadGeom g = head_geom(d);
+    if (d->loss_in_forward && !g.fwd_tm)
+        return fail(STGCN_ERR_UNSUPPORTED, "loss_in_forward: this head has no one-launch forward that can carry the loss tail (plan.fwd_loss_ok = 0)");
     memset(p, 0, sizeof(*p));
+    p->fwd_loss_ok = g.fwd_tm ? 1 : 0;
     p->T1 = g.T1; p->rows = g.rows; p->rows_in = g.rows_in; p->out_floats = g.rows * d->c_end;
     int64_t o = 0;
     auto take = [&](int64_t n) { int64_t at = o; o += rup(n, 64); return at; };
@@ -235,8 +290,30 @@
 }
 extern "C" {
 
+}
+namespace {
+int outblock_forward_impl(const stgcn_outblock_desc* d, const stgcn_outblock_params* P, const float* x, float* out, float* saved,
+                          float* ws, const stgcn_head_loss* hl, uint64_t seed, uint64_t offset, const uint64_t* offset_dev, void* stream);
+}
+extern "C" {
 int stgcn_outblock_forward(const stgcn_outblock_desc* d, const stgcn_outblock_params* P, const float* x, float* out, float* saved,
                            float* ws, uint64_t seed, uint64_t offset, const uint64_t* offset_dev, void* stream) {
+    if (d && d->loss_in_forward) return fail(STGCN_ERR_INVALID, "stgcn_outblock_forward: desc.loss_in_forward is set (stgcn_outblock_forward_loss takes the labels)");
+    return outblock_forward_impl(d, P, x, out, saved, ws, nullptr, seed, offset, offset_dev, stream);
+}
+int stgcn_outblock_forward_loss(const stgcn_outblock_desc* d, const stgcn_outblock_params* P, const float* x, float* out, float* saved,
+                                float* ws, const stgcn_head_loss* hl, uint64_t seed, uint64_t offset, const uint64_t* offset_dev,
+                                void* stream) {
+    if (!hl || !hl->target) return fail(STGCN_ERR_INVALID, "stgcn_outblock_forward_loss: NULL loss / target");
+    if (hl->target_window_dev && !hl->target_index_dev)
+        return fail(STGCN_ERR_INVALID, "stgcn_outblock_forward_loss: target_window_dev (window table) needs target_index_dev != NULL");
+    if (!d || !d->loss_in_forward) return fail(STGCN_ERR_INVALID, "stgcn_outblock_forward_loss: desc.loss_in_forward is not set");
+    return outblock_forward_impl(d, P, x, out, saved, ws, hl, seed, offset, offset_dev, stream);
+}
+}
+namespace {
+int outblock_forward_impl(const stgcn_outblock_desc* d, const stgcn_outblock_params* P, const float* x, float* out, float* saved,
+                          float* ws, const stgcn_head_loss* hl, uint64_t seed, uint64_t offset, const uint64_t* offset_dev, void* stream) {
     STGCN_FLUSH_PENDING_PACK();
     stgcn_outblock_plan pl;
     int rc = stgcn_outblock_plan_query(d, &pl);
@@ -263,25 +340,11 @@
     t.Wp = ws + pl.ws_Wp; t.bias = ws + pl.ws_b; t.KCH = g.KCH; t.Cout = d->c0; t.act = d->act;
     t.U = saved + pl.sv_U; t.S = saved + pl.sv_S; t.rowstat = reinterpret_cast<float2*>(saved + pl.sv_rowstat);
 
+    if (hl && !g.fwd_tm) return fail(STGCN_ERR_UNSUPPORTED, "stgcn_outblock_forward_loss: no one-launch forward for this head");
     if (head_fuse_mode() && g.T1 == 1 && d->c0 == 128 && d->c1 == 128 && tconv4_ok(t)) {
         constexpr int KC = 4;
-        int tm = 0, ticket = 0;
-        {
-            const int forced = head_fuse_mode() > 1 ? head_fuse_mode() : 0;
-            const size_t l2 = (size_t)(tconv2_lds_floats(g.KP, 256, 32) + 48) * sizeof(float), l4 = (size_t)(tconv2_lds_floats(g.KP, 256, 64) + 48) * sizeof(float);
-            const int cap2 = STGCN_ET_VALUE(wg_capacity(head_fwd_kernel<2, KC, ET>, 512, l2));
-            const int cap4 = STGCN_ET_VALUE(wg_capacity(head_fwd_kernel<4, KC, ET>, 512, l4));
-            const int t2 = cdiv(g.rows, 32), t4 = cdiv(g.rows, 64);
-            const bool tk2 = d->N >= 32 && d->N <= 1024 && cap2 >= 4 * cdiv(d->N, 32) + 16, tk4 = d->N >= 64 && d->N <= 2048 && cap4 >= 4 * cdiv(d->N, 64) + 16;
-            if (forced == 2) { if (d->N >= 32 && t2 <= cap2) tm = 2; }
-            else if (forced == 4) { if (d->N >= 64 && t4 <= cap4) tm = 4; }
-            else if (forced == 3) { if (tk2) { tm = 2; ticket = 1; } }
-            else if (forced == 5) { if (tk4) { tm = 4; ticket = 1; } }
-            else if (tk2 && t2 <= cap2) { tm = 2; ticket = 1; }
-            else if (tk4 && t4 <= cap4) { tm = 4; ticket = 1; }
-            else if (tk2) { tm = 2; ticket = 1; }
-            else if (tk4) { tm = 4; ticket = 1; }
-        }
+        const HeadFwdForm ff = hl ? HeadFwdForm{g.fwd_tm, g.fwd_ticket, 1} : head_fwd_form<false>(d, g.KP, g.rows);
+        const int tm = ff.tm, ticket = ff.ticket;
         if (tm) {
             Tconv4Args aa;
             memset(&aa, 0, sizeof(aa));
@@ -299,6 +362,18 @@
             f.offset_dev = offset_dev;
             f.use_ticket = ticket;
             const size_t lds = (size_t)(tconv2_lds_floats(g.KP, 256, TR) + 48) * sizeof(float);
+            if (hl) {
+                HeadLossTail lt;
+                memset(&lt, 0, sizeof(lt));
+                lt.target = hl->target; lt.target_index = reinterpret_cast<const long*>(hl->target_index_dev);
+                lt.target_index_stride = (long)hl->target_index_stride; lt.target_window = reinterpret_cast<const long*>(hl->target_window_dev);
+                lt.target_window_elems = (unsigned)(g.rows / d->B); lt.loss_scale = hl->grad_scale;
+                lt.W1d = ws + pl.ws_W1d; lt.dh1 = ws + pl.ws_dh1; lt.dyln = ws + pl.ws_dyln;
+                lt.rowstat_b = reinterpret_cast<float2*>(ws + pl.ws_rowstat_b); lt.part = ws + pl.ws_part + g.off_fc;
+                if (tm == 2) STGCN_LAUNCH_ET("head.fwd_loss", st, (head_fwd_loss_kernel<2, KC, ET>), dim3(tiles), dim3(512), lds, aa, f, lt);
+                else STGCN_LAUNCH_ET("head.fwd_loss", st, (head_fwd_loss_kernel<4, KC, ET>), dim3(tiles), dim3(512), lds, aa, f, lt);
+                return STGCN_OK;
+            }
             if (tm == 2) STGCN_LAUNCH_ET("head.fwd", st, (head_fwd_kernel<2, KC, ET>), dim3(tiles), dim3(512), lds, aa, f);
             else STGCN_LAUNCH_ET("head.fwd", st, (head_fwd_kernel<4, KC, ET>), dim3(tiles), dim3(512), lds, aa, f);
             return STGCN_OK;
@@ -334,7 +409,8 @@
     else STGCN_LAUNCH_ET("head.fc_fwd", st, (fc_fwd_kernel<2, ET>), dim3(cdiv(g.rows, 32)), dim3(kThreads), lds, f);
     return STGCN_OK;
 }
-
+}
+extern "C" {
 
 int stgcn_outblock_chain_status(const stgcn_outblock_desc* d, const float* ws, uint32_t* sticky, void* stream) {
     STGCN_FLUSH_PENDING_PACK();
@@ -400,8 +476,10 @@
     float* part = ws + pl.ws_part;
     const int training = d->training && d->droprate > 0.f;
     const bool own_rowstats = (fuse_mask() & FUSE_ROWSTATS) && d->c0 == d->c1 && d->c0 == 128;
-
-    {
+    if (d->loss_in_forward && !hl)
+        return fail(STGCN_ERR_INVALID, "stgcn_outblock_backward: desc.loss_in_forward is set (the gradient was formed from the loss in the forward): a dout cannot replace it");
+
+    if (!d->loss_in_forward) {
         FcBwdArgs a;
         memset(&a, 0, sizeof(a));
         a.dout = dout; a.hd = saved + pl.sv_hd; a.w2 = P->fc2_w; a.W1d = ws + pl.ws_W1d; a.dh1 = ws + pl.ws_dh1; a.dyln = ws + pl.ws_dyln;
@@ -417,7 +495,9 @@
             a.rs.mean = saved + pl.sv_mean; a.rs.rstd = saved + pl.sv_rstd; a.rs.N = d->N; a.rs.C = d->c0; a.rs.act = d->act; a.rs.training = 0;
             a.rs.keep_scale = 1.f;
         }
-        const size_t lds = (size_t)(head_fc_tile_rows() * (d->c1 + 4) + 8 * d->c1 + 16) * sizeof(float);
+        a.per_block = g.fwd_tm ? 1 : 0;
+        const int red_floats = a.per_block ? head_fc_tile_rows() * (d->c1 + 4) : 8 * d->c1 + 16;
+        const size_t lds = (size_t)(head_fc_tile_rows() * (d->c1 + 4) + red_floats) * sizeof(float);
         if (head_fc_tile_rows() == 16) {
             if (d->c0 == 128) STGCN_LAUNCH_ETB("head.fc_bwd", st, (fc_bwd_kernel<1, 2, ET>), dim3(g.fc_wgs), dim3(kThreads), lds, a);
             else STGCN_LAUNCH_ETB("head.fc_bwd", st, (fc_bwd_kernel<1, 1, ET>), dim3(g.fc_wgs), dim3(kThreads), lds, a);
diff --git a/stgcn_amd/csrc/stgcn_kernels_fwd.hip.h b/stgcn_amd/csrc/stgcn_kernels_fwd.hip.h
--- a/stgcn_amd/csrc/stgcn_kernels_fwd.hip.h
+++ b/stgcn_amd/csrc/stgcn_kernels_fwd.hip.h
@@ -623,6 +623,17 @@
 __device__ __forceinline__ uint64_t ln_rowstat_offset(const LnRowstatOut& o) {
     return (o.rowstat && o.training) ? o.offset + (o.offset_dev ? *o.offset_dev : 0) : 0;
 }
+__device__ __forceinline__ float2 ln_rowstat4_us(f32x4 dy, f32x4 u, f32x4 s, f32x4 ga, float mean, float rstd, int act) {
+    float s1 = 0.f, s2 = 0.f;
+#pragma unroll
+    for (int i = 0; i < 4; ++i) {
+        const float xh = fmaf(act == 0 ? u[i] : tanh_f(u[i]), s[i], -mean) * rstd;
+        const float gg = dy[i] * ga[i];
+        s1 += gg;
+        s2 = fmaf(gg, xh, s2);
+    }
+    return make_float2(s1, s2);
+}
 template <typename ET = float>
 __device__ __forceinline__ float2 ln_rowstat4(const LnRowstatOut& o, uint64_t off, f32x4 dy, long slab, int node, int c) {
     const size_t e = ((size_t)slab * o.N + node) * o.C + c;
@@ -653,14 +664,7 @@
     const float mean = o.mean[slab], rstd = o.rstd[slab];
 #pragma unroll
     for (int i = 0; i < 4; ++i) dy[i] *= k[i];
-#pragma unroll
-    for (int i = 0; i < 4; ++i) {
-        const float xh = (gate_fwd(u[i], s[i], o.act) - mean) * rstd;
-        const float gg = dy[i] * ga[i];
-        s1 += gg;
-        s2 += gg * xh;
-    }
-    return make_float2(s1, s2);
+    return ln_rowstat4_us(dy, u, s, ga, mean, rstd, o.act);
 }
 
 struct LnGateBwdIn {
@@ -706,9 +710,30 @@
     int use_ticket;
 };
 
-template <int TM, int KC, bool PLAIN, typename ET, bool HEADF = false>
-__device__ __forceinline__ void tconv_fwd4_body(const Tconv4Args& aa, const HeadFcTail* ht) {
+__device__ __forceinline__ const float* label_ptr(const float* y, const long* tab, long stride, unsigned per_w, long e) {
+    if (!tab) return y + e;
+    const unsigned eu = (unsigned)e, b = eu / per_w;
+    return y + tab[b] * stride + (eu - b * per_w);
+}
+
+struct HeadLossTail {
+    const float* target;
+    const long* target_index;
+    long target_index_stride;
+    const long* target_window;
+    unsigned target_window_elems;
+    float loss_scale;
+    const float* W1d;
+    float* dh1;
+    float* dyln;
+    float2* rowstat_b;
+    float* part;
+};
+
+template <int TM, int KC, bool PLAIN, typename ET, bool HEADF = false, bool LOSS = false>
+__device__ __forceinline__ void tconv_fwd4_body(const Tconv4Args& aa, const HeadFcTail* ht, const HeadLossTail* hl = nullptr) {
     static_assert(!(PLAIN && HEADF), "the fused head tail follows the gated epilogue");
+    static_assert(HEADF || !LOSS, "the loss tail follows the fused head tail");
     constexpr int WAVES = 8, NT = 2, THREADS = 512, TR = TM * 16, NC = 256, COUT = 128, LDZ = NC + 4;
     const TconvFwdArgs& a = aa.f;
     ET* const U_ = et_ptr<ET>(a.U);
@@ -935,6 +960,20 @@
             }
             PreW<1, 8> w1;
             pre_load_weights<1, 8>(w1, f.W1p, 8, wave, 8);
+            PreW<1, LOSS ? 8 : 1> w1d;
+            float lab[LOSS ? NIT : 1];
+            if constexpr (LOSS) {
+                pre_load_weights<1, 8>(w1d, hl->W1d, 8, wave, 8);
+                const float* tgt = hl->target;
+                const long* ttab = nullptr;
+                if (hl->target_window) ttab = hl->target_window + *hl->target_index;
+                else if (hl->target_index) tgt += *hl->target_index * hl->target_index_stride;
+#pragma unroll
+                for (int it = 0; it < NIT; ++it) {
+                    const long R = row0 + (tid + it * THREADS) / C4N;
+                    lab[it] = R < rows ? *label_ptr(tgt, ttab, hl->target_index_stride, hl->target_window_elems, R) : 0.f;
+                }
+            }
             f32x4 ga[NIT], be[NIT];
 #pragma unroll
             for (int it = 0; it < NIT; ++it) {
@@ -1044,6 +1083,7 @@
                 for (int r = 0; r < 4; ++r) Zt[(i * 16 + 4 * g + r) * LDZ + COUT + wave * 16 + l15] = acc1[i][0][r];
             __syncthreads();
             ET* const hd_ = et_ptr<ET>(f.hd);
+            const float inv_n = 1.0f / (float)rows;
 #pragma unroll
             for (int it = 0; it < NIT; ++it) {
                 const int row = (tid + it * THREADS) / C4N;
@@ -1059,9 +1099,73 @@
                 float pd = h[0] * w2[0] + h[1] * w2[1] + h[2] * w2[2] + h[3] * w2[3];
 #pragma unroll
                 for (int m = 16; m >= 1; m >>= 1) pd += __shfl_xor(pd, m);
+                const float pred = pd + b2 + poison;
                 if (R < rows) {
                     stx4_wt(hd_ + (size_t)R * COUT + 4 * c4, h);
-                    if (c4 == 0) f.out[R] = pd + b2 + poison;
+                    if (c4 == 0) f.out[R] = pred;
+                }
+                if constexpr (LOSS) {
+                    f32x4 d = zero4(), q = zero4();
+                    float go = 0.f, sq = 0.f;
+                    if (R < rows) {
+                        const float df = pred - lab[it];
+                        go = 2.0f * df * inv_n * hl->loss_scale;
+                        sq = df * df;
+                        const f32x4 hr = et_round4<ET>(h);
+                        const float gs = f.training ? f.keep_scale : 1.0f;
+#pragma unroll
+                        for (int i = 0; i < 4; ++i) {
+                            d[i] = hr[i] != 0.f ? go * w2[i] * gs : 0.f;
+                            q[i] = go * hr[i];
+                        }
+                        stx4_wt(et_ptr<ET>(hl->dh1) + (size_t)R * COUT + 4 * c4, d);
+                    }
+                    st4(Zt + row * LDZ + COUT + 4 * c4, d);
+                    st4(Zt + row * LDZ + 4 * c4, q);
+                    if (c4 == 0) {
+                        Zt[row * LDZ + NC] = go;
+                        Zt[row * LDZ + NC + 1] = sq;
+                    }
+                }
+            }
+            if constexpr (LOSS) {
+                __syncthreads();
+                for (int idx = tid; idx < TM * (COUT + 2); idx += THREADS) {
+                    const int blk = idx / (COUT + 2), col = idx - blk * (COUT + 2);
+                    if (row0 + blk * 16 < rows) {
+                        const float* src = Zt + blk * 16 * LDZ + (col < COUT ? col : NC + col - COUT);
+                        float s = 0.f;
+                        for (int r = 0; r < 16; ++r) s += src[r * LDZ];
+                        hl->part[(size_t)(row0 / 16 + blk) * (COUT + 2) + col] = col == COUT + 1 ? s * inv_n : s;
+                    }
+                }
+                f32x4 acc2[TM][1];
+#pragma unroll
+                for (int i = 0; i < TM; ++i) acc2[i][0] = zero4();
+                pre_mma<TM, 1, 8, ET>(acc2, Zt + COUT, LDZ, 0, 8, w1d);
+                __syncthreads();
+#pragma unroll
+                for (int i = 0; i < TM; ++i)
+#pragma unroll
+                    for (int r = 0; r < 4; ++r) Zt[(i * 16 + 4 * g + r) * LDZ + wave * 16 + l15] = acc2[i][0][r];
+                __syncthreads();
+                ET* const dyln_ = et_ptr<ET>(hl->dyln);
+#pragma unroll
+                for (int it = 0; it < NIT; ++it) {
+                    const int row = (tid + it * THREADS) / C4N;
+                    const long R = row0 + row;
+                    const bool rin = R < rows;
+                    const f32x4 v = et_round4<ET>(ld4(Zt + row * LDZ + 4 * c4));
+                    if (rin) stx4_wt(dyln_ + (size_t)R * COUT + 4 * c4, v);
+                    const int wi = rin ? (int)(R / N) - s_lo : 0;
+                    float2 p = make_float2(0.f, 0.f);
+                    if (rin) p = ln_rowstat4_us(v, et_round4<ET>(uk[it]), et_round4<ET>(sk[it]), ga[it], wi ? mean2[1] : mean2[0], wi ? rstd2[1] : rstd2[0], a.act);
+#pragma unroll
+                    for (int m = C4N >> 1; m >= 1; m >>= 1) {
+                        p.x += __shfl_xor(p.x, m);
+                        p.y += __shfl_xor(p.y, m);
+                    }
+                    if (rin && c4 == 0) hl->rowstat_b[R] = p;
                 }
             }
             chain_exit(f.chain);
@@ -1075,6 +1179,10 @@
 template <int TM, int KC, typename ET>
 __global__ __launch_bounds__(512) void head_fwd_kernel(Tconv4Args aa, HeadFcTail ht) {
     tconv_fwd4_body<TM, KC, false, ET, true>(aa, &ht);
+}
+template <int TM, int KC, typename ET>
+__global__ __launch_bounds__(512) void head_fwd_loss_kernel(Tconv4Args aa, HeadFcTail ht, HeadLossTail hl) {
+    tconv_fwd4_body<TM, KC, false, ET, true, true>(aa, &ht, &hl);
 }
 
 struct GconvFwdArgs {
diff --git a/stgcn_amd/csrc/stgcn_kernels_head.hip.h b/stgcn_amd/csrc/stgcn_kernels_head.hip.h
--- a/stgcn_amd/csrc/stgcn_kernels_head.hip.h
+++ b/stgcn_amd/csrc/stgcn_kernels_head.hip.h
@@ -128,13 +128,8 @@
     unsigned target_window_elems;
     float loss_scale;
     LnRowstatOut rs;
+    int per_block;
 };
-
-__device__ __forceinline__ const float* label_ptr(const float* y, const long* tab, long stride, unsigned per_w, long e) {
-    if (!tab) return y + e;
-    const unsigned eu = (unsigned)e, b = eu / per_w;
-    return y + tab[b] * stride + (eu - b * per_w);
-}
 
 template <int WM, int NT, typename ET>
 __global__ __launch_bounds__(256) void fc_bwd_kernel(FcBwdArgs a) {
@@ -163,26 +158,52 @@
             const long R = row0 + row;
             f32x4 d = zero4();
             if (R < a.rows) {
-                float go;
+                float go, sq = 0.f;
                 if (a.pred) {
                     const float df = a.pred[R] - *label_ptr(tgt, ttab, a.target_index_stride, a.target_window_elems, R);
                     go = 2.0f * df * inv_n * a.loss_scale;
-                    if (c4 == 0) lsum += df * df;
+                    sq = df * df;
+                    if (c4 == 0) lsum += sq;
                 } else {
                     go = a.dout[R];
                 }
                 const f32x4 h = ldx4(et_ptr<ET>(a.hd) + (size_t)R * c1 + 4 * c4);
+                f32x4 q;
 #pragma unroll
                 for (int i = 0; i < 4; ++i) {
                     d[i] = h[i] != 0.f ? go * w2[i] * a.grad_scale : 0.f;
+                    q[i] = go * h[i];
                     dw2[i] += go * h[i];
                 }
                 if (c4 == 0) db2 += go;
                 stx4_wt(et_ptr<ET>(a.dh1) + (size_t)R * c1 + 4 * c4, d);
+                if (a.per_block) {
+                    st4(red + row * lda + 4 * c4, q);
+                    if (c4 == 0) {
+                        red[row * lda + c1] = go;
+                        red[row * lda + c1 + 1] = sq;
+                    }
+                }
+            } else if (a.per_block) {
+                st4(red + row * lda + 4 * c4, zero4());
+                if (c4 == 0) {
+                    red[row * lda + c1] = 0.f;
+                    red[row * lda + c1 + 1] = 0.f;
+                }
             }
             st4(At + row * lda + 4 * c4, d);
         }
         __syncthreads();
+        if (a.per_block) {
+            for (int idx = tid; idx < WM * (c1 + 2); idx += kThreads) {
+                const int blk = idx / (c1 + 2), col = idx - blk * (c1 + 2);
+                if (row0 + blk * 16 < a.rows) {
+                    float s = 0.f;
+                    for (int r = 0; r < 16; ++r) s += red[(blk * 16 + r) * lda + col];
+                    a.part[(size_t)(row0 / 16 + blk) * (c1 + 2) + col] = col == c1 + 1 ? s * inv_n : s;
+                }
+            }
+        }
         f32x4 acc[WM][NT];
 #pragma unroll
         for (int i = 0; i < WM; ++i)
@@ -229,6 +250,7 @@
             }
         }
     }
+    if (a.per_block) return;
     __syncthreads();
     st4(red + rsub * c1 + 4 * c4, dw2);
     if (c4 == 0) {
diff --git a/stgcn_amd/ops.py b/stgcn_amd/ops.py
--- a/stgcn_amd/ops.py
+++ b/stgcn_amd/ops.py
@@ -1,5 +1,6 @@
 from __future__ import annotations
 
+import contextlib
 import ctypes as C
 import os
 from dataclasses import dataclass
@@ -291,10 +292,37 @@
 
 
 class _PendingLoss:
-    __slots__ = ("placeholder", "pred", "target", "index", "index_stride", "window", "grad_scale", "loss")
+    __slots__ = ("placeholder", "pred", "target", "index", "index_stride", "window", "grad_scale", "loss", "in_forward")
 
 
 _pending_loss: Optional[_PendingLoss] = None
+
+
+class _HeadLossScope:
+    __slots__ = ("target", "grad_scale")
+
+
+_head_loss_scope: Optional[_HeadLossScope] = None
+_HEAD_FWD_LOSS = os.environ.get("STGCN_HEAD_FWD_LOSS", "1") != "0"
+
+
+@contextlib.contextmanager
+def head_loss_scope(target: torch.Tensor, grad_scale: float = 1.0):
+    global _head_loss_scope
+    prev = _head_loss_scope
+    sc = None
+    if _HEAD_FWD_LOSS and target is not None and target.dtype == torch.float32 and target.is_contiguous():
+        sc = _HeadLossScope()
+        sc.target, sc.grad_scale = target, float(grad_scale)
+    _head_loss_scope = sc
+    try:
+        yield
+    finally:
+        _head_loss_scope = prev
+
+
+def _loss_key(target: torch.Tensor, grad_scale: float):
+    return (target.data_ptr(), target.numel()) + tuple(_index_of(target)) + (float(grad_scale),)
 _VIEW_NODES = ("ViewBackward", "UnsafeViewBackward", "ReshapeAliasBackward", "UnsqueezeBackward", "SqueezeBackward", "AliasBackward")
 
 
@@ -322,6 +350,9 @@
     pl.pred, pl.target, pl.grad_scale = p, target, float(grad_scale)
     pl.index, pl.index_stride, pl.window = _index_of(target)
     pl.loss = torch.empty(1, dtype=torch.float32, device=p.device)
+    node = _head_node_of(pred)
+    pl.in_forward = (getattr(node, "loss_fwd", None) == _loss_key(target, grad_scale)
+                     and getattr(node, "loss_gen", None) == node.wsc.head_forwards)
     _pending_loss = pl
     try:
         pred.backward(pl.placeholder)
@@ -414,6 +445,7 @@
         self.bufs: Dict[int, torch.Tensor] = {}
         self.prepacked = False
         self.pending_sink = None
+        self.head_forwards = 0
 
     @property
     def buf(self) -> Optional[torch.Tensor]:
@@ -677,7 +709,7 @@
 
 
 def query_head_plan(desc: OutblockDesc) -> OutblockPlan:
-    key = tuple(getattr(desc, f) for f, _ in OutblockDesc._fields_) + (os.environ.get("STGCN_HEAD_FC_TILE"),)
+    key = tuple(getattr(desc, f) for f, _ in OutblockDesc._fields_) + (os.environ.get("STGCN_HEAD_FC_TILE"), os.environ.get("STGCN_HEAD_FUSE"))
     p = _head_plan_cache.get(key)
     if p is None:
         L = _lib.lib()
@@ -709,8 +741,24 @@
         saved = torch.empty(plan.saved_floats, dtype=torch.float32, device=dev)
         ws = wsc.get(plan.ws_floats, dev)
         pst = _head_struct(OutblockParams, ps)
-        L.check(L.dll.stgcn_outblock_forward(C.byref(desc), C.byref(pst), x_cl.data_ptr(), out.data_ptr(), saved.data_ptr(), ws.data_ptr(),
-                                             seed, offset, _optr(offset_dev), _stream_of(x_cl)), "stgcn_outblock_forward")
+        sc = _head_loss_scope
+        ctx.loss_fwd = None
+        wsc.head_forwards += 1
+        ctx.loss_gen = wsc.head_forwards
+        if (sc is not None and plan.fwd_loss_ok and any(ctx.needs_input_grad) and sc.target.numel() == plan.rows
+                and sc.target.device == dev):
+            desc.loss_in_forward = 1
+            hl = _lib.HeadLoss()
+            hl.target, hl.grad_scale = sc.target.data_ptr(), sc.grad_scale
+            hl.target_index_dev, hl.target_index_stride, hl.target_window_dev = _index_of(sc.target)
+            L.check(L.dll.stgcn_outblock_forward_loss(C.byref(desc), C.byref(pst), x_cl.data_ptr(), out.data_ptr(), saved.data_ptr(),
+                                                      ws.data_ptr(), C.byref(hl), seed, offset, _optr(offset_dev), _stream_of(x_cl)),
+                    "stgcn_outblock_forward_loss")
+            ctx.loss_fwd = _loss_key(sc.target, sc.grad_scale)
+            ctx.keep_target = sc.target
+        else:
+            L.check(L.dll.stgcn_outblock_forward(C.byref(desc), C.byref(pst), x_cl.data_ptr(), out.data_ptr(), saved.data_ptr(), ws.data_ptr(),
+                                                 seed, offset, _optr(offset_dev), _stream_of(x_cl)), "stgcn_outblock_forward")
         ctx.in_hook = _take_ln_hook(x_cl) if need_dx else None
         ctx.save_for_backward(x_cl, saved, *[p for p in params if p is not None])
         ctx.param_present = [p is not None for p in params]
@@ -735,6 +783,8 @@
         fused_loss = _pending_loss if (_pending_loss is not None and _pending_loss.placeholder.data_ptr() == dout.data_ptr()) else None
         if fused_loss is not None:
             _pending_loss = None
+            if fused_loss.in_forward:
+                desc.loss_in_forward = 1
         used = {"tc_aw": c_in > cfg.channels[0], "tc_ab": c_in > cfg.channels[0]}
         grads = []
         for name, p, need in zip(HEAD_PARAM_FIELDS, params, ctx.param_needs_grad):
diff --git a/stgcn_amd/train.py b/stgcn_amd/train.py
--- a/stgcn_amd/train.py
+++ b/stgcn_amd/train.py
@@ -160,7 +160,8 @@
 
 def fwd_loss_bwd(model, x, y):
     from . import ops
-    y_pred = model(x).reshape(len(x), -1)
+    with ops.head_loss_scope(y):
+        y_pred = model(x).reshape(len(x), -1)
     return ops.mse_backward(y_pred, y)[0]
 
 
@@ -211,7 +212,8 @@
                            "use train_step")
     arena.install()
     with ops.grad_sink_scope(arena.sink):
-        y_pred = model(x).reshape(len(x), -1)
+        with ops.head_loss_scope(y, 1.0 / world):
+            y_pred = model(x).reshape(len(x), -1)
         loss = ops.mse_backward(y_pred, y, grad_scale=1.0 / world)
     if world <= 1 and hasattr(optimizer, "flush_with"):
         optimizer.flush_with(arena.sink, arena.grads)
@@ -248,8 +250,10 @@
         model._step_counters = None
     try:
         if hi > lo:
-            pred = model(x[lo:hi]).reshape(hi - lo, -1)
-            loss = ops.mse_backward(pred, y[lo:hi].contiguous(), grad_scale=(hi - lo) / n)
+            y_loc = y[lo:hi].contiguous()
+            with ops.head_loss_scope(y_loc, (hi - lo) / n):
+                pred = model(x[lo:hi]).reshape(hi - lo, -1)
+            loss = ops.mse_backward(pred, y_loc, grad_scale=(hi - lo) / n)
             loss_sum = loss * ((hi - lo) / n)
     finally:
         if folded is not None:
@@ -502,7 +506,8 @@
         from . import ops
         self.arena.install()
         with ops.grad_sink_scope(self.arena.sink):
-            y_pred = self.model(self.x).reshape(len(self.x), -1)
+            with ops.head_loss_scope(self.y, 1.0 / self.world):
+                y_pred = self.model(self.x).reshape(len(self.x), -1)
             loss = ops.mse_backward(y_pred, self.y, grad_scale=1.0 / self.world)
         if self.world > 1:
             self.arena.sink.flush(stream=torch.cuda.current_stream(self.x.device).cuda_stream)
```

After: 92650 windows/s, median of 6. +2.8%, better.
